# dasongli1/Shift-Net

Hardware: AMD Instinct MI355X
Metric: restored frames/sec at 1280x720 T=16 bf16 (higher is better)
Workload: dtype bf16; 1 GPU; Shift-Net-s (gshift_deblur2), 1280x720, one_len=16 (T_in=20), one window per GPU, synthetic checkpoint; parallelism=clip-parallel x1, gsts_schedule=unit-major, one stream

## Files before the change

include/shiftnet_hip.h:

```cpp
#ifndef SHIFTNET_HIP_H
#define SHIFTNET_HIP_H
#include <stdint.h>

#ifdef __cplusplus
extern "C" {
#endif

#define SN_ABI_VERSION 20

#define SN_F32 0
#define SN_F16 1
#define SN_BF16 2

int sn_abi_version(void);

int sn_selftest_mfma(const float* a, const float* b, float* d, void* stream);

int sn_ingest(const void* src, int src_dtype, const void* noise, void* dst, int T, int C, int H, int W, void* stream);

typedef struct sn_conv_desc {
    const void* in[3];
    int n_in;
    int cs_in;
    int T, h_in, w_in;
    int in_mode;
    int k, stride, pad;
    int h_out, w_out;
    const void* wfrag;
    int mt, ks;
    const float* bias;
    int act;
    float prelu;
    const void* res;
    void* out;
    int cs_out;
    int out_mode;
    int c_out;
    int nchw_dtype;
    const void* sc;
    int sc_dtype;
    float* pool;
    const float* oscale;
    int oscale_stride;
    const void* res2;
    int flags;
    int clip_n, clip_T, clip_lo;
} sn_conv_desc;
#define SN_CONV_TILE_KERNEL 1
int sn_conv2d(const sn_conv_desc* d, void* stream);
int sn_conv_pool_blocks(const sn_conv_desc* d);
#define SN_CONV_K_GENERIC 1
#define SN_CONV_K_FAST    2
#define SN_CONV_K_STATS   3
#define SN_CONV_K_STREAM  4
#define SN_CONV_ROUTE(kernel, mt, a, d, mode, rl) (((kernel) << 24) | ((mt) << 20) | ((a) << 12) | ((d) << 8) | ((mode) << 4) | (rl))
int sn_conv2d_route(const sn_conv_desc* d, int lines_len, int ncu, int* plan);

int sn_upsample2_add(const void* lo, const void* res, void* out, int T, int hs, int ws, int cs, void* stream);

int sn_ca_mlp(const float* partial, int nblk, int cpad, int c, int cr, float inv_hw,
              const float* wa, const float* wb, float* ca, int T, unsigned* bad, void* stream);

int sn_cab_ca_scratch_floats(int T);
int sn_cab_ca(const float* partial, int nblk, int cpad, const void* mid, int cs, int c, int cr, int h, int w,
              const float* w2, const float* wa, const float* wb, float* scratch, float* ca, int T, void* stream);
int sn_cab_fused_supported(const sn_conv_desc* conv1, const sn_conv_desc* conv2);
int sn_cab_stats(const sn_conv_desc* conv1, int lines_len, void* stream);
int sn_cab_ca_lines(const float* partial, int nblk, int cpad, const void* lines, int lines_len, int cs, int c, int cr, int h, int w,
                    const float* w2, const float* wa, const float* wb, float* scratch, float* ca, int T, void* stream);
int sn_cab_fused(const sn_conv_desc* conv1, const sn_conv_desc* conv2, int tile_rows, void* stream);

int sn32_cab_ca(const float* partial, int nblk, int cpad, const float* mid, int c, int cr, int h, int w,
                const float* w2, const float* wa, const float* wb, float* scratch, float* ca, int T, void* stream);

typedef struct sn_unit_src {
    const void* x;
    int T, h, w, C;
    int mode;
    int wrap;
    const void* halo;
    int t0, nt;
    int clip;
} sn_unit_src;

int sn_gsts_gather(const sn_unit_src* s, const int8_t* offs, void* u, void* stream);

int sn_temporal_roll(const sn_unit_src* s, void* y, void* stream);

int sn_gsts_shiftconv(const sn_unit_src* s, const int8_t* offs, const uint32_t* w1, void* hw, void* stream);
int sn_gsts_shiftconv_mfma(const sn_unit_src* s, const int8_t* offs, const uint32_t* w1, void* hw, void* stream);
#define SN_K0_TILE 1
#define SN_K0_WALK 2
#define SN_K0_PLAN_LEN 10
typedef struct sn_k0_opts {
    int form;
    int seg;
    int wgs;
} sn_k0_opts;
int sn_gsts_shiftconv_mfma_plan(const sn_unit_src* s, int ncu, int* plan);
int sn_gsts_shiftconv_mfma_plan_opt(const sn_unit_src* s, int ncu, const sn_k0_opts* opt, int* plan);
int sn_gsts_shiftconv_mfma_opt(const sn_unit_src* s, const int8_t* offs, const uint32_t* w1, void* hw, const sn_k0_opts* opt, void* stream);

int sn_ln_gemm_gate(const sn_unit_src* s, const void* hw, const void* wfrag, const float* bias, const uint32_t* wdw,
                    void* g1, float* pool, int g1_blocked, void* stream);
int sn_lngate_blocks(int h, int w);

int sn_grp5_gemm_gate(const void* g1, const float* ca_in, const void* wgrp, const void* wfrag, void* g2, float* pool,
                      int T, int h, int w, int C, void* stream);
int sn_grp5_blocks(int h, int w);

int sn_planar_pitch(int w);
int sn_nhwc_to_planar(const void* x, void* xp, int T, int h, int w, int C, void* stream);

int sn_dw5m_blocks(int h, int w);
int sn_dw5m_gemm_gate(const void* g1p, const float* ca_in, const void* ttab, const void* wfrag, void* g2, float* pool,
                      int T, int h, int w, int C, void* stream);

typedef struct sn_phase1_weights {
    const void* wfrag1;
    const uint32_t* w3;
    const void* wgrp;
    const void* wfrag2;
} sn_phase1_weights;
typedef struct sn_se_fold {
    const float* wa;
    const float* wb;
    int c, cr;
    unsigned* ticket;
    float* ca;
    unsigned* bad;
} sn_se_fold;
typedef struct sn_phase1_opts {
    const float* g1_scale;
    int g1_sums;
    int team;
    void* g1_store;
} sn_phase1_opts;
int sn_phase1_pool_blocks(int T, int h, int w);
int sn_phase1_g1_store_bytes(int T, int h, int w, int C, long long* bytes);
int sn_gsts_cab2_phase1(const sn_unit_src* s, const void* hw, const sn_phase1_weights* wt, void* g2, float* pool, const sn_se_fold* se,
                        const sn_phase1_opts* opt, void* stream);
int sn_cab1_phase1(const sn_unit_src* s, const sn_phase1_weights* wt, void* g2, float* pool, const sn_se_fold* se, const sn_phase1_opts* opt, void* stream);
int sn_p1r_plan(int nfr, int h, int w, int ncu, int team, int* out7);
int sn_p1r_strip_begin(const int* plan7, int s, int w);

int sn_gsts_cab2_phase2(const sn_unit_src* s, const void* g2, const float* ca, const void* wfrag, const float* bias, void* y, void* stream);
int sn_cab1_phase2(const sn_unit_src* s, const void* g2, const float* ca, const void* wfrag, const float* bias, void* y, void* stream);

int sn_cab2_phase2_cab1_phase1_supported(const sn_unit_src* s);
int sn_cab2_phase2_cab1_phase1(const sn_unit_src* s, const void* g2_in, const float* ca, const void* wfrag, const float* bias, void* y,
                               const sn_phase1_weights* wt, void* g2, float* pool, const sn_se_fold* se, const sn_phase1_opts* opt, void* stream);


typedef struct sn32_conv_desc {
    const float* in[3];
    int c_in[3];
    int cs_in[3];
    int n_in;
    int T, h_in, w_in;
    int in_mode;
    int k, stride, pad, groups;
    int h_out, w_out, c_out;
    const float* w;
    const float* bias;
    int act; float prelu;
    const float* oscale; int oscale_stride;
    const float* res; int cs_res;
    void* out; int cs_out;
    int out_mode;
    int nchw_dtype; const void* sc;
    const void* wsplit;
    const float* iscale; int iscale_stride;
    const float* rscale; int rscale_stride;
    const float* ln_w; const float* ln_b;
    float* csum; int csum_cpad;
    int clip_n, clip_T, clip_lo;
} sn32_conv_desc;
int sn32_conv_csum_tiles(int h_out, int w_out);
int sn32_conv2d(const sn32_conv_desc* d, void* stream);
#define SN32_K_1X1      1
#define SN32_K_SPLIT    2
#define SN32_K_SPLIT_G8 3
#define SN32_K_EXACT    4
#define SN32_K_DW       5
#define SN32_K_DIRECT   6
#define SN32_ROUTE(kernel, a, b) (((kernel) << 16) | ((a) << 8) | (b))
int sn32_conv2d_route(const sn32_conv_desc* d);
int sn32_gsts_gather(const sn_unit_src* s, const int8_t* offs, float* u, float* u2, void* stream);
int sn32_gsts_shiftconv(const sn_unit_src* s, const int8_t* offs, const float* w, float* vin, float* u, void* stream);
int sn32_layernorm(const float* x, int cs_x, int K, const float* w, const float* b, float* out, int cs_out, long long npix, void* stream);
int sn32_gate(const float* a, int C, int mode, float* out, long long npix, void* stream);
int sn32_gate_sum(const float* a, int C, int cpad, int mode, float* out, int T, int hw, int nblk, float* partial, void* stream);
int sn32_conv1x1_gate2(const float* x, int cs_x, int cin, const void* wsplit, int C, int cpad, float* out, int T, int hw, float* partial, void* stream);
int sn32_dw_gate(const float* a, int cs_a, const float* w, int C, int cpad, float* out, int T, int h, int wd, int nblk, float* partial, void* stream);
int sn32_chan_sum(const float* x, int cs, int C, int cpad, int T, int hw, int nblk, float* partial, void* stream);
int sn32_scale_residual(const float* r, const float* x, const float* ca, int ca_stride, float* out, int T, int hw, int C, void* stream);
int sn32_ingest(const void* src, int src_dtype, const void* noise, float* dst, int T, int C, int H, int W, void* stream);


int sn_ingest_u8(const uint8_t* src, void* dst, int dst_dtype, int T, int H, int W, void* stream);
int sn_egress_blocks(void);
int sn_egress_u8(const void* out, int out_dtype, const uint8_t* gt, uint8_t* img, float* sse, int T, int H, int W, void* stream);
int sn_ssim_blocks(void);
int sn_ssim_u8(const void* out, int out_dtype, const uint8_t* gt, float* scratch, float* partial, int T, int H, int W, void* stream);

#define SN_YUV_444 0
#define SN_YUV_420_CENTER 1
#define SN_YUV_420_LEFT 2
#define SN_YUV_BT601 0
#define SN_YUV_BT709 1
#define SN_YUV_LIMITED 0
#define SN_YUV_FULL 1
typedef struct sn_yuv_fmt {
    int bits;
    int chroma;
    int matrix;
    int range;
} sn_yuv_fmt;
int sn_ingest_yuv(const uint8_t* src, const sn_yuv_fmt* fmt, void* dst, int dst_dtype, int T, int H, int W, int Hp, int Wp, void* stream);
int sn_egress_yuv(const void* out, int out_dtype, const sn_yuv_fmt* fmt, uint8_t* dst, int T, int H, int W, int Hp, int Wp, void* stream);

int sn_yuv_thumb(const uint8_t* src, const sn_yuv_fmt* fmt, uint16_t* dst, int T, int H, int W, void* stream);

// ... 100 lines not shown
```

shift-net_amd/csrc/sn_cabf.hip:

```cpp
#include "sn_common.h"
#include "../../include/shiftnet_hip.h"

int sn_cabp_launch(const sn_conv_desc* a, const sn_conv_desc* b, void* stream);

namespace {

struct CabK {
    const bf16_t* x; int h, w;
    const uint4* w1; const float* b1; float prelu; int act;
    const uint4* w2; const float* b2;
    const float* oscale; int oscale_stride;
    const bf16_t* res2; bf16_t* out;
    XcdTiles xg;
};

constexpr __host__ __device__ int cabf_lds_slots(int npb) {
    const int k = npb <= 2 ? 2 : 4 * ((npb - 2 + 3) / 4) + 2;
    return k <= npb + 1 ? k : ((npb & 1) ? npb : npb + 1);
}
constexpr int cabf_waves(int mt, int th) {
    return mt == 1 ? (th == 8 ? 6 : 3) : mt == 2 ? 4 : mt == 3 ? 2 : 2;
}

template <int MT, int CS, int TH, int NC1, int NC2>
__global__ __launch_bounds__(256, cabf_waves(MT, TH)) void cab_fused_kernel(const CabK P) {
    extern __shared__ __attribute__((aligned(16))) char smem[];
    constexpr int TW = 32, RH = TH + 4, RW = TW + 4, MH = TH + 2, MW = TW + 2, NPB = CS / 8;
    constexpr int PS = 16 * cabf_lds_slots(NPB);
    constexpr int KTOT = 9 * CS, KS = (KTOT + 31) / 32;
    constexpr int ROWP = RW * NPB, NITEM = RH * ROWP, NIT = (NITEM + 255) / 256;
    constexpr int X_BYTES = RH * RW * PS;
    constexpr int NM = MH * MW, NT1 = (NM + 15) / 16, PER1 = (NT1 + 3) / 4;
    constexpr int NT2 = (TH * TW) / 64, XB = TW / 16;
    char* const xs = smem;
    char* const ms = smem + X_BYTES;
    const int tid = threadIdx.x & 255, lane = tid & 63, wv = wave_id();
    const int g = lane >> 4, p = lane & 15;
    int t, tyi, txi;
    if (!sn_xcd_tile(P.xg, t, tyi, txi)) return;
    const int oy0 = tyi * TH, ox0 = txi * TW;

    {
        const int iy0 = oy0 - 2, ix0 = ox0 - 2;
        const bf16_t* inb = P.x + (size_t)t * P.h * P.w * CS;
        const bool interior = iy0 >= 0 && iy0 + RH <= P.h && ix0 >= 0 && ix0 + RW <= P.w;
        uint4 v[NIT];
        if (interior) {
#pragma unroll
            for (int k = 0; k < NIT; ++k) {
                const int idx = tid + k * 256, idc = idx < NITEM ? idx : NITEM - 1;
                const int r = idc / ROWP, i = idc - r * ROWP;
                v[k] = *(const uint4*)(inb + ((size_t)iy0 * P.w + ix0) * CS + (size_t)r * P.w * CS + i * 8);
            }
#pragma unroll
            for (int k = 0; k < NIT; ++k) {
                const int idx = tid + k * 256;
                const int r = idx / ROWP, i = idx - r * ROWP, px = i / NPB, blk = i - px * NPB;
                if (idx < NITEM) *(uint4*)(xs + (r * RW + px) * PS + blk * 16) = v[k];
            }
        } else {
            bool in[NIT];
#pragma unroll
            for (int k = 0; k < NIT; ++k) {
                const int idx = tid + k * 256, idc = idx < NITEM ? idx : NITEM - 1;
                const int r = idc / ROWP, i = idc - r * ROWP, px = i / NPB, blk = i - px * NPB;
                const int gy = iy0 + r, gx = ix0 + px;
                in[k] = gy >= 0 && gy < P.h && gx >= 0 && gx < P.w;
                v[k] = *(const uint4*)(inb + (in[k] ? ((size_t)gy * P.w + gx) * CS + blk * 8 : 0));
            }
#pragma unroll
            for (int k = 0; k < NIT; ++k) {
                const int idx = tid + k * 256;
                const int r = idx / ROWP, i = idx - r * ROWP, px = i / NPB, blk = i - px * NPB;
                if (idx < NITEM) *(uint4*)(xs + (r * RW + px) * PS + blk * 16) = in[k] ? v[k] : make_uint4(0, 0, 0, 0);
            }
        }
    }
    const int c0 = g * 4 * MT;
    const float slope = P.prelu;
    const int act = P.act != 1 ? 0 : ((slope >= 0.f && slope <= 1.f) ? 1 : 2);
    __syncthreads();

#pragma unroll
    for (int ch = 0; ch < (PER1 + NC1 - 1) / NC1; ++ch) {
        int pixbase[NC1], moff[NC1];
        bool live[NC1], inimg[NC1];
#pragma unroll
        for (int n = 0; n < NC1; ++n) {
            const int j = wv + 4 * (ch * NC1 + n);
            const int q = j * 16 + p, qc = q < NM ? q : NM - 1;
            const int my = qc / MW, mx = qc - my * MW;
            pixbase[n] = (my * RW + mx) * PS;
            moff[n] = qc * PS;
            live[n] = (ch * NC1 + n < PER1) && q < NM;
            const int gy = oy0 - 1 + my, gx = ox0 - 1 + mx;
            inimg[n] = gy >= 0 && gy < P.h && gx >= 0 && gx < P.w;
        }
        f32x4_t acc[MT][NC1];
#pragma unroll
        for (int m = 0; m < MT; ++m) {
            const float4 b4 = P.b1 ? *(const float4*)(P.b1 + c0 + m * 4) : make_float4(0.f, 0.f, 0.f, 0.f);
#pragma unroll
            for (int n = 0; n < NC1; ++n) acc[m][n] = (f32x4_t){b4.x, b4.y, b4.z, b4.w};
        }
#pragma unroll
        for (int s = 0; s < KS; ++s) {
            int toff = 0;
#pragma unroll
            for (int gg = 0; gg < 4; ++gg) {
                const int kk0 = (s * 4 + gg) * 8;
                const int tap = kk0 / CS, cc0 = kk0 - tap * CS, dy = tap / 3, dx = tap - dy * 3;
                const int o = kk0 < KTOT ? (dy * RW + dx) * PS + cc0 * 2 : 0;
                toff = g == gg ? o : toff;
            }
            bf16x8_t a[MT];
#pragma unroll
            for (int m = 0; m < MT; ++m) a[m] = as_frag(P.w1[(m * KS + s) * 64 + lane]);
            bf16x8_t b[NC1];
#pragma unroll
            for (int n = 0; n < NC1; ++n) b[n] = as_frag(*(const uint4*)(xs + pixbase[n] + toff));
#pragma unroll
            for (int m = 0; m < MT; ++m)
#pragma unroll
                for (int n = 0; n < NC1; ++n) acc[m][n] = mfma16(a[m], b[n], acc[m][n]);
        }
#pragma unroll
        for (int n = 0; n < NC1; ++n) {
            if (ch * NC1 + n >= PER1) continue;
            uint32_t wd[MT][2];
#pragma unroll
            for (int m = 0; m < MT; ++m) {
                float v[4] = {acc[m][n][0], acc[m][n][1], acc[m][n][2], acc[m][n][3]};
                if (act == 1) {
#pragma unroll
                    for (int r = 0; r < 4; ++r) v[r] = fmaxf(v[r], slope * v[r]);
                } else if (act == 2) {
#pragma unroll
                    for (int r = 0; r < 4; ++r) v[r] = fmaf(slope, fminf(v[r], 0.f), fmaxf(v[r], 0.f));
                }
                wd[m][0] = inimg[n] ? pack_bf2(v[0], v[1]) : 0u;
                wd[m][1] = inimg[n] ? pack_bf2(v[2], v[3]) : 0u;
            }
            if (live[n]) {
                char* dst = ms + moff[n] + c0 * 2;
                if constexpr (MT == 2 || MT == 4) {
#pragma unroll
                    for (int m = 0; m < MT; m += 2)
                        if (c0 + m * 4 < CS) *(uint4*)(dst + m * 8) = make_uint4(wd[m][0], wd[m][1], wd[m + 1][0], wd[m + 1][1]);
                } else {
#pragma unroll
                    for (int m = 0; m < MT; ++m)
                        if (c0 + m * 4 < CS) *(uint2*)(dst + m * 8) = make_uint2(wd[m][0], wd[m][1]);
                }
            }
        }
    }
// ... 1 lines not shown

    const bool full = (oy0 + TH <= P.h) && (ox0 + TW <= P.w);
    const size_t tbase = (((size_t)t * P.h + oy0) * P.w + ox0) * CS;
    bf16_t* const outb = P.out + tbase;
    const bf16_t* const res2b = P.res2 ? P.res2 + tbase : nullptr;
    float4 osc[MT];
    const bool has_osc = P.oscale != nullptr;
#pragma unroll
    for (int m = 0; m < MT; ++m)
        osc[m] = has_osc ? *(const float4*)(P.oscale + (size_t)t * P.oscale_stride + c0 + m * 4) : make_float4(1.f, 1.f, 1.f, 1.f);
#pragma unroll
    for (int ch = 0; ch < (NT2 + NC2 - 1) / NC2; ++ch) {
        int pixbase[NC2], loff[NC2], xoff[NC2];
        bool valid[NC2];
#pragma unroll
        for (int n = 0; n < NC2; ++n) {
            const int nl = ch * NC2 + n < NT2 ? ch * NC2 + n : NT2 - 1;
            const int nn = wv * NT2 + nl, row = nn / XB, xb = nn - row * XB;
            pixbase[n] = (row * MW + xb * 16 + p) * PS;
            xoff[n] = ((row + 2) * RW + xb * 16 + p + 2) * PS + c0 * 2;
            loff[n] = (row * P.w + xb * 16 + p) * CS + c0;
            valid[n] = full || ((oy0 + row < P.h) && (ox0 + xb * 16 + p < P.w));
        }
        f32x4_t acc[MT][NC2];
#pragma unroll
        for (int m = 0; m < MT; ++m) {
            const float4 b4 = P.b2 ? *(const float4*)(P.b2 + c0 + m * 4) : make_float4(0.f, 0.f, 0.f, 0.f);
#pragma unroll
            for (int n = 0; n < NC2; ++n) acc[m][n] = (f32x4_t){b4.x, b4.y, b4.z, b4.w};
        }
#pragma unroll
        for (int s = 0; s < KS; ++s) {
            int toff = 0;
#pragma unroll
            for (int gg = 0; gg < 4; ++gg) {
                const int kk0 = (s * 4 + gg) * 8;
                const int tap = kk0 / CS, cc0 = kk0 - tap * CS, dy = tap / 3, dx = tap - dy * 3;
                const int o = kk0 < KTOT ? (dy * MW + dx) * PS + cc0 * 2 : 0;
                toff = g == gg ? o : toff;
            }
            bf16x8_t a[MT];
#pragma unroll
            for (int m = 0; m < MT; ++m) a[m] = as_frag(P.w2[(m * KS + s) * 64 + lane]);
            bf16x8_t b[NC2];
#pragma unroll
            for (int n = 0; n < NC2; ++n) b[n] = as_frag(*(const uint4*)(ms + pixbase[n] + toff));
#pragma unroll
            for (int m = 0; m < MT; ++m)
#pragma unroll
                for (int n = 0; n < NC2; ++n) acc[m][n] = mfma16(a[m], b[n], acc[m][n]);
        }
#pragma unroll
        for (int n = 0; n < NC2; ++n) {
            if (ch * NC2 + n >= NT2) continue;
            float v[MT][4];
#pragma unroll
            for (int m = 0; m < MT; ++m) {
                v[m][0] = acc[m][n][0]; v[m][1] = acc[m][n][1]; v[m][2] = acc[m][n][2]; v[m][3] = acc[m][n][3];
                if (has_osc) { v[m][0] *= osc[m].x; v[m][1] *= osc[m].y; v[m][2] *= osc[m].z; v[m][3] *= osc[m].w; }
            }
            if constexpr (MT == 2 || MT == 4) {
#pragma unroll
                for (int m = 0; m < MT; m += 2)
                    if (c0 + m * 4 < CS) {
                        const uint4 rr = *(const uint4*)(xs + xoff[n] + m * 8);
                        v[m][0] += bf_lo(rr.x); v[m][1] += bf_hi(rr.x); v[m][2] += bf_lo(rr.y); v[m][3] += bf_hi(rr.y);
                        v[m + 1][0] += bf_lo(rr.z); v[m + 1][1] += bf_hi(rr.z); v[m + 1][2] += bf_lo(rr.w); v[m + 1][3] += bf_hi(rr.w);
                    }
            } else {
#pragma unroll
                for (int m = 0; m < MT; ++m)
                    if (c0 + m * 4 < CS) {
                        const uint2 rr = *(const uint2*)(xs + xoff[n] + m * 8);
                        v[m][0] += bf_lo(rr.x); v[m][1] += bf_hi(rr.x); v[m][2] += bf_lo(rr.y); v[m][3] += bf_hi(rr.y);
                    }
            }
            if (!valid[n]) continue;
            if (res2b) {
                const bf16_t* src = res2b + loff[n];
                if constexpr (MT == 2 || MT == 4) {
#pragma unroll
                    for (int m = 0; m < MT; m += 2)
                        if (c0 + m * 4 < CS) {
                            const uint4 rr = *(const uint4*)(src + m * 4);
                            v[m][0] += bf_lo(rr.x); v[m][1] += bf_hi(rr.x); v[m][2] += bf_lo(rr.y); v[m][3] += bf_hi(rr.y);
                            v[m + 1][0] += bf_lo(rr.z); v[m + 1][1] += bf_hi(rr.z); v[m + 1][2] += bf_lo(rr.w); v[m + 1][3] += bf_hi(rr.w);
                        }
                } else {
#pragma unroll
                    for (int m = 0; m < MT; ++m)
                        if (c0 + m * 4 < CS) {
                            const uint2 rr = *(const uint2*)(src + m * 4);
                            v[m][0] += bf_lo(rr.x); v[m][1] += bf_hi(rr.x); v[m][2] += bf_lo(rr.y); v[m][3] += bf_hi(rr.y);
                        }
                }
            }
            bf16_t* dst = outb + loff[n];
            if constexpr (MT == 2 || MT == 4) {
#pragma unroll
                for (int m = 0; m < MT; m += 2)
                    if (c0 + m * 4 < CS)
                        *(uint4*)(dst + m * 4) = make_uint4(pack_bf2(v[m][0], v[m][1]), pack_bf2(v[m][2], v[m][3]),
                                                            pack_bf2(v[m + 1][0], v[m + 1][1]), pack_bf2(v[m + 1][2], v[m + 1][3]));
            } else {
#pragma unroll
                for (int m = 0; m < MT; ++m)
                    if (c0 + m * 4 < CS) {
                        uint2 o; o.x = pack_bf2(v[m][0], v[m][1]); o.y = pack_bf2(v[m][2], v[m][3]);
                        *(uint2*)(dst + m * 4) = o;
                    }
            }
        }
    }
}

template <int MT, int CS, int TH, int NC1, int NC2>
int launch_cab_fused(const CabK& K, int T, hipStream_t st) {
    constexpr int TW = 32, PS = 16 * cabf_lds_slots(CS / 8);
    CabK P = K; P.xg = sn_xcd_tiles((K.w + TW - 1) / TW, (K.h + TH - 1) / TH, T);
    const dim3 grid = sn_xcd_grid(P.xg);
    const size_t lds = (size_t)((TH + 4) * (TW + 4) + (TH + 2) * (TW + 2)) * PS;
    if (lds > 64 * 1024) {
        if (hipFuncSetAttribute((const void*)cab_fused_kernel<MT, CS, TH, NC1, NC2>, hipFuncAttributeMaxDynamicSharedMemorySize, (int)lds) != hipSuccess)
            return SN_ELAUNCH;
    }
    hipLaunchKernelGGL((cab_fused_kernel<MT, CS, TH, NC1, NC2>), grid, dim3(256), lds, st, P);
    return sn_check_launch();
}

int cabf_key(const sn_conv_desc* a, const sn_conv_desc* b) {
    if (!a || !b) return 0;
    const sn_conv_desc* ds[2] = {a, b};
    for (const sn_conv_desc* d : ds)
        if (!(d->k == 3 && d->stride == 1 && d->pad == 1 && d->in_mode == 0 && d->out_mode == 0 && d->n_in == 1 && d->cs_in == d->cs_out &&
              d->ks == (9 * d->cs_in + 31) / 32 && d->h_in == d->h_out && d->w_in == d->w_out && d->wfrag &&
              !sn_remap_set(d->clip_n, d->clip_T, d->clip_lo))) return 0;
    if (a->mt != b->mt || a->cs_in != b->cs_in || a->T != b->T || a->h_in != b->h_in || a->w_in != b->w_in) return 0;
    const int key = a->mt * 1000 + a->cs_in;
    return (key == 1016 || key == 2024) ? key : 0;
}

}

extern "C" {

int sn_cab_fused_supported(const sn_conv_desc* conv1, const sn_conv_desc* conv2) { return cabf_key(conv1, conv2) != 0 ? 1 : 0; }

int sn_cab_fused(const sn_conv_desc* a, const sn_conv_desc* b, int tile_rows, void* stream) {
    sn_clear_error();
    const int key = cabf_key(a, b);
    if (!key) return SN_EINVAL;
    if (tile_rows == 0) {
        if (!a->in[0] || a->res || a->res2 || a->oscale || b->pool || b->act != 0 || !b->out || b->res != a->in[0] || a->h_in < 2 || a->w_in < 2) return SN_EINVAL;
        return sn_cabp_launch(a, b, stream);
    }
    if (!a->in[0] || a->res || a->res2 || a->oscale || b->pool || b->act != 0 || !b->out || b->res != a->in[0]) return SN_EINVAL;
    if (b->oscale && b->oscale_stride < 16 * b->mt) return SN_EINVAL;
    if (a->h_in < 2 || a->w_in < 2) return SN_EINVAL;
    CabK K;
    K.x = (const bf16_t*)a->in[0]; K.h = a->h_in; K.w = a->w_in;
    K.w1 = (const uint4*)a->wfrag; K.b1 = a->bias; K.prelu = a->prelu; K.act = a->act;
    K.w2 = (const uint4*)b->wfrag; K.b2 = b->bias; K.oscale = b->oscale; K.oscale_stride = b->oscale_stride;
    K.res2 = (const bf16_t*)b->res2; K.out = (bf16_t*)b->out;
    hipStream_t st = (hipStream_t)stream;
    const bool tall = tile_rows == 16;
    switch (key) {
        case 1016: return tall ? launch_cab_fused<1, 16, 16, 5, 4>(K, a->T, st) : launch_cab_fused<1, 16, 8, 6, 4>(K, a->T, st);
        case 2024: return tall ? launch_cab_fused<2, 24, 16, 5, 4>(K, a->T, st) : launch_cab_fused<2, 24, 8, 3, 4>(K, a->T, st);
        default: return SN_EINVAL;
    }
}

}
```

shift-net_amd/csrc/sn_conv.hip:

```cpp
#include "sn_common.h"
#include "../../include/shiftnet_hip.h"

int sn_conv3p_key(const sn_conv_desc* d, bool want_pool);
int sn_conv3p_pool_rows(const sn_conv_desc* d);
int sn_conv3p_route(const sn_conv_desc* d, int lines_len, int ncu, int* plan8);
int sn_conv3p_launch(const sn_conv_desc* d, int lines_len, int route, const int* plan8, void* stream);

namespace {

struct ConvK {
    const bf16_t* in0; const bf16_t* in1; const bf16_t* in2;
    int n_in, cs, cv;
    int hin, win, in_mode, k, stride, pad, hout, wout;
    const uint4* wfrag; int ks;
    const float* bias; int act; float prelu;
    const bf16_t* res; bf16_t* out; int cs_out, out_mode, c_out, nchw_dtype, sc_dtype;
    const void* sc; float* pool; const float* oscale; int oscale_stride; const bf16_t* res2;
    int rh, rw, ps;
    int clip_n, clip_T, clip_lo;
    int lines_len;
    XcdTiles xg;
    unsigned m_nblk8, m_rw, m_csb, m_cv, m_k;
};

constexpr __host__ __device__ int sn_lds_slots(int npb) {
    const int k = npb <= 2 ? 2 : 4 * ((npb - 2 + 3) / 4) + 2;
    return k <= npb + 1 ? k : ((npb & 1) ? npb : npb + 1);
}

__device__ __forceinline__ int fdiv(int x, unsigned magic) { return (int)(((unsigned)x * (unsigned long long)magic) >> 24); }

__device__ __forceinline__ uint4 ld_bilinear(const bf16_t* src, int t, int hs, int ws, int cs, int cb, int gy, int gx) {
    float sy = gy * 0.5f - 0.25f; if (sy < 0.f) sy = 0.f;
    float sx = gx * 0.5f - 0.25f; if (sx < 0.f) sx = 0.f;
    int y0 = (int)sy, x0 = (int)sx;
    int y1 = min(y0 + 1, hs - 1), x1 = min(x0 + 1, ws - 1);
    float ly = sy - y0, lx = sx - x0, hy = 1.f - ly, hx = 1.f - lx;
    const bf16_t* b = src + (size_t)t * hs * ws * cs + cb * 8;
    float v00[8], v01[8], v10[8], v11[8], o[8];
    unpack8(*(const uint4*)(b + ((size_t)y0 * ws + x0) * cs), v00);
    unpack8(*(const uint4*)(b + ((size_t)y0 * ws + x1) * cs), v01);
    unpack8(*(const uint4*)(b + ((size_t)y1 * ws + x0) * cs), v10);
    unpack8(*(const uint4*)(b + ((size_t)y1 * ws + x1) * cs), v11);
#pragma unroll
    for (int j = 0; j < 8; ++j) o[j] = hy * (hx * v00[j] + lx * v01[j]) + ly * (hx * v10[j] + lx * v11[j]);
    return pack8(o);
}

constexpr int sn_conv_waves(int mt) {
    return mt == 1 ? 6 : mt == 2 ? 5 : mt == 3 ? 4 : mt == 4 ? 3 : 2;
}
constexpr int sn_conv3_waves(int mt, int cs) {
    return mt == 1 ? 7 : mt == 2 ? 6 : mt == 3 ? (cs == 48 ? 3 : 4) : mt == 4 ? 3 : 2;
}

template <int MT, int TH, int TW>
__global__ __launch_bounds__(256, sn_conv_waves(MT)) void conv_mfma_kernel(const ConvK P) {
    extern __shared__ __attribute__((aligned(16))) char smem[];
    constexpr int NTW = (TH * TW) / 64;
    constexpr int XB = TW / 16;
    const int tid = threadIdx.x, lane = tid & 63, wv = wave_id();
    const int g = lane >> 4, p = lane & 15;
    int t, tyi, txi;
    if (!sn_xcd_tile(P.xg, t, tyi, txi)) return;
    const int ti = sn_remap_frame(t, P.clip_n, P.clip_T, P.clip_lo);
    const int oy0 = tyi * TH, ox0 = txi * TW;
    const int tile_bytes = P.rh * P.rw * P.ps;
    int* tapoff = (int*)(smem + tile_bytes);
    float* red = (float*)(smem + tile_bytes + ((P.ks * 4 * 4 + 15) & ~15));

    for (int e = tid; e < P.ks * 4; e += 256) {
        const int kk0 = e * 8, K = P.k * P.k * P.cv;
        int off = 0;
        if (kk0 < K) {
            const int tap = fdiv(kk0, P.m_cv), cc0 = kk0 - tap * P.cv;
            const int dy = fdiv(tap, P.m_k), dx = tap - dy * P.k;
            off = (dy * P.rw + dx) * P.ps + cc0 * 2;
        }
        tapoff[e] = off;
    }
    {
        const int nblk8 = P.cv >> 3, csb = P.cs >> 3, total = P.rh * P.rw * nblk8;
        const int iy0 = oy0 * P.stride - P.pad, ix0 = ox0 * P.stride - P.pad;
        for (int idx0 = tid; idx0 < total; idx0 += 4 * 256) {
            uint4 v[4];
            int dst[4];
#pragma unroll
            for (int u = 0; u < 4; ++u) {
                const int idx = idx0 + u * 256;
                const int idc = idx < total ? idx : tid;
                const int pix = fdiv(idc, P.m_nblk8), blk = idc - pix * nblk8;
                const int ry = fdiv(pix, P.m_rw), rx = pix - ry * P.rw;
                const int ii = fdiv(blk, P.m_csb), cb = blk - ii * csb;
                const bf16_t* src = ii == 0 ? P.in0 : (ii == 1 ? P.in1 : P.in2);
                const int gy = iy0 + ry, gx = ix0 + rx;
                const bool in = gy >= 0 && gy < P.hin && gx >= 0 && gx < P.win;
                dst[u] = idx < total ? (in ? pix * P.ps + blk * 16 : -(pix * P.ps + blk * 16) - 1) : 0x7fffffff;
                if (P.in_mode == 0) v[u] = *(const uint4*)(src + (in ? (((size_t)ti * P.hin + gy) * P.win + gx) * P.cs + cb * 8 : 0));
                else v[u] = in ? ld_bilinear(src, ti, P.hin >> 1, P.win >> 1, P.cs, cb, gy, gx) : make_uint4(0, 0, 0, 0);
            }
#pragma unroll
            for (int u = 0; u < 4; ++u) {
                if (dst[u] == 0x7fffffff) continue;
                const bool in = dst[u] >= 0;
                *(uint4*)(smem + (in ? dst[u] : -(dst[u] + 1))) = in ? v[u] : make_uint4(0, 0, 0, 0);
            }
        }
    }
    bf16x8_t a_cur[MT];
#pragma unroll
    for (int m = 0; m < MT; ++m) a_cur[m] = as_frag(P.wfrag[(m * P.ks) * 64 + lane]);
    __syncthreads();

    f32x4_t acc[MT][NTW];
#pragma unroll
    for (int m = 0; m < MT; ++m)
#pragma unroll
        for (int n = 0; n < NTW; ++n) acc[m][n] = (f32x4_t){0.f, 0.f, 0.f, 0.f};
    int pixbase[NTW];
#pragma unroll
    for (int n = 0; n < NTW; ++n) {
        const int nn = wv * NTW + n, row = nn / XB, xb = nn - row * XB;
        pixbase[n] = ((row * P.stride) * P.rw + (xb * 16 + p) * P.stride) * P.ps;
    }
    constexpr bool PRE_RES = MT == 1;
    uint2 rres[PRE_RES ? MT : 1][PRE_RES ? NTW : 1];
    if constexpr (PRE_RES) {
        const bf16_t* rb = P.res ? P.res : (const bf16_t*)P.wfrag;
#pragma unroll
        for (int n = 0; n < NTW; ++n) {
            const int nn = wv * NTW + n, row = nn / XB, xb = nn - row * XB;
            const int oy = oy0 + row, ox = ox0 + xb * 16 + p;
            const bool valid = P.res && (oy < P.hout) && (ox < P.wout);
            const size_t opix = ((size_t)t * P.hout + oy) * P.wout + ox;
#pragma unroll
            for (int m = 0; m < MT; ++m) {
                const int co0 = g * 4 * MT + m * 4;
                rres[m][n] = *(const uint2*)(rb + ((valid && co0 < P.cs_out) ? opix * P.cs_out + co0 : 0));
            }
        }
    }
    for (int s = 0; s < P.ks; ++s) {
        const int toff = tapoff[s * 4 + g];
        const int sn = s + 1 < P.ks ? s + 1 : s;
        bf16x8_t a_nxt[MT];
#pragma unroll
        for (int m = 0; m < MT; ++m) a_nxt[m] = as_frag(P.wfrag[(m * P.ks + sn) * 64 + lane]);
        bf16x8_t b[NTW];
#pragma unroll
        for (int n = 0; n < NTW; ++n) b[n] = as_frag(*(const uint4*)(smem + pixbase[n] + toff));
#pragma unroll
        for (int m = 0; m < MT; ++m)
#pragma unroll
// ... 406 lines not shown
    }
    __syncthreads();
    if (tid < cr) {
        float h = 0.f;
        for (int j = 0; j < c; ++j) h += wa[tid * c + j] * mean[j];
        hid[tid] = h > 0.f ? h : 0.f;
    }
    __syncthreads();
    if (tid < cpad) {
        float o = 0.f;
        if (tid < c) {
            for (int j = 0; j < cr; ++j) o += wb[tid * cr + j] * hid[j];
            o = sigmoidf_(o);
        }
        ca[(size_t)t * cpad + tid] = o;
    }
}

#define SN_CABCA_NS 16
__device__ __forceinline__ float cab_ldf(const bf16_t* p) { return bf_to_f(*p); }
__device__ __forceinline__ float cab_ldf(const float* p) { return *p; }
template <typename E>
__device__ __forceinline__ const E* cab_px(const E* mt, int L, int w, int cs, int line, int y, int x) {
    return L > 0 ? mt + ((size_t)line * L + (line < 2 ? x : y)) * cs : mt + ((size_t)y * w + x) * cs;
}
template <typename E>
__global__ __launch_bounds__(256) void cab_ca_part_kernel(const float* partial, int nblk, int cpad, const E* mid, int cs,
                                                        int h, int w, float* scratch, int L) {
    __shared__ float acc[256];
    const int t = blockIdx.y, sidx = blockIdx.x, tid = threadIdx.x;
    const E* mt = mid + (L > 0 ? (size_t)t * 4 * L * cs : (size_t)t * h * w * cs);
    float* out = scratch + ((size_t)t * SN_CABCA_NS + sidx) * 5 * 128;
    {
        const int nsplit = 256 / cpad, ch = tid % cpad, part = tid / cpad;
        float sm = 0.f;
        if (part < nsplit) {
            const float* pp = partial + (size_t)t * nblk * cpad + ch;
            for (int bb = sidx * nsplit + part; bb < nblk; bb += SN_CABCA_NS * nsplit) sm += pp[(size_t)bb * cpad];
        }
        acc[tid] = sm;
        __syncthreads();
        if (tid < cpad) {
            float m = 0.f;
            for (int q = 0; q < nsplit; ++q) m += acc[q * cpad + tid];
            if (tid < 128) out[tid] = m;
        }
        __syncthreads();
    }
    for (int line = 0; line < 4; ++line) {
        const int len = line < 2 ? w : h;
        const int nseg = 256 / cs, ch = tid % cs, seg = tid / cs;
        float sm = 0.f;
        if (seg < nseg)
            for (int i = sidx * nseg + seg; i < len; i += SN_CABCA_NS * nseg) {
                const int y = line == 0 ? 0 : (line == 1 ? h - 1 : i), x = line == 2 ? 0 : (line == 3 ? w - 1 : i);
                sm += cab_ldf(cab_px(mt, L, w, cs, line, y, x) + ch);
            }
        acc[tid] = sm;
        __syncthreads();
        if (tid < cs) {
            float m = 0.f;
            for (int q = 0; q < nseg; ++q) m += acc[q * cs + tid];
            out[(1 + line) * 128 + tid] = m;
        }
        __syncthreads();
    }
}

template <typename E>
__global__ __launch_bounds__(1024) void cab_ca_kernel(const float* scratch, int cpad, const E* mid, int cs, int c, int cr,
                                                     int h, int w, const float* w2, const float* wa, const float* wb, float* ca, int L) {
    __shared__ float acc[1024];
    __shared__ float S[9][128];
    __shared__ float mean[128];
    __shared__ float hid[128];
    const int t = blockIdx.x, tid = threadIdx.x;
    const E* mt = mid + (L > 0 ? (size_t)t * 4 * L * cs : (size_t)t * h * w * cs);
    if (tid < 5 * 128) {
        const int k = tid >> 7, ch = tid & 127;
        float m = 0.f;
        if (ch < (k == 0 ? cpad : cs)) {
            const float* sp = scratch + (size_t)t * SN_CABCA_NS * 5 * 128 + tid;
            for (int q = 0; q < SN_CABCA_NS; ++q) m += sp[q * 5 * 128];
        }
        S[k][ch] = m;
    }
    if (tid < cs) {
        S[5][tid] = cab_ldf(cab_px(mt, L, w, cs, 0, 0, 0) + tid);
        S[6][tid] = cab_ldf(cab_px(mt, L, w, cs, 0, 0, w - 1) + tid);
        S[7][tid] = cab_ldf(cab_px(mt, L, w, cs, 1, h - 1, 0) + tid);
        S[8][tid] = cab_ldf(cab_px(mt, L, w, cs, 1, h - 1, w - 1) + tid);
    }
    __syncthreads();
    {
        const int nsplit = 1024 / cpad, co = tid % cpad, part = tid / cpad;
        float r = 0.f;
        if (part < nsplit)
            for (int cin = part; cin < c; cin += nsplit) {
                const float tot = S[0][cin], r0 = S[1][cin], r1 = S[2][cin], c0 = S[3][cin], c1 = S[4][cin];
                const float k00 = S[5][cin], k01 = S[6][cin], k10 = S[7][cin], k11 = S[8][cin];
                const float* wk = w2 + (size_t)cin * 9 * cpad + co;
                const float rowex[3] = {r1, 0.f, r0}, colex[3] = {c1, 0.f, c0};
                const float cor[3][3] = {{k11, 0.f, k10}, {0.f, 0.f, 0.f}, {k01, 0.f, k00}};
#pragma unroll
                for (int ky = 0; ky < 3; ++ky)
#pragma unroll
                    for (int kx = 0; kx < 3; ++kx) r += wk[(ky * 3 + kx) * cpad] * (tot - rowex[ky] - colex[kx] + cor[ky][kx]);
            }
        acc[tid] = r;
        __syncthreads();
        if (tid < cpad) {
            float m = 0.f;
            for (int q = 0; q < nsplit; ++q) m += acc[q * cpad + tid];
            if (tid < 128) mean[tid] = m / ((float)h * (float)w);
        }
    }
    __syncthreads();
    if (tid < cr) {
        float hh = 0.f;
        for (int j = 0; j < c; ++j) hh += wa[tid * c + j] * mean[j];
        hid[tid] = hh > 0.f ? hh : 0.f;
    }
    __syncthreads();
    if (tid < cpad) {
        float o = 0.f;
        if (tid < c) {
            for (int j = 0; j < cr; ++j) o += wb[tid * cr + j] * hid[j];
            o = sigmoidf_(o);
        }
        ca[(size_t)t * cpad + tid] = o;
    }
}

__global__ void selftest_mfma_kernel(const float* a, const float* b, float* d) {
    const int lane = threadIdx.x, g = lane >> 4, m = lane & 15;
    float av[8], bv[8];
#pragma unroll
    for (int j = 0; j < 8; ++j) {
        av[j] = a[m * 32 + g * 8 + j];
        bv[j] = b[(g * 8 + j) * 16 + m];
    }
    f32x4_t acc = {0.f, 0.f, 0.f, 0.f};
    acc = mfma16(as_frag(pack8(av)), as_frag(pack8(bv)), acc);
#pragma unroll
    for (int r = 0; r < 4; ++r) d[(g * 4 + r) * 16 + m] = acc[r];
}

__global__ __launch_bounds__(256) void upsample2_add_kernel(const bf16_t* __restrict__ lo, const bf16_t* __restrict__ res, bf16_t* __restrict__ out,
                                                            int hs, int ws, int npb) {
    const int w2 = 2 * ws, cs = npb * 8, i = (int)blockIdx.y, t = (int)blockIdx.z;
    const int e = (int)blockIdx.x * 256 + (int)threadIdx.x;
    if (e >= w2 * npb) return;
    const int x = e / npb, piece = e - x * npb;
    float sx = x * 0.5f - 0.25f; if (sx < 0.f) sx = 0.f;
    const int x0 = (int)sx, x1 = min(x0 + 1, ws - 1);
    const float lx = sx - x0, hx = 1.f - lx;
    const int ra = max(i - 1, 0), rc = min(i + 1, hs - 1);
    const bf16_t* b = lo + (size_t)t * hs * ws * cs + piece * 8;
    const uint4 qa0 = *(const uint4*)(b + ((size_t)ra * ws + x0) * cs), qa1 = *(const uint4*)(b + ((size_t)ra * ws + x1) * cs);
    const uint4 qb0 = *(const uint4*)(b + ((size_t)i * ws + x0) * cs), qb1 = *(const uint4*)(b + ((size_t)i * ws + x1) * cs);
    const uint4 qc0 = *(const uint4*)(b + ((size_t)rc * ws + x0) * cs), qc1 = *(const uint4*)(b + ((size_t)rc * ws + x1) * cs);
    const size_t o0 = (((size_t)t * 2 * hs + 2 * i) * w2 + x) * cs + piece * 8, o1 = o0 + (size_t)w2 * cs;
    const uint4 r0 = *(const uint4*)(res + o0), r1 = *(const uint4*)(res + o1);
    float a0[8], a1[8], b0[8], b1[8], c0[8], c1[8], f0[8], f1[8], u0[8], u1[8];
    unpack8(qa0, a0); unpack8(qa1, a1); unpack8(qb0, b0); unpack8(qb1, b1); unpack8(qc0, c0); unpack8(qc1, c1); unpack8(r0, f0); unpack8(r1, f1);
    const float ly0 = i > 0 ? 0.75f : 0.f, hy0 = 1.f - ly0;
#pragma unroll
    for (int j = 0; j < 8; ++j) {
        const float va = hx * a0[j] + lx * a1[j], vb = hx * b0[j] + lx * b1[j], vc = hx * c0[j] + lx * c1[j];
        u0[j] = (hy0 * va + ly0 * vb) + f0[j];
        u1[j] = (0.75f * vb + 0.25f * vc) + f1[j];
    }
    *(uint4*)(out + o0) = pack8(u0);
    *(uint4*)(out + o1) = pack8(u1);
}

}

extern "C" {

int sn_abi_version(void) { return SN_ABI_VERSION; }

int sn_selftest_mfma(const float* a, const float* b, float* d, void* stream) {
    sn_clear_error();
    hipLaunchKernelGGL(selftest_mfma_kernel, dim3(1), dim3(64), 0, (hipStream_t)stream, a, b, d);
    return sn_check_launch();
}

int sn_ingest(const void* src, int dt, const void* noise, void* dst, int T, int C, int H, int W, void* stream) {
    sn_clear_error();
    if (!src || !dst || C < 1 || C + (noise ? 1 : 0) > 8 || dt < 0 || dt > 2) return SN_EINVAL;
    const int hw = H * W;
    hipLaunchKernelGGL(ingest_kernel, dim3((hw + 255) / 256, T), dim3(256), 0, (hipStream_t)stream, src, dt, noise, (uint4*)dst, C, hw);
    return sn_check_launch();
}

static int conv3_key(const sn_conv_desc* d) {
    if (!(d->k == 3 && d->stride == 1 && d->pad == 1 && d->in_mode == 0 && d->out_mode == 0 && d->n_in == 1 && d->ks == (9 * d->cs_in + 31) / 32)) return 0;
    const int key = d->mt * 1000 + d->cs_in;
    return (key == 1016 || key == 2024 || key == 4064 || key == 3040 || key == 3048 || key == 5080) ? key : 0;
}
static void conv_tile(const sn_conv_desc* d, int* th, int* tw) {
    if (d->stride == 1) { *tw = 32; *th = 8; }
    else if (d->n_in * d->cs_in <= 24 && !(d->flags & (1 << 15))) { *th = 8; *tw = 32; }
    else { *th = 4; *tw = 16; }
}

int sn_conv_pool_blocks(const sn_conv_desc* d) {
    if (!d) return SN_EINVAL;
    if (!(d->flags & SN_CONV_TILE_KERNEL)) {
        const int rows = sn_conv3p_pool_rows(d);
        if (rows > 0) return rows;
    }
    int th, tw; conv_tile(d, &th, &tw);
    return ((d->h_out + th - 1) / th) * ((d->w_out + tw - 1) / tw);
}

static int conv_ps(const sn_conv_desc* d) {
    const int blocks = d->n_in * d->cs_in >> 3;
    return d->stride == 1 ? 16 * sn_lds_slots(blocks) : ((blocks & 1) ? blocks * 16 : blocks * 16 + 16);
}

static int conv_route(const sn_conv_desc* d, int lines_len, int ncu, int* plan8) {
    if (!d) return SN_EINVAL;
    const bool stream_ok = !(d->flags & SN_CONV_TILE_KERNEL);
    if (lines_len > 0) {
        if (!d->out || !d->pool || !d->wfrag || !d->in[0] || d->res || d->res2 || d->oscale || d->cs_in != d->cs_out ||
            sn_remap_set(d->clip_n, d->clip_T, d->clip_lo)) return SN_EINVAL;
        if (lines_len < (d->h_out > d->w_out ? d->h_out : d->w_out) || d->h_out < 2 || d->w_out < 2) return SN_EINVAL;
        if (stream_ok) {
            const int r = sn_conv3p_route(d, lines_len, ncu, plan8);
            if (r >= 0) return r;
        }
        const int key = conv3_key(d);
        if (key != 1016 && key != 2024) return SN_EINVAL;
        return SN_CONV_ROUTE(SN_CONV_K_STATS, key / 1000, key % 1000, 0, 0, 0);
    }
    if (d->n_in < 1 || d->n_in > 3 || (d->cs_in & 7) || (d->cs_out & 7) || !d->wfrag) return SN_EINVAL;
    if (!d->out) return SN_EINVAL;
    if (d->k < 1 || d->k > 5 || (d->stride != 1 && d->stride != 2) || d->mt < 1 || d->mt > 6 || d->ks < 1) return SN_EINVAL;
    if (d->in_mode == 1 && ((d->h_in | d->w_in) & 1)) return SN_EINVAL;
    if (d->out_mode == 2 && (!d->sc || d->c_out > 4 * d->mt || d->nchw_dtype < 0 || d->nchw_dtype > 2 || d->sc_dtype < 0 || d->sc_dtype > 2)) return SN_EINVAL;
    if (d->ks * 32 < d->k * d->k * d->n_in * d->cs_in) return SN_EINVAL;
    if (d->oscale && d->oscale_stride < 16 * d->mt) return SN_EINVAL;
    if ((d->res || d->res2) && d->out_mode != 0) return SN_EINVAL;
    if (d->out_mode == 1 && d->cs_out != 4 * d->mt) return SN_EINVAL;
    const bool remap = sn_remap_set(d->clip_n, d->clip_T, d->clip_lo);
    if (!sn_remap_ok(d->T, d->clip_n, d->clip_T, d->clip_lo) || (remap && (conv3_key(d) || (stream_ok && sn_conv3p_key(d, false)))))
        return SN_EINVAL;
    if (stream_ok && sn_conv3p_key(d, false)) {
        const int r = sn_conv3p_route(d, 0, ncu, plan8);
        if (r >= 0) return r;
    }
    const int key = conv3_key(d);
    if (key) return SN_CONV_ROUTE(SN_CONV_K_FAST, key / 1000, key % 1000, 0, 0, 0);
    int th, tw; conv_tile(d, &th, &tw);
    if (conv_generic_lds(th, tw, d->stride, d->k, conv_ps(d), d->ks, d->mt) > 160 * 1024) return SN_EINVAL;
    return SN_CONV_ROUTE(SN_CONV_K_GENERIC, d->mt, th, 0, 0, 0);
}

int sn_conv2d_route(const sn_conv_desc* d, int lines_len, int ncu, int* plan) {
    sn_clear_error();
    return conv_route(d, lines_len, ncu, plan);
}

int sn_conv2d(const sn_conv_desc* d, void* stream) {
    sn_clear_error();
    int plan8[8];
    const int route = conv_route(d, 0, 0, plan8);
    if (route < 0) return route;
    ConvK K;
    K.in0 = (const bf16_t*)d->in[0]; K.in1 = (const bf16_t*)d->in[1]; K.in2 = (const bf16_t*)d->in[2];
    K.n_in = d->n_in; K.cs = d->cs_in; K.cv = d->n_in * d->cs_in;
    K.hin = d->h_in; K.win = d->w_in; K.in_mode = d->in_mode; K.k = d->k; K.stride = d->stride; K.pad = d->pad;
    K.hout = d->h_out; K.wout = d->w_out;
    K.wfrag = (const uint4*)d->wfrag; K.ks = d->ks; K.bias = d->bias; K.act = d->act; K.prelu = d->prelu;
    K.res = (const bf16_t*)d->res; K.out = (bf16_t*)d->out; K.cs_out = d->cs_out; K.out_mode = d->out_mode;
    K.c_out = d->c_out; K.nchw_dtype = d->nchw_dtype; K.sc_dtype = d->sc_dtype; K.sc = d->sc; K.pool = d->pool; K.oscale = d->oscale; K.oscale_stride = d->oscale_stride; K.res2 = (const bf16_t*)d->res2;
    K.ps = conv_ps(d);
    K.rh = K.rw = 0; K.lines_len = 0;
    K.clip_n = d->clip_n; K.clip_T = d->clip_T; K.clip_lo = d->clip_lo;
    hipStream_t st = (hipStream_t)stream;
    const int mt = (route >> 20) & 15, a = (route >> 12) & 255;
    switch (route >> 24) {
        case SN_CONV_K_STREAM: return sn_conv3p_launch(d, 0, route, plan8, stream);
        case SN_CONV_K_FAST:
            switch (mt * 1000 + a) {
                case 1016: return launch_conv3_fast<1, 16>(K, d->T, st);
                case 2024: return launch_conv3_fast<2, 24>(K, d->T, st);
                case 4064: return launch_conv3_fast<4, 64>(K, d->T, st);
                case 3040: return launch_conv3_fast<3, 40>(K, d->T, st);
                case 3048: return launch_conv3_fast<3, 48>(K, d->T, st);
                case 5080: return launch_conv3_fast<5, 80>(K, d->T, st);
                default: return SN_EINVAL;
            }
        case SN_CONV_K_GENERIC: return a == 8 ? launch_conv<8, 32>(K, mt, d->T, st) : launch_conv<4, 16>(K, mt, d->T, st);
        default: return SN_EINVAL;
    }
}


int sn_ca_mlp(const float* partial, int nblk, int cpad, int c, int cr, float inv_hw,
              const float* wa, const float* wb, float* ca, int T, unsigned* bad, void* stream) {
    sn_clear_error();
    if (!partial || !wa || !wb || !ca || cpad < 16 || cpad > 128 || c > cpad || cr > 128 || cr < 1 || nblk < 1) return SN_EINVAL;
    hipLaunchKernelGGL(ca_mlp_kernel, dim3(T), dim3(1024), 0, (hipStream_t)stream, partial, nblk, cpad, c, cr, inv_hw, wa, wb, ca, bad);
    return sn_check_launch();
}

int sn_cab_ca_scratch_floats(int T) { return T * SN_CABCA_NS * 5 * 128; }

static int cab_ca_launch(const float* partial, int nblk, int cpad, const void* mid, int lines_len, int cs, int c, int cr, int h, int w,
                         const float* w2, const float* wa, const float* wb, float* scratch, float* ca, int T, void* stream) {
    sn_clear_error();
    if (!partial || !mid || !w2 || !wa || !wb || !ca || !scratch || cpad < 16 || cpad > 128 || cs > 128 || (cs & 7) || c > cs ||
        c > cpad || cr < 1 || cr > 128 || nblk < 1 || h < 2 || w < 2 || (lines_len != 0 && lines_len < (h > w ? h : w))) return SN_EINVAL;
    hipLaunchKernelGGL(cab_ca_part_kernel<bf16_t>, dim3(SN_CABCA_NS, T), dim3(256), 0, (hipStream_t)stream, partial, nblk, cpad,
                       (const bf16_t*)mid, cs, h, w, scratch, lines_len);
    hipLaunchKernelGGL(cab_ca_kernel<bf16_t>, dim3(T), dim3(1024), 0, (hipStream_t)stream, (const float*)scratch, cpad, (const bf16_t*)mid, cs,
                       c, cr, h, w, w2, wa, wb, ca, lines_len);
    return sn_check_launch();
}

int sn_cab_ca(const float* partial, int nblk, int cpad, const void* mid, int cs, int c, int cr, int h, int w,
// ... 51 lines not shown
```

shift-net_amd/csrc/sn_conv3p.hip:

```cpp
#include "sn_common.h"
#include "../../include/shiftnet_hip.h"

namespace {

typedef __attribute__((address_space(3))) void lds_void_t;

struct C3P {
    const bf16_t* in; const bf16_t* res; bf16_t* out;
    const uint4* wfrag; const float* bias; const float* oscale; int oscale_stride;
    const uint4* w2; const float* b2;
    float* pool; int pool_rows;
    int act; float prelu;
    int T, h, w, ntx, nty;
    int dbg;
    int lines_len;
    int S, nseg, nsg, qs;
};

__device__ __forceinline__ float max_bare(float a, float b) {
    float r;
    asm("v_max_f32 %0, %1, %2" : "=v"(r) : "v"(a), "v"(b));
    return r;
}

__device__ __forceinline__ float mul_then_add(float a, float b, float c) {
    float r;
    asm("v_mul_f32 %0, %1, %2\n\tv_add_f32 %0, %0, %3" : "=&v"(r) : "v"(a), "v"(b), "v"(c));
    return r;
}

__device__ __forceinline__ void dma16(const __amdgpu_buffer_rsrc_t rs, char* dst, int voffset) {
    __builtin_amdgcn_raw_ptr_buffer_load_lds(rs, (lds_void_t*)dst, 16, voffset, 0, 0, 0);
}

template <typename V> __device__ __forceinline__ void pin(V& x) { asm volatile("" : "+v"(x)); }

template <int N> __device__ __forceinline__ void wait_vmcnt() { asm volatile("s_waitcnt vmcnt(%0)" ::"n"(N) : "memory"); }

__device__ __forceinline__ __amdgpu_buffer_rsrc_t frame_rsrc(const bf16_t* base, int frame_bytes) {
    return __builtin_amdgcn_make_buffer_rsrc((void*)base, 0, frame_bytes, 0x00020000);
}

constexpr int c3p_waves(int mt) { return mt == 1 ? 4 : mt == 2 ? 3 : 2; }

template <int MT, int CS, int TH, int D, int MODE, bool RL = false>
__global__ __launch_bounds__(320, c3p_waves(MT)) void conv3p_kernel(const C3P P) {
    extern __shared__ __attribute__((aligned(16))) char smem[];
    constexpr int TW = 32, RH = TH + 2, RW = TW + 2, NPB = CS / 8, PSB = CS * 2;
    constexpr int KTOT = 9 * CS, KS = (KTOT + 31) / 32;
    constexpr int ROWP = RW * NPB, NITEM = RH * ROWP, NDMA = (NITEM + 63) / 64, XBUF = NDMA * 1024;
    static_assert(!RL || MODE == 2, "residual staging belongs to MODE 2");
    constexpr int RDMA = RL ? (TH * TW * NPB) / 64 : 0;
    constexpr int NBUF = D + 1, BUFSZ = XBUF + RDMA * 1024, NL = NDMA + RDMA;
    constexpr bool WLDS = MT * KS > 16;
    constexpr int WBYTES = WLDS ? MT * KS * 1024 : 0;
    constexpr int RPW = TH / 4, NTW = RPW * 2;
    constexpr int NH = MT == 1 ? (NTW < 4 ? NTW : 4) : 2;
    static_assert(NTW % NH == 0 && NTW <= 4 * NH, "passes");
    static_assert(TH % 4 == 0 && NL * (D - 1) <= 63 && D >= 1, "tile / prefetch shape");
    const int lane = threadIdx.x & 63, wv = wave_id();
    const int G = (int)gridDim.x, c = ((int)blockIdx.x & 7) * (G >> 3) + ((int)blockIdx.x >> 3);
    const int fseg = c * P.qs, nsegs = min(P.qs, P.nsg - fseg);
    if (nsegs <= 0) return;
    int t = fseg / (P.ntx * P.nseg), tx, ty, n = 0;
    {
        const int rem = fseg - t * (P.ntx * P.nseg);
        tx = rem / P.nseg;
        const int sg = rem - tx * P.nseg;
        ty = sg * P.S;
        const int tail = P.nty - (P.nseg - 1) * P.S;
        for (int k = 0, g2 = sg; k < nsegs; ++k) { n += g2 == P.nseg - 1 ? tail : P.S; if (++g2 == P.nseg) g2 = 0; }
    }
    n = __builtin_amdgcn_readfirstlane(n);
    t = __builtin_amdgcn_readfirstlane(t); tx = __builtin_amdgcn_readfirstlane(tx); ty = __builtin_amdgcn_readfirstlane(ty);
    const int rowpitch = P.w * PSB, frame_bytes = P.h * rowpitch;
    const size_t frame_elems = (size_t)P.h * P.w * CS;
    char* const xbufs = smem + WBYTES;
    if constexpr (WLDS) {
        for (int i = (int)threadIdx.x; i < MT * KS * 64; i += 320) *(uint4*)(smem + i * 16) = P.wfrag[i];
        __syncthreads();
    }

    if (wv == 4) {
        int voff[NDMA], pxk[NDMA];
#pragma unroll
        for (int k = 0; k < NDMA; ++k) {
            const int i = k * 64 + lane, ic = i < NITEM ? i : NITEM - 1;
            const int r = ic / ROWP, j = ic - r * ROWP;
            voff[k] = r * rowpitch + j * 16;
            pxk[k] = j / NPB;
        }
        int rvoff[RL ? RDMA : 1];
        if constexpr (RL) {
#pragma unroll
            for (int k = 0; k < RDMA; ++k) {
                const int i = k * 64 + lane, row = i / (TW * NPB), rem = i - row * (TW * NPB);
                rvoff[k] = row * rowpitch + rem * 16;
            }
        }
        int ft = t, ftx = tx, fty = ty;
        for (int i = -D; i < n; ++i) {
            if (i >= 0) {
                if (n - 1 - i >= D - 1) wait_vmcnt<NL * (D - 1)>(); else wait_vmcnt<0>();
                __builtin_amdgcn_s_barrier();
            }
            const int j = i + D;
            if (j < n && !(P.dbg & 1)) {
                const __amdgpu_buffer_rsrc_t rs = frame_rsrc(P.in + (size_t)ft * frame_elems, frame_bytes);
                const int ix0 = ftx * TW - 1;
                const int o = ((fty * TH - 1) * P.w + ix0) * PSB;
                const bool edge = ftx == 0 || ix0 + RW > P.w;
                char* const dst = xbufs + (j % NBUF) * BUFSZ;
#pragma unroll
                for (int k = 0; k < NDMA; ++k) {
                    int vo = voff[k] + o;
                    if (edge) { const int gx = ix0 + pxk[k]; vo = (gx < 0 || gx >= P.w) ? (int)0x80000000 : vo; }
                    dma16(rs, dst + k * 1024, vo);
                }
                if constexpr (RL) {
                    const __amdgpu_buffer_rsrc_t rr = frame_rsrc(P.res + (size_t)ft * frame_elems, frame_bytes);
                    const int o2 = ((fty * TH) * P.w + ftx * TW) * PSB;
#pragma unroll
                    for (int k = 0; k < RDMA; ++k)
                        dma16(rr, dst + XBUF + k * 1024, rvoff[k] + o2);
                }
                if (++fty == P.nty) { fty = 0; if (++ftx == P.ntx) { ftx = 0; ++ft; } }
            }
        }
        return;
    }

    const int g = lane >> 4, p = lane & 15;
    const int c0 = g * 4 * MT;
    int addr_s[KS];
    const int lane_base = ((wv * RPW) * RW + p) * PSB;
#pragma unroll
    for (int s = 0; s < KS; ++s) {
        int toff = 0;
#pragma unroll
        for (int gg = 0; gg < 4; ++gg) {
            const int kk0 = (s * 4 + gg) * 8;
            const int tap = kk0 / CS, cc0 = kk0 - tap * CS, dy = tap / 3, dx = tap - dy * 3;
            const int o = kk0 < KTOT ? (dy * RW + dx) * PSB + cc0 * 2 : 0;
            toff = g == gg ? o : toff;
        }
        addr_s[s] = lane_base + toff;
    }
    bf16x8_t A[WLDS ? 1 : MT][WLDS ? 1 : KS];
    if constexpr (!WLDS) {
#pragma unroll
        for (int m = 0; m < MT; ++m)
#pragma unroll
            for (int s = 0; s < KS; ++s) A[m][s] = as_frag(P.wfrag[(m * KS + s) * 64 + lane]);
    }
    const char* const wl = smem + lane * 16;
    f32x4_t biasv[MT];
#pragma unroll
    for (int m = 0; m < MT; ++m) {
        const float4 b4 = P.bias ? *(const float4*)(P.bias + c0 + m * 4) : make_float4(0.f, 0.f, 0.f, 0.f);
        biasv[m] = (f32x4_t){b4.x, b4.y, b4.z, b4.w};
    }
    const float slope = P.prelu;
    float4 osc[MT];
    auto load_osc = [&](int ft) {
        if constexpr (MODE == 2) {
#pragma unroll
            for (int m = 0; m < MT; ++m) osc[m] = *(const float4*)(P.oscale + (size_t)ft * P.oscale_stride + c0 + m * 4);
        }
    };
    load_osc(t);
    auto pin_loaded = [&]() __attribute__((always_inline)) {
        if constexpr (!WLDS) {
#pragma unroll
            for (int m = 0; m < MT; ++m)
#pragma unroll
                for (int s = 0; s < KS; ++s) pin(A[m][s]);
        }
#pragma unroll
        for (int m = 0; m < MT; ++m) {
            pin(biasv[m]);
            if constexpr (MODE == 2) { pin(osc[m].x); pin(osc[m].y); pin(osc[m].z); pin(osc[m].w); }
        }
    };
    pin_loaded();
    constexpr int OOR = (int)0x80000000;
    constexpr int PIECE = (MT == 2 || MT == 4) ? 16 : 8;
    constexpr int NP = (MT * 8) / PIECE;
    typedef unsigned rword_t __attribute__((ext_vector_type(PIECE / 4)));
    int ooff[RPW][NP];
#pragma unroll
    for (int rr = 0; rr < RPW; ++rr)
#pragma unroll
        for (int q = 0; q < NP; ++q)
            ooff[rr][q] = (c0 + q * (PIECE / 2) < CS) ? ((wv * RPW + rr) * P.w + p) * PSB + c0 * 2 + q * PIECE : OOR;
    typedef rword_t rset_t[(MODE == 2 && !RL) ? NTW : 1][(MODE == 2 && !RL) ? NP : 1];
    rset_t rA, rB;
    auto load_res = [&](rset_t& rnxt, int ft, int ftx, int fty) __attribute__((always_inline)) {
        if constexpr (MODE == 2 && !RL) {
            const __amdgpu_buffer_rsrc_t rr = frame_rsrc(P.res + (size_t)ft * frame_elems, frame_bytes);
            const int o2 = ((fty * TH) * P.w + ftx * TW) * PSB;
#pragma unroll
            for (int nn = 0; nn < NTW; ++nn)
#pragma unroll
                for (int q = 0; q < NP; ++q) {
                    const int vo = o2 + ooff[nn >> 1][q] + (nn & 1) * 16 * PSB;
                    if constexpr (PIECE == 16) rnxt[nn][q] = __builtin_amdgcn_raw_buffer_load_b128(rr, vo, 0, 0);
                    else rnxt[nn][q] = __builtin_amdgcn_raw_buffer_load_b64(rr, vo, 0, 0);
                }
        }
    };
    load_res(rA, t, tx, ty);
    float psum[MT][4];
#pragma unroll
    for (int m = 0; m < MT; ++m)
#pragma unroll
        for (int r = 0; r < 4; ++r) psum[m][r] = 0.f;
    auto flush_pool = [&](int ft, int ftx, int fsg) {
        if constexpr (MODE == 1 || MODE == 3) {
            const int row = (ftx * P.nseg + fsg) * 4 + wv;
            float* dst = P.pool + ((size_t)ft * P.pool_rows + row) * (16 * MT);
#pragma unroll
            for (int m = 0; m < MT; ++m)
#pragma unroll
                for (int r = 0; r < 4; ++r) {
                    const float sm = row_sum16(psum[m][r]);
                    if (p == 0) dst[c0 + m * 4 + r] = sm;
                    psum[m][r] = 0.f;
                }
        }
    };

    const int raddr = XBUF + ((wv * RPW) * TW + p) * PSB + c0 * 2;
    auto finish = [&](const f32x4_t (&acc)[MT][NH], const rset_t& rres, const char* xs, const int N0, const __amdgpu_buffer_rsrc_t ro, int o2, const bool MASKED,
                      int ylim, int xlim) __attribute__((always_inline)) {
#pragma unroll
        for (int nh = 0; nh < NH; ++nh) {
            const int nn = N0 + nh, rr = nn >> 1, xb = nn & 1;
            float v[MT][4];
#pragma unroll
            for (int m = 0; m < MT; ++m) {
                v[m][0] = acc[m][nh][0]; v[m][1] = acc[m][nh][1]; v[m][2] = acc[m][nh][2]; v[m][3] = acc[m][nh][3];
                if constexpr (MODE == 1 || MODE == 3) {
#pragma unroll
                    for (int r = 0; r < 4; ++r) {
                        v[m][r] = max_bare(v[m][r], slope * v[m][r]);
                    }
                }
            }
            if constexpr (MODE == 2) {
#pragma unroll
                for (int m = 0; m < MT; ++m) {
                    rword_t qv;
                    if constexpr (RL) qv = *(const rword_t*)(xs + raddr + (rr * TW + xb * 16) * PSB + ((m * 8) / PIECE) * PIECE);
                    else qv = rres[nn][(m * 8) / PIECE];
                    const unsigned lo = qv[((m * 8) % PIECE) / 4], hi = qv[((m * 8) % PIECE) / 4 + 1];
                    v[m][0] = mul_then_add(v[m][0], osc[m].x, bf_lo(lo)); v[m][1] = mul_then_add(v[m][1], osc[m].y, bf_hi(lo));
                    v[m][2] = mul_then_add(v[m][2], osc[m].z, bf_lo(hi)); v[m][3] = mul_then_add(v[m][3], osc[m].w, bf_hi(hi));
                }
            }
            bool ok = true;
            if (MASKED) ok = (rr < ylim) && (xb * 16 < xlim);
            if constexpr (MODE == 1 || MODE == 3) {
#pragma unroll
                for (int m = 0; m < MT; ++m)
#pragma unroll
                    for (int r = 0; r < 4; ++r) psum[m][r] += (MASKED && !ok) ? 0.f : v[m][r];
            }
            if constexpr (MODE == 3) {
                if (MASKED && ok && c0 < CS) {
                    const int oy = ty * TH + wv * RPW + rr, ox = tx * TW + xb * 16 + p;
                    bf16_t* const lb = P.out + (size_t)t * 4 * P.lines_len * CS + c0;
                    bf16_t* tgt[4] = {oy == 0 ? lb + (size_t)ox * CS : nullptr, oy == P.h - 1 ? lb + ((size_t)P.lines_len + ox) * CS : nullptr,
                                      ox == 0 ? lb + ((size_t)2 * P.lines_len + oy) * CS : nullptr, ox == P.w - 1 ? lb + ((size_t)3 * P.lines_len + oy) * CS : nullptr};
#pragma unroll
                    for (int e = 0; e < 4; ++e) {
                        if (!tgt[e]) continue;
#pragma unroll
                        for (int m = 0; m < MT; ++m)
                            if (c0 + m * 4 < CS) *(uint2*)(tgt[e] + m * 4) = make_uint2(pack_bf2(v[m][0], v[m][1]), pack_bf2(v[m][2], v[m][3]));
                    }
                }
                continue;
            }
#pragma unroll
            for (int q = 0; q < NP; ++q) {
                int vo = o2 + ooff[rr][q] + xb * 16 * PSB;
                if (MASKED) vo = ok ? vo : OOR;
                if (P.dbg & 4) vo = OOR;
                if constexpr (PIECE == 16) {
                    const int m = q * 2;
                    const rword_t d = {pack_bf2(v[m][0], v[m][1]), pack_bf2(v[m][2], v[m][3]), pack_bf2(v[m + 1][0], v[m + 1][1]), pack_bf2(v[m + 1][2], v[m + 1][3])};
                    __builtin_amdgcn_raw_buffer_store_b128(d, ro, vo, 0, 0);
                } else {
                    const rword_t d = {pack_bf2(v[q][0], v[q][1]), pack_bf2(v[q][2], v[q][3])};
                    __builtin_amdgcn_raw_buffer_store_b64(d, ro, vo, 0, 0);
                }
            }
        }
    };

    int sgi = ty / P.S, sleft = min(P.S, P.nty - ty);
    int t2 = t, tx2 = tx, ty2 = ty;
    auto advance2 = [&]() { if (++ty2 == P.nty) { ty2 = 0; if (++tx2 == P.ntx) { tx2 = 0; ++t2; } } };
    advance2();
    auto tile = [&](const int i, const rset_t& rres, rset_t& rnxt) __attribute__((always_inline)) {
        __builtin_amdgcn_s_barrier();
        const char* const xs = xbufs + (i % NBUF) * BUFSZ;
        if (i + 1 < n) load_res(rnxt, t2, tx2, ty2);
        const int oy0 = ty * TH, ox0 = tx * TW;
        const __amdgpu_buffer_rsrc_t ro = frame_rsrc(P.out + (size_t)t * frame_elems, frame_bytes);
        const int o2 = (oy0 * P.w + ox0) * PSB;
        const bool full = (oy0 + TH <= P.h) && (ox0 + TW <= P.w);
#pragma unroll
        for (int ps = 0; ps < NTW / NH; ++ps) {
            const int N0 = ps * NH;
            f32x4_t acc[MT][NH];
            bf16x8_t bq[2][NH], aq[2][WLDS ? MT : 1];
#pragma unroll
            for (int m = 0; m < MT; ++m)
#pragma unroll
                for (int nh = 0; nh < NH; ++nh) acc[m][nh] = biasv[m];
            if (!(P.dbg & 2)) {
#pragma unroll
            for (int nh = 0; nh < NH; ++nh)
                bq[0][nh] = as_frag(*(const uint4*)(xs + addr_s[0] + (((N0 + nh) >> 1) * RW + ((N0 + nh) & 1) * 16) * PSB));
            if constexpr (WLDS) {
#pragma unroll
                for (int m = 0; m < MT; ++m) aq[0][m] = as_frag(*(const uint4*)(wl + (m * KS) * 1024));
            }
#pragma unroll
            for (int s = 0; s < KS; ++s) {
                if (s + 1 < KS) {
#pragma unroll
                    for (int nh = 0; nh < NH; ++nh)
                        bq[(s + 1) & 1][nh] = as_frag(*(const uint4*)(xs + addr_s[s + 1] + (((N0 + nh) >> 1) * RW + ((N0 + nh) & 1) * 16) * PSB));
                    if constexpr (WLDS) {
#pragma unroll
                        for (int m = 0; m < MT; ++m) aq[(s + 1) & 1][m] = as_frag(*(const uint4*)(wl + (m * KS + s + 1) * 1024));
                    }
                }
                __builtin_amdgcn_sched_barrier(0);
#pragma unroll
                for (int m = 0; m < MT; ++m)
#pragma unroll
                    for (int nh = 0; nh < NH; ++nh)
                        acc[m][nh] = mfma16(WLDS ? aq[s & 1][m] : A[WLDS ? 0 : m][WLDS ? 0 : s], bq[s & 1][nh], s == 0 ? biasv[m] : acc[m][nh]);
                __builtin_amdgcn_sched_barrier(0);
            }
            }
            const bool plain = full && !(MODE == 3 && (ty == 0 || ty == P.nty - 1 || tx == 0 || tx == P.ntx - 1));
            if (plain) finish(acc, rres, xs, N0, ro, o2, false, 0, 0);
            else finish(acc, rres, xs, N0, ro, o2, true, P.h - oy0 - wv * RPW, P.w - ox0 - p);
        }
        if (--sleft == 0) {
            flush_pool(t, tx, sgi);
            ++sgi;
            sleft = min(P.S, P.nty - ty - 1);
        }
        if (++ty == P.nty) {
            ty = 0; sgi = 0; sleft = min(P.S, P.nty);
            if (++tx == P.ntx) {
                tx = 0;
                ++t;
                if (i + 1 < n) {
                    load_osc(t);
                    if constexpr (MODE == 2) {
#pragma unroll
                        for (int m = 0; m < MT; ++m) { pin(osc[m].x); pin(osc[m].y); pin(osc[m].z); pin(osc[m].w); }
                    }
                }
            }
        }
        advance2();
    };
    for (int i = 0; i < n; i += 2) {
        tile(i, rA, rB);
        if (i + 1 < n) tile(i + 1, rB, rA);
    }
}

template <int MT, int CS, int TH, int D, int WR>
__global__ __launch_bounds__(320, c3p_waves(MT)) void cabp_kernel(const C3P P) {
    extern __shared__ __attribute__((aligned(16))) char smem[];
    constexpr int TW = 32, RH = TH + 4, RW = TW + 4, MH = TH + 2, MW = TW + 2, NPB = CS / 8, PSB = CS * 2;
    constexpr int KTOT = 9 * CS, KS = (KTOT + 31) / 32;
    constexpr int ROWP = RW * NPB, NITEM = RH * ROWP, NDMA = (NITEM + 63) / 64, XBUF = NDMA * 1024;
    constexpr int NBUF = D + 1, NL = NDMA;
    constexpr bool W1L = !(WR & 1), W2L = !(WR & 2);
    constexpr int WSET = MT * KS * 1024, W2OFF = W1L ? WSET : 0, WBYTES = W2OFF + (W2L ? WSET : 0);
    constexpr int NM = MH * MW, NT1 = (NM + 15) / 16, PER1 = (NT1 + 3) / 4;
    constexpr int NH1 = MT == 1 ? 3 : 2;
    constexpr int RPW = TH / 4, NTW = RPW * 2, NH = MT == 1 ? (NTW < 4 ? NTW : 4) : 2;
    constexpr int MIDB = (NM * PSB + 15) / 16 * 16;
    static_assert(TH % 4 == 0 && NL * (D - 1) <= 63 && D >= 1 && PER1 % NH1 == 0 && NTW % NH == 0, "tile / prefetch shape");
    const int lane = threadIdx.x & 63, wv = wave_id();
    const int G = (int)gridDim.x, c = ((int)blockIdx.x & 7) * (G >> 3) + ((int)blockIdx.x >> 3);
    const int fseg = c * P.qs, nsegs = min(P.qs, P.nsg - fseg);
    if (nsegs <= 0) return;
    int t = fseg / (P.ntx * P.nseg), tx, ty, n = 0;
    {
        const int rem = fseg - t * (P.ntx * P.nseg);
        tx = rem / P.nseg;
        const int sg = rem - tx * P.nseg;
        ty = sg * P.S;
        const int tail = P.nty - (P.nseg - 1) * P.S;
        for (int k = 0, g2 = sg; k < nsegs; ++k) { n += g2 == P.nseg - 1 ? tail : P.S; if (++g2 == P.nseg) g2 = 0; }
    }
    n = __builtin_amdgcn_readfirstlane(n);
    t = __builtin_amdgcn_readfirstlane(t); tx = __builtin_amdgcn_readfirstlane(tx); ty = __builtin_amdgcn_readfirstlane(ty);
    const int rowpitch = P.w * PSB, frame_bytes = P.h * rowpitch;
    const size_t frame_elems = (size_t)P.h * P.w * CS;
    char* const mids = smem + WBYTES;
    char* const xbufs = mids + MIDB;
    if constexpr (W1L || W2L) {
        for (int i = (int)threadIdx.x; i < MT * KS * 64; i += 320) {
            if constexpr (W1L) *(uint4*)(smem + i * 16) = P.wfrag[i];
            if constexpr (W2L) *(uint4*)(smem + W2OFF + i * 16) = P.w2[i];
        }
        __syncthreads();
    }

    if (wv == 4) {
        int voff[NDMA], pxk[NDMA];
#pragma unroll
        for (int k = 0; k < NDMA; ++k) {
            const int i = k * 64 + lane, ic = i < NITEM ? i : NITEM - 1;
            const int r = ic / ROWP, j = ic - r * ROWP;
            voff[k] = r * rowpitch + j * 16;
            pxk[k] = j / NPB;
        }
        int ft = t, ftx = tx, fty = ty;
        for (int i = -D; i < n; ++i) {
            if (i >= 0) {
                if (n - 1 - i >= D - 1) wait_vmcnt<NL * (D - 1)>(); else wait_vmcnt<0>();
                __builtin_amdgcn_s_barrier();
            }
            const int j = i + D;
            if (j < n) {
                const __amdgpu_buffer_rsrc_t rs = frame_rsrc(P.in + (size_t)ft * frame_elems, frame_bytes);
                const int ix0 = ftx * TW - 2;
                const int o = ((fty * TH - 2) * P.w + ix0) * PSB;
                const bool edge = ftx == 0 || ix0 + RW > P.w;
                char* const dst = xbufs + (j % NBUF) * XBUF;
#pragma unroll
                for (int k = 0; k < NDMA; ++k) {
                    int vo = voff[k] + o;
                    if (edge) { const int gx = ix0 + pxk[k]; vo = (gx < 0 || gx >= P.w) ? (int)0x80000000 : vo; }
                    dma16(rs, dst + k * 1024, vo);
                }
                if (++fty == P.nty) { fty = 0; if (++ftx == P.ntx) { ftx = 0; ++ft; } }
            }
            if (i >= 0) __builtin_amdgcn_s_barrier();
        }
        return;
    }

    const int g = lane >> 4, p = lane & 15;
    const int c0 = g * 4 * MT;
    int toff1[KS], addr2[KS];
    const int lane_base2 = ((wv * RPW) * MW + p) * PSB;
#pragma unroll
    for (int s = 0; s < KS; ++s) {
        int o1 = 0, o2 = 0;
#pragma unroll
        for (int gg = 0; gg < 4; ++gg) {
            const int kk0 = (s * 4 + gg) * 8;
            const int tap = kk0 / CS, cc0 = kk0 - tap * CS, dy = tap / 3, dx = tap - dy * 3;
            const int a = kk0 < KTOT ? (dy * RW + dx) * PSB + cc0 * 2 : 0, b = kk0 < KTOT ? (dy * MW + dx) * PSB + cc0 * 2 : 0;
            o1 = g == gg ? a : o1; o2 = g == gg ? b : o2;
        }
        toff1[s] = o1;
        addr2[s] = lane_base2 + o2;
    }
    int pix1[PER1], mwr[PER1];
#pragma unroll
    for (int i = 0; i < PER1; ++i) {
        const int q = (wv + 4 * i) * 16 + p, qc = q < NM ? q : NM - 1;
        const int my = qc / MW, mx = qc - my * MW;
        pix1[i] = (my * RW + mx) * PSB;
        mwr[i] = (q < NM && c0 < CS) ? qc * PSB + c0 * 2 : -1;
    }
    bf16x8_t A1[W1L ? 1 : MT][W1L ? 1 : KS], A2[W2L ? 1 : MT][W2L ? 1 : KS];
    if constexpr (!W1L) {
#pragma unroll
        for (int m = 0; m < MT; ++m)
#pragma unroll
            for (int s = 0; s < KS; ++s) A1[m][s] = as_frag(P.wfrag[(m * KS + s) * 64 + lane]);
    }
    if constexpr (!W2L) {
#pragma unroll
        for (int m = 0; m < MT; ++m)
#pragma unroll
            for (int s = 0; s < KS; ++s) A2[m][s] = as_frag(P.w2[(m * KS + s) * 64 + lane]);
    }
    const char* const wl = smem + lane * 16;
    f32x4_t bias1[MT], bias2[MT];
#pragma unroll
    for (int m = 0; m < MT; ++m) {
        const float4 a4 = P.bias ? *(const float4*)(P.bias + c0 + m * 4) : make_float4(0.f, 0.f, 0.f, 0.f);
        const float4 b4 = P.b2 ? *(const float4*)(P.b2 + c0 + m * 4) : make_float4(0.f, 0.f, 0.f, 0.f);
        bias1[m] = (f32x4_t){a4.x, a4.y, a4.z, a4.w};
        bias2[m] = (f32x4_t){b4.x, b4.y, b4.z, b4.w};
    }
    const float slope = P.prelu;
    float4 osc[MT];
    auto load_osc = [&](int ft) {
#pragma unroll
        for (int m = 0; m < MT; ++m) osc[m] = *(const float4*)(P.oscale + (size_t)ft * P.oscale_stride + c0 + m * 4);
    };
    load_osc(t);
    auto pin_osc = [&]() __attribute__((always_inline)) {
#pragma unroll
        for (int m = 0; m < MT; ++m) { pin(osc[m].x); pin(osc[m].y); pin(osc[m].z); pin(osc[m].w); }
    };
#pragma unroll
    for (int m = 0; m < MT; ++m) {
        pin(bias1[m]); pin(bias2[m]);
        if constexpr (!W1L) {
#pragma unroll
            for (int s = 0; s < KS; ++s) pin(A1[m][s]);
        }
        if constexpr (!W2L) {
#pragma unroll
            for (int s = 0; s < KS; ++s) pin(A2[m][s]);
        }
    }
    pin_osc();
    constexpr int OOR = (int)0x80000000;
    constexpr int PIECE = (MT == 2 || MT == 4) ? 16 : 8, NP = (MT * 8) / PIECE;
    typedef unsigned rword_t __attribute__((ext_vector_type(PIECE / 4)));
    int ooff[RPW][NP];
#pragma unroll
    for (int rr = 0; rr < RPW; ++rr)
#pragma unroll
        for (int q = 0; q < NP; ++q)
            ooff[rr][q] = (c0 + q * (PIECE / 2) < CS) ? ((wv * RPW + rr) * P.w + p) * PSB + c0 * 2 + q * PIECE : OOR;
    const int raddr = ((wv * RPW + 2) * RW + p + 2) * PSB + c0 * 2;

    for (int i = 0; i < n; ++i) {
        __builtin_amdgcn_s_barrier();
        const char* const xs = xbufs + (i % NBUF) * XBUF;
        const int oy0 = ty * TH, ox0 = tx * TW;
        const bool inner = oy0 >= 1 && oy0 + TH + 1 <= P.h && ox0 >= 1 && ox0 + TW + 1 <= P.w;
#pragma unroll
        for (int ps = 0; ps < PER1 / NH1; ++ps) {
            f32x4_t acc[MT][NH1];
            bf16x8_t bq[2][NH1], aq[2][W1L ? MT : 1];
#pragma unroll
            for (int nh = 0; nh < NH1; ++nh) bq[0][nh] = as_frag(*(const uint4*)(xs + pix1[ps * NH1 + nh] + toff1[0]));
            if constexpr (W1L) {
#pragma unroll
                for (int m = 0; m < MT; ++m) aq[0][m] = as_frag(*(const uint4*)(wl + (m * KS) * 1024));
            }
#pragma unroll
            for (int s = 0; s < KS; ++s) {
                if (s + 1 < KS) {
#pragma unroll
                    for (int nh = 0; nh < NH1; ++nh) bq[(s + 1) & 1][nh] = as_frag(*(const uint4*)(xs + pix1[ps * NH1 + nh] + toff1[s + 1]));
                    if constexpr (W1L) {
#pragma unroll
                        for (int m = 0; m < MT; ++m) aq[(s + 1) & 1][m] = as_frag(*(const uint4*)(wl + (m * KS + s + 1) * 1024));
                    }
                }
                __builtin_amdgcn_sched_barrier(0);
#pragma unroll
                for (int m = 0; m < MT; ++m)
#pragma unroll
                    for (int nh = 0; nh < NH1; ++nh)
                        acc[m][nh] = mfma16(W1L ? aq[s & 1][m] : A1[W1L ? 0 : m][W1L ? 0 : s], bq[s & 1][nh], s == 0 ? bias1[m] : acc[m][nh]);
                __builtin_amdgcn_sched_barrier(0);
            }
#pragma unroll
            for (int nh = 0; nh < NH1; ++nh) {
                const int i1 = ps * NH1 + nh;
                bool in = true;
                if (!inner) {
                    const int pq = pix1[i1] / PSB, my = pq / RW, mx = pq - my * RW;
                    const int gy = oy0 - 1 + my, gx = ox0 - 1 + mx;
                    in = gy >= 0 && gy < P.h && gx >= 0 && gx < P.w;
                }
                unsigned wd[MT][2];
#pragma unroll
                for (int m = 0; m < MT; ++m) {
                    float v[4] = {acc[m][nh][0], acc[m][nh][1], acc[m][nh][2], acc[m][nh][3]};
#pragma unroll
                    for (int r = 0; r < 4; ++r) v[r] = max_bare(v[r], slope * v[r]);
                    wd[m][0] = in ? pack_bf2(v[0], v[1]) : 0u;
                    wd[m][1] = in ? pack_bf2(v[2], v[3]) : 0u;
                }
                if (mwr[i1] >= 0) {
                    char* dst = mids + mwr[i1];
                    if constexpr (MT == 2 || MT == 4) {
#pragma unroll
                        for (int m = 0; m < MT; m += 2)
                            if (c0 + m * 4 < CS) *(uint4*)(dst + m * 8) = make_uint4(wd[m][0], wd[m][1], wd[m + 1][0], wd[m + 1][1]);
                    } else {
#pragma unroll
                        for (int m = 0; m < MT; ++m)
                            if (c0 + m * 4 < CS) *(uint2*)(dst + m * 8) = make_uint2(wd[m][0], wd[m][1]);
                    }
                }
            }
        }
        __builtin_amdgcn_s_barrier();
        const __amdgpu_buffer_rsrc_t ro = frame_rsrc(P.out + (size_t)t * frame_elems, frame_bytes);
        const int o2 = (oy0 * P.w + ox0) * PSB;
        const bool full = (oy0 + TH <= P.h) && (ox0 + TW <= P.w);
        const int ylim = P.h - oy0 - wv * RPW, xlim = P.w - ox0 - p;
#pragma unroll
        for (int ps = 0; ps < NTW / NH; ++ps) {
            const int N0 = ps * NH;
            f32x4_t acc[MT][NH];
            bf16x8_t bq[2][NH], aq[2][W2L ? MT : 1];
#pragma unroll
            for (int nh = 0; nh < NH; ++nh)
                bq[0][nh] = as_frag(*(const uint4*)(mids + addr2[0] + (((N0 + nh) >> 1) * MW + ((N0 + nh) & 1) * 16) * PSB));
            if constexpr (W2L) {
#pragma unroll
                for (int m = 0; m < MT; ++m) aq[0][m] = as_frag(*(const uint4*)(wl + W2OFF + (m * KS) * 1024));
            }
#pragma unroll
            for (int s = 0; s < KS; ++s) {
                if (s + 1 < KS) {
#pragma unroll
                    for (int nh = 0; nh < NH; ++nh)
                        bq[(s + 1) & 1][nh] = as_frag(*(const uint4*)(mids + addr2[s + 1] + (((N0 + nh) >> 1) * MW + ((N0 + nh) & 1) * 16) * PSB));
                    if constexpr (W2L) {
#pragma unroll
                        for (int m = 0; m < MT; ++m) aq[(s + 1) & 1][m] = as_frag(*(const uint4*)(wl + W2OFF + (m * KS + s + 1) * 1024));
                    }
                }
                __builtin_amdgcn_sched_barrier(0);
#pragma unroll
                for (int m = 0; m < MT; ++m)
#pragma unroll
                    for (int nh = 0; nh < NH; ++nh)
                        acc[m][nh] = mfma16(W2L ? aq[s & 1][m] : A2[W2L ? 0 : m][W2L ? 0 : s], bq[s & 1][nh], s == 0 ? bias2[m] : acc[m][nh]);
                __builtin_amdgcn_sched_barrier(0);
            }
#pragma unroll
            for (int nh = 0; nh < NH; ++nh) {
                const int nn = N0 + nh, rr = nn >> 1, xb = nn & 1;
                float v[MT][4];
#pragma unroll
                for (int m = 0; m < MT; ++m) {
                    const rword_t qv = *(const rword_t*)(xs + raddr + (rr * RW + xb * 16) * PSB + ((m * 8) / PIECE) * PIECE);
                    const unsigned lo = qv[((m * 8) % PIECE) / 4], hi = qv[((m * 8) % PIECE) / 4 + 1];
                    v[m][0] = mul_then_add(acc[m][nh][0], osc[m].x, bf_lo(lo)); v[m][1] = mul_then_add(acc[m][nh][1], osc[m].y, bf_hi(lo));
                    v[m][2] = mul_then_add(acc[m][nh][2], osc[m].z, bf_lo(hi)); v[m][3] = mul_then_add(acc[m][nh][3], osc[m].w, bf_hi(hi));
                }
                const bool ok = full || ((rr < ylim) && (xb * 16 < xlim));
#pragma unroll
                for (int q = 0; q < NP; ++q) {
                    int vo = o2 + ooff[rr][q] + xb * 16 * PSB;
                    vo = ok ? vo : OOR;
                    if constexpr (PIECE == 16) {
                        const int m = q * 2;
                        const rword_t d = {pack_bf2(v[m][0], v[m][1]), pack_bf2(v[m][2], v[m][3]), pack_bf2(v[m + 1][0], v[m + 1][1]), pack_bf2(v[m + 1][2], v[m + 1][3])};
                        __builtin_amdgcn_raw_buffer_store_b128(d, ro, vo, 0, 0);
                    } else {
                        const rword_t d = {pack_bf2(v[q][0], v[q][1]), pack_bf2(v[q][2], v[q][3])};
                        __builtin_amdgcn_raw_buffer_store_b64(d, ro, vo, 0, 0);
                    }
                }
            }
        }
        if (++ty == P.nty) {
            ty = 0;
            if (++tx == P.ntx) { tx = 0; ++t; if (i + 1 < n) { load_osc(t); pin_osc(); } }
        }
    }
}

int c3p_segment(int h, int w, int th, int wgs_model) {
    const int ntx = (w + 31) / 32, nty = (h + th - 1) / th;
    const int cand[6] = {8, 6, 4, 3, 2, 1}, Ts[5] = {12, 16, 20, 36, 52};
    double best = 1e30;
    int bestS = 1;
    for (int k = 0; k < 6; ++k) {
        const int S = cand[k] < nty ? cand[k] : nty;
        const int nseg = (nty + S - 1) / S;
        double cost = 0.0;
        for (int j = 0; j < 5; ++j) {
            const long ntiles = (long)ntx * nty * Ts[j];
            long g = 256L * wgs_model;
            if (g > (ntiles + 7) / 8) g = (ntiles + 7) / 8;
            if (g < 1) g = 1;
            const long nsg = (long)nseg * ntx * Ts[j], qs = (nsg + g - 1) / g;
            cost += (1.0 + 0.25 / S) * (double)(qs * S) * (double)g / (double)ntiles;
        }
        if (cost < best - 1e-9) { best = cost; bestS = S; }
    }
    return bestS;
}

struct C3PPlan { int ntx, nty, S, nseg, nsg, qs, grid, pool_rows; };

C3PPlan c3p_plan(int T, int h, int w, int th, int ncu, int wgs, int S) {
    C3PPlan p;
    p.ntx = (w + 31) / 32; p.nty = (h + th - 1) / th;
    const long ntiles = (long)p.ntx * p.nty * T;
    long g = (long)ncu * wgs;
    if (g > (ntiles + 7) / 8) g = (ntiles + 7) / 8;
    if (g < 1) g = 1;
    p.S = S < p.nty ? S : p.nty;
    p.nseg = (p.nty + p.S - 1) / p.S;
    const long nsg = (long)p.nseg * p.ntx * T;
    p.nsg = (int)nsg;
    p.qs = (int)((nsg + g - 1) / g);
    const int chunks = (p.nsg + p.qs - 1) / p.qs;
    p.grid = (chunks + 7) / 8 * 8;
    p.pool_rows = 4 * p.ntx * p.nseg;
    return p;
}

template <int MT, int CS, int TH, int D, int MODE, bool RL>
int launch_conv3p_mode(const C3P& K, const C3PPlan& pl, hipStream_t st) {
    constexpr int NPB = CS / 8, NDMA = ((TH + 2) * 34 * NPB + 63) / 64, KS = (9 * CS + 31) / 32, RDMA = RL ? (TH * 32 * NPB) / 64 : 0;
    C3P P = K;
    P.ntx = pl.ntx; P.nty = pl.nty; P.S = pl.S; P.nseg = pl.nseg; P.nsg = pl.nsg; P.qs = pl.qs; P.pool_rows = pl.pool_rows;
    const size_t lds = (size_t)(D + 1) * (NDMA + RDMA) * 1024 + (MT * KS > 16 ? MT * KS * 1024 : 0);
    if (lds > 160 * 1024) return SN_EINVAL;
    if (lds > 64 * 1024 && hipFuncSetAttribute((const void*)conv3p_kernel<MT, CS, TH, D, MODE, RL>, hipFuncAttributeMaxDynamicSharedMemorySize, (int)lds) != hipSuccess)
        return SN_ELAUNCH;
    hipLaunchKernelGGL((conv3p_kernel<MT, CS, TH, D, MODE, RL>), dim3(pl.grid), dim3(320), lds, st, P);
    return sn_check_launch();
}

template <int MT, int CS, int TH, int D, int D2, bool RL2>
int launch_conv3p(const C3P& K, const C3PPlan& pl, int mode, hipStream_t st) {
    switch (mode) {
        case 0: return launch_conv3p_mode<MT, CS, TH, D, 0, false>(K, pl, st);
        case 1: return launch_conv3p_mode<MT, CS, TH, D, 1, false>(K, pl, st);
        case 2: return launch_conv3p_mode<MT, CS, TH, D2, 2, RL2>(K, pl, st);
        case 3: return launch_conv3p_mode<MT, CS, TH, D, 3, false>(K, pl, st);
        default: return SN_EINVAL;
    }
}

template <int MT, int CS, int TH, int D, int WR = 0>
int launch_cabp(const C3P& K, const C3PPlan& pl, hipStream_t st) {
    constexpr int NPB = CS / 8, NDMA = ((TH + 4) * 36 * NPB + 63) / 64, KS = (9 * CS + 31) / 32;
    C3P P = K;
    P.ntx = pl.ntx; P.nty = pl.nty; P.S = pl.S; P.nseg = pl.nseg; P.nsg = pl.nsg; P.qs = pl.qs; P.pool_rows = 0;
    const size_t lds = (size_t)(D + 1) * NDMA * 1024 + ((TH + 2) * 34 * CS * 2 + 15) / 16 * 16 + ((WR & 1) ? 0 : MT * KS * 1024) + ((WR & 2) ? 0 : MT * KS * 1024);
    if (lds > 160 * 1024) return SN_EINVAL;
    if (lds > 64 * 1024 && hipFuncSetAttribute((const void*)cabp_kernel<MT, CS, TH, D, WR>, hipFuncAttributeMaxDynamicSharedMemorySize, (int)lds) != hipSuccess)
        return SN_ELAUNCH;
    hipLaunchKernelGGL((cabp_kernel<MT, CS, TH, D, WR>), dim3(pl.grid), dim3(320), lds, st, P);
    return sn_check_launch();
}

int c3p_mode(const sn_conv_desc* d, bool want_pool = false) {
    if (d->res2) return -1;
    const bool pool = d->pool != nullptr || want_pool;
    if (d->act == 0 && !pool && !d->oscale && !d->res) return 0;
    if (d->act == 1 && d->prelu >= 0.f && d->prelu <= 1.f && pool && !d->oscale && !d->res) return 1;
    if (d->act == 0 && !pool && d->oscale && d->res) return 2;
    return -1;
}

}

int sn_conv3p_key(const sn_conv_desc* d, bool want_pool) {
    if (!(d->k == 3 && d->stride == 1 && d->pad == 1 && d->in_mode == 0 && d->out_mode == 0 && d->n_in == 1 && d->cs_in == d->cs_out &&
          d->ks == (9 * d->cs_in + 31) / 32 && d->h_in == d->h_out && d->w_in == d->w_out) || c3p_mode(d, want_pool) < 0) return 0;
    if ((size_t)d->h_out * d->w_out * d->cs_out * 2 >= 0x7fffffffull) return 0;
    const int key = d->mt * 1000 + d->cs_in;
    if (key == 1016 && c3p_mode(d, want_pool) == 2 && !(d->flags & 256)) return 0;
    return (key == 1016 || key == 2024 || key == 3040 || key == 3048 || key == 4064) ? key : 0;
}

static int c3p_ncu() {
    int dev = 0, ncu = 0;
    if (hipGetDevice(&dev) != hipSuccess || hipDeviceGetAttribute(&ncu, hipDeviceAttributeMultiprocessorCount, dev) != hipSuccess || ncu < 1) {
        (void)hipGetLastError();
        return 0;
    }
    return ncu;
}
static bool c3p_rl(const sn_conv_desc* d, int key, int mode) { return mode == 2 && (key == 1016 || key == 2024) && !(d->flags & 512); }
static int c3p_wgs_default(int key) { return key == 1016 ? 3 : key == 2024 ? 2 : 1; }
static int c3p_wgs(const sn_conv_desc* d, int key, int mode) {
    const int o = (d->flags >> 4) & 15;
    if (o) return o;
    if (key == 1016) return c3p_rl(d, key, mode) ? 2 : 3;
    return key == 2024 ? 2 : 1;
}

int sn_conv3p_pool_rows(const sn_conv_desc* d) {
    const int key = sn_conv3p_key(d, true), ncu = key ? c3p_ncu() : 0;
    if (!key || !ncu) return 0;
    return c3p_plan(d->T, d->h_out, d->w_out, 8, ncu, c3p_wgs(d, key, 1), c3p_segment(d->h_out, d->w_out, 8, c3p_wgs_default(key))).pool_rows;
}

int sn_conv3p_route(const sn_conv_desc* d, int lines_len, int ncu, int* plan8) {
    const int key = sn_conv3p_key(d, false);
    if (!key) return SN_EINVAL;
    if (ncu == 0) ncu = c3p_ncu();
    if (ncu < 1) return SN_EINVAL;
    const int mode = lines_len > 0 ? 3 : c3p_mode(d);
    if (mode < 0 || (lines_len > 0 && c3p_mode(d) != 1)) return SN_EINVAL;
    const int mt = key / 1000, cs = key % 1000, depth = (d->flags >> 10) & 3;
    bool rl = c3p_rl(d, key, mode);
    int D = 2;
    if (key == 1016 && (depth == 1 || depth == 2)) { D = depth + 2; rl = false; }
    else if (key == 2024 && rl) D = 1;
    else if (key == 4064) D = 1;
    const int npb = cs / 8, ndma = (10 * 34 * npb + 63) / 64, ks = (9 * cs + 31) / 32, rdma = rl ? (8 * 32 * npb) / 64 : 0;
    const size_t lds = (size_t)(D + 1) * (ndma + rdma) * 1024 + (mt * ks > 16 ? mt * ks * 1024 : 0);
    if (lds > 160 * 1024) return SN_EINVAL;
    if (plan8) {
        const C3PPlan pl = c3p_plan(d->T, d->h_out, d->w_out, 8, ncu, c3p_wgs(d, key, mode), c3p_segment(d->h_out, d->w_out, 8, c3p_wgs_default(key)));
        const int v[8] = {pl.ntx, pl.nty, pl.S, pl.nseg, pl.nsg, pl.qs, pl.grid, pl.pool_rows};
        for (int i = 0; i < 8; ++i) plan8[i] = v[i];
    }
    return SN_CONV_ROUTE(SN_CONV_K_STREAM, mt, cs, D, mode, rl ? 1 : 0);
}

template <int MT, int CS, int D>
int launch_conv3p_rf(const C3P& K, const C3PPlan& pl, int mode, hipStream_t st) {
    return launch_conv3p<MT, CS, 8, D, D, false>(K, pl, mode, st);
}

int sn_conv3p_launch(const sn_conv_desc* d, int lines_len, int route, const int* plan8, void* stream) {
    if ((route >> 24) != SN_CONV_K_STREAM || !plan8) return SN_EINVAL;
    C3P K;
    K.in = (const bf16_t*)d->in[0]; K.res = (const bf16_t*)d->res; K.out = (bf16_t*)d->out;
    K.wfrag = (const uint4*)d->wfrag; K.bias = d->bias; K.oscale = d->oscale; K.oscale_stride = d->oscale_stride;
    K.pool = d->pool; K.pool_rows = 0; K.act = d->act; K.prelu = d->prelu;
    K.T = d->T; K.h = d->h_out; K.w = d->w_out; K.lines_len = lines_len; K.dbg = (d->flags >> 12) & 7;
    const C3PPlan pl = {plan8[0], plan8[1], plan8[2], plan8[3], plan8[4], plan8[5], plan8[6], plan8[7]};
    hipStream_t st = (hipStream_t)stream;
    const int mt = (route >> 20) & 15, cs = (route >> 12) & 255, D = (route >> 8) & 15, mode = (route >> 4) & 15;
    const bool rl = route & 1;
    switch (mt * 1000 + cs) {
        case 1016:
            if (rl) return launch_conv3p_mode<1, 16, 8, 2, 2, true>(K, pl, st);
            return D == 3 ? launch_conv3p_rf<1, 16, 3>(K, pl, mode, st) : (D == 4 ? launch_conv3p_rf<1, 16, 4>(K, pl, mode, st)
                                                                                  : launch_conv3p_rf<1, 16, 2>(K, pl, mode, st));
        case 2024: return rl ? launch_conv3p_mode<2, 24, 8, 1, 2, true>(K, pl, st) : launch_conv3p_rf<2, 24, 2>(K, pl, mode, st);
        case 3040: return launch_conv3p_rf<3, 40, 2>(K, pl, mode, st);
        case 3048: return launch_conv3p_rf<3, 48, 2>(K, pl, mode, st);
        case 4064: return launch_conv3p_rf<4, 64, 1>(K, pl, mode, st);
        default: return SN_EINVAL;
    }
}

int sn_cabp_launch(const sn_conv_desc* a, const sn_conv_desc* b, void* stream) {
    const int key = a->mt * 1000 + a->cs_in, ncu = c3p_ncu();
    if (!ncu || !(key == 1016 || key == 2024) || a->act != 1 || !(a->prelu >= 0.f && a->prelu <= 1.f) || !b->oscale || b->res2) return SN_EINVAL;
    if ((size_t)a->h_out * a->w_out * a->cs_out * 2 >= 0x7fffffffull) return SN_EINVAL;
    C3P K;
    K.in = (const bf16_t*)a->in[0]; K.res = nullptr; K.out = (bf16_t*)b->out;
    K.wfrag = (const uint4*)a->wfrag; K.bias = a->bias; K.w2 = (const uint4*)b->wfrag; K.b2 = b->bias;
    K.oscale = b->oscale; K.oscale_stride = b->oscale_stride; K.pool = nullptr; K.pool_rows = 0; K.act = 1; K.prelu = a->prelu;
    K.T = a->T; K.h = a->h_out; K.w = a->w_out; K.lines_len = 0; K.dbg = 0;
    const int o = (a->flags >> 4) & 15;
    const bool shallow = ((a->flags >> 10) & 3) == 3;
    const C3PPlan pl = c3p_plan(a->T, a->h_out, a->w_out, 8, ncu, o ? o : (key == 1016 ? (shallow ? 3 : 2) : 1), c3p_segment(a->h_out, a->w_out, 8, c3p_wgs_default(key)));
    hipStream_t st = (hipStream_t)stream;
    if (shallow) return key == 1016 ? launch_cabp<1, 16, 8, 1>(K, pl, st) : launch_cabp<2, 24, 8, 1>(K, pl, st);
    if (key == 1016 && !((b->flags >> 12) & 1)) return launch_cabp<1, 16, 8, 2, 2>(K, pl, st);
    return key == 1016 ? launch_cabp<1, 16, 8, 2>(K, pl, st) : launch_cabp<2, 24, 8, 2>(K, pl, st);
}
```

shift-net_amd/shiftnet_amd/engine.py:

```python
from __future__ import annotations

import contextlib
import ctypes as C
import os
from typing import Dict, List, NamedTuple, Optional, Sequence, Tuple

import torch

from . import lib as L
from . import prep
from .network import Act, Network, _dtype_code
from .plan import Plan, host_f32_copy
from .schedule import stream_plan, wavefront_order
from .spec import UNIT_NAMES, Variant


class Route(NamedTuple):
    fused: bool
    fold: bool
    k4: bool
    mstencil: bool
    g1_store: bool


class Engine(Network):

    def __init__(self, plan: Plan, dtype: torch.dtype = torch.bfloat16) -> None:
        super().__init__(plan, dtype, graph_auto=True)
        self._tickets = None
        self._old_tickets: List[torch.Tensor] = []
        self._bad = None
        self.fallbacks = 0
        if self.phase1 not in ("auto", "r", "0"):
            raise ValueError(f"SN_PHASE1={self.phase1!r}: expected auto, r (fused kernel) or 0 (two-kernel bf16 chain)")
        if self.k4_fuse not in ("0", "1"):
            raise ValueError(f"SN_K4_FUSE={self.k4_fuse!r}: expected 1 (CAB2's phase 2 inside CAB1's phase 1, four launches per unit) or 0 (five launches)")
        if self.cab_fused not in ("0", "p", "p16", "8", "16", "s8", "s16"):
            raise ValueError(f"SN_CAB_FUSED={self.cab_fused!r}: expected 0 (two launches), p / p16 (streaming form) or 8 / 16 / s8 / s16 (tile form)")
        bad = getattr(plan, "p1r_not_finite", None)
        if bad is not None and self.phase1 != "0":
            msg = (f"shiftnet_amd: {bad}: an fp16 operand of the fused phase-1 kernel is not finite for this checkpoint (body.0 rows small against the "
                   "second 1x1, which the kernel takes times 16 in fp16)")
            if self.phase1 == "r":
                raise ValueError(msg + ".  SN_PHASE1=r was asked for explicitly; SN_PHASE1=auto starts the module on the two-kernel chain, float32 has no fp16 operands.")
            import warnings
            warnings.warn(msg + ": this module runs phase 1 as the two-kernel chain (SN_PHASE1=0), whose second 1x1 is bf16.")
            self.phase1 = "0"

    act_dtype = torch.bfloat16

    conv_tiles = os.environ.get("SN_CONV_TILES", "0") == "1"
    conv_stream_all = os.environ.get("SN_CONV_STREAM_ALL", "0") == "1"
    conv_res_regs = os.environ.get("SN_CONV_RES_REGS", "0") == "1"
    conv_dbg = int(os.environ.get("SN_CONV_DBG", "0"))
    conv_depth = int(os.environ.get("SN_CONV_DEPTH", "0"))
    conv_wgs = int(os.environ.get("SN_CONV_WGS", "0"))
    conv_s2_small = os.environ.get("SN_CONV_S2_SMALL", "0") == "1"

    def conv(self, name: str, ins: Sequence[Act], *, stride: int = 1, pad: Optional[int] = None, prelu: Optional[float] = None,
             res: Optional[Act] = None, out_mode: int = 0, pool: bool = False, in_mode: int = 0, oscale: Optional[torch.Tensor] = None,
             nchw_out: Optional[torch.Tensor] = None, nchw_sc: Optional[torch.Tensor] = None, res2: Optional[Act] = None,
             remap: Optional[Tuple[int, int, int]] = None):
        p = self.P.convs[name]
        k, cout = int(p["k"]), int(p["cout"])
        T, hs, ws, cs_in = ins[0].dims
        if remap is not None:
            T = T // remap[1] * remap[0]
        assert cs_in == p["cs_in"] and len(ins) == p["n_in"], (name, cs_in, p["cs_in"])
        h_in, w_in = (2 * hs, 2 * ws) if in_mode == 1 else (hs, ws)
        if pad is None:
            pad = k // 2
        h_out = (h_in + 2 * pad - k) // stride + 1
        w_out = (w_in + 2 * pad - k) // stride + 1
        d = L.ConvDesc()
        for i in range(3):
            d.inp[i] = ins[i].t.data_ptr() if i < len(ins) else None
        d.n_in, d.cs_in, d.T, d.h_in, d.w_in, d.in_mode = len(ins), cs_in, T, h_in, w_in, in_mode
        d.k, d.stride, d.pad, d.h_out, d.w_out = k, stride, pad, h_out, w_out
        d.wfrag, d.mt, d.ks = p["wfrag"].data_ptr(), int(p["mt"]), int(p["ks"])
        d.bias = p["bias"].data_ptr() if p["bias"] is not None else None
        d.act, d.prelu = (1, prelu) if prelu is not None else (0, 0.0)
        pool_buf = None
        out_act: Optional[Act] = None
        if out_mode == 2:
            assert nchw_out is not None and nchw_sc is not None
            d.out, d.sc, d.cs_out = nchw_out.data_ptr(), nchw_sc.data_ptr(), 8
            d.c_out, d.nchw_dtype, d.sc_dtype = cout, _dtype_code(nchw_out.dtype), _dtype_code(nchw_sc.dtype)
        else:
            c_log = cout // 4 if out_mode == 1 else cout
            cs_out = prep.ceil8(c_log)
            o = self._new(T, 2 * h_out, 2 * w_out, cs_out) if out_mode == 1 else self._new(T, h_out, w_out, cs_out)
            out_act = Act(o, c_log)
            d.out, d.cs_out, d.c_out = o.data_ptr(), cs_out, cout
        d.out_mode = out_mode
        d.flags = (L.SN_CONV_TILE_KERNEL | L.conv_flags(s2_small=self.conv_s2_small) if self.conv_tiles else
                   L.conv_flags(self.conv_wgs, self.conv_stream_all, self.conv_res_regs, self.conv_depth, self.conv_dbg, self.conv_s2_small))
        if res is not None:
            assert out_mode == 0 and res.dims == out_act.dims
            d.res = res.t.data_ptr()
        if res2 is not None:
            assert out_mode == 0 and res2.dims == out_act.dims
            d.res2 = res2.t.data_ptr()
        if oscale is not None:
            d.oscale, d.oscale_stride = oscale.data_ptr(), oscale.shape[1]
        if remap is not None:
            d.clip_n, d.clip_T, d.clip_lo = remap
        if pool:
            nblk = self.lib.sn_conv_pool_blocks(C.byref(d))
            pool_buf = torch.empty((T, nblk, 16 * d.mt), dtype=torch.float32, device=self.dev)
            d.pool = pool_buf.data_ptr()
        self._meta = ("conv", T, h_out, w_out, len(ins) * cs_in, int(d.cs_out), k, stride, in_mode, out_mode)
        self._call("sn_conv2d", f"sn_conv2d[{name}]", C.byref(d), self._stream())
        if pool:
            return out_act, pool_buf, h_out * w_out
        return out_act

    k0_mfma = os.environ.get("SN_K0_MFMA", "1") != "0"
    g1_store = os.environ.get("SN_G1_STORE", "1") != "0"
    fold_se = True
    phase1 = os.environ.get("SN_PHASE1", "auto")
    k4_fuse = os.environ.get("SN_K4_FUSE", "1")
    range_guard = os.environ.get("SN_RANGE_GUARD", "1") != "0"
    range_guard_async = os.environ.get("SN_RANGE_GUARD", "1") == "async"

    def cab(self, pre: str, x: Act, extra: Optional[Act] = None) -> Act:
        p = self.P.cas[pre + "CA"]
        T, h, w, cs = x.dims
        slope = self.P.scalar(pre + "body.1.weight")
        if self.cab_fused in ("8", "16", "s8", "s16") or (self.cab_fused[0] == "p" and extra is None and not self.conv_tiles and
                                                          (self.cab_fused == "p" or (cs == 16 and T * h * w >= self.CAB_FUSED_MIN_PX))):
            out = self._cab_fused(pre, x, extra, slope)
            if out is not None:
                return out
        scratch = torch.empty((self.lib.sn_cab_ca_scratch_floats(T),), dtype=torch.float32, device=self.dev)
        mid, pool, _ = self.conv(pre + "body.0", [x], prelu=slope, pool=True)
        _, nblk, cpad = pool.shape
        ca = torch.empty((T, cpad), dtype=torch.float32, device=self.dev)
        self._call("sn_cab_ca", f"sn_cab_ca[{pre}]", pool.data_ptr(), nblk, cpad, mid.t.data_ptr(), cs, p["c"], p["cr"], h, w,
                   p["w2"].data_ptr(), p["wa"].data_ptr(), p["wb"].data_ptr(), scratch.data_ptr(), ca.data_ptr(), T, self._stream())
        return self.conv(pre + "body.2", [mid], res=x, oscale=ca, res2=extra)

    cab_fused = os.environ.get("SN_CAB_FUSED", "p16")
    CAB_FUSED_MIN_PX = 4 << 20

    def _conv_desc(self, name: str, x: Act, *, prelu: Optional[float] = None) -> L.ConvDesc:
        p = self.P.convs[name]
        T, h, w, cs = x.dims
        assert cs == p["cs_in"] and p["n_in"] == 1 and int(p["k"]) == 3
        d = L.ConvDesc()
        d.inp[0] = x.t.data_ptr()
        d.n_in, d.cs_in, d.T, d.h_in, d.w_in, d.in_mode = 1, cs, T, h, w, 0
        d.k, d.stride, d.pad, d.h_out, d.w_out = 3, 1, 1, h, w
        d.wfrag, d.mt, d.ks = p["wfrag"].data_ptr(), int(p["mt"]), int(p["ks"])
        d.bias = p["bias"].data_ptr() if p["bias"] is not None else None
        d.act, d.prelu = (1, prelu) if prelu is not None else (0, 0.0)
        d.cs_out, d.c_out, d.out_mode = prep.ceil8(int(p["cout"])), int(p["cout"]), 0
        d.flags = L.SN_CONV_TILE_KERNEL
        return d

    def _cab_fused(self, pre: str, x: Act, extra: Optional[Act], slope: float) -> Optional[Act]:
        lib = self.lib
        T, h, w, cs = x.dims
        if h < 2 or w < 2:
            return None
        if self.cab_fused[0] == "p" and not 0.0 <= slope <= 1.0:
            return None
        d1 = self._conv_desc(pre + "body.0", x, prelu=slope)
        d2 = self._conv_desc(pre + "body.2", x)
        if self.cab_fused[0] in "sp" and not self.conv_tiles:
            d1.flags = L.conv_flags(wgs=self.conv_wgs, depth=self.conv_depth, dbg=0 if self.cab_fused[0] == "p" else self.conv_dbg)
            if self.cab_fused[0] == "p":
                d2.flags = L.conv_flags(dbg=self.conv_dbg & 1)
        if d1.cs_out != cs or d2.cs_out != cs or not lib.sn_cab_fused_supported(C.byref(d1), C.byref(d2)):
            return None
        p = self.P.cas[pre + "CA"]
        ll = max(h, w)
        lines = torch.empty((T, 4, ll, cs), dtype=self.act_dtype, device=self.dev)
        nblk = lib.sn_conv_pool_blocks(C.byref(d1))
        pool = torch.empty((T, nblk, 16 * d1.mt), dtype=torch.float32, device=self.dev)
        scratch = torch.empty((lib.sn_cab_ca_scratch_floats(T),), dtype=torch.float32, device=self.dev)
        ca = torch.empty((T, 16 * d1.mt), dtype=torch.float32, device=self.dev)
        out = self._new(T, h, w, cs)
        d1.out, d1.pool = lines.data_ptr(), pool.data_ptr()
        d2.out, d2.res, d2.oscale, d2.oscale_stride = out.data_ptr(), x.t.data_ptr(), ca.data_ptr(), ca.shape[1]
        if extra is not None:
            assert extra.dims == x.dims
            d2.res2 = extra.t.data_ptr()
        rows = 0 if self.cab_fused[0] == "p" else 16 if self.cab_fused.endswith("16") else 8
        st = self._stream()
        self._meta = ("cabf", T, h, w, cs, 1)
        self._call("sn_cab_stats", f"sn_cab_stats[{pre}]", C.byref(d1), ll, st)
        self._meta = ()
        self._call("sn_cab_ca_lines", f"sn_cab_ca[{pre}]", pool.data_ptr(), nblk, 16 * d1.mt, lines.data_ptr(), ll, cs, p["c"], p["cr"], h, w,
                   p["w2"].data_ptr(), p["wa"].data_ptr(), p["wb"].data_ptr(), scratch.data_ptr(), ca.data_ptr(), T, st)
        self._meta = ("cabf", T, h, w, cs, 3 if extra is not None else 2)
        self._call("sn_cab_fused", f"sn_cab_fused[{pre}]", C.byref(d1), C.byref(d2), rows, st)
        return Act(out, x.c)

    def temporal_roll(self, x: Act, reverse: bool) -> Act:
        T, h, w, cs = x.dims
        assert cs == x.c, "Shift_CAB widths (24, 80) are stored unpadded"
        y = self._new(T, h, w, cs)
        mode = 2 if reverse else 1
        self._meta = ("roll", T, h, w, cs)
        for wrap, halo, t0, nt in self._split_pieces(x, mode, False):
            s = self._unit_src(x, mode, wrap=wrap, halo=halo, t0=t0, nt=nt)
            self._call("sn_temporal_roll", "sn_temporal_roll", C.byref(s), y.data_ptr(), self._stream())
        return Act(y, x.c)

    def _guard_ptr(self) -> Optional[int]:
        if not self.range_guard:
            return None
        if self._bad is None:
            self._bad = torch.zeros((1,), dtype=torch.int32, device=self.dev)
        return self._bad.data_ptr()

    def _fold_ok(self, T: int) -> bool:
        return self.fold_se and (self._clip or T) <= self.MAX_TICKETS

    def _ticket_ptr(self, T: int) -> int:
        if self._tickets is None or self._tickets.numel() < T:
            if self._tickets is not None:
                self._old_tickets.append(self._tickets)
            self._tickets = torch.zeros((max(self.MAX_TICKETS, T),), dtype=torch.int32, device=self.dev)
        return self._tickets.data_ptr()

    def _fused_phase1(self, T: int) -> bool:
        if self.phase1 == "0":
            return False
        return not (self.V.denoise and not self._fold_ok(T))

    def k4_fused(self, T: int, c: int) -> bool:
        return (self.k4_fuse == "1" and self._fused_phase1(T) and self._fold_ok(T) and c == 64 and not self.V.denoise and self.split is None
                and not self._clip and self.schedule == "unit")

    def route(self, T: int, c: int) -> Route:
        fused = self._fused_phase1(T)
        return Route(fused, fused and self._fold_ok(T), self.k4_fused(T, c), not self.V.grouped_rep, fused and self.V.denoise and self.g1_store)

    def _k0(self, pre: str, src: L.UnitSrc, B: Dict[str, torch.Tensor], st: int) -> None:
        fn = "sn_gsts_shiftconv_mfma" if self.k0_mfma and self.P.k0_mfma_ok else "sn_gsts_shiftconv"
        self._call(fn, "sn_gsts_shiftconv", C.byref(src), self.P.offs.data_ptr(), self.P.units[pre]["w1"].data_ptr(), B["hwb"].data_ptr(), st)

    def _se_fold(self, name: str, T: int, ca: torch.Tensor):
        q = self.P.cas[name]
        return C.byref(L.SeFold(q["wa"].data_ptr(), q["wb"].data_ptr(), q["c"], q["cr"], self._ticket_ptr(T), ca.data_ptr(), self._guard_ptr()))

    def _phase1(self, pre: str, r: Route, src: L.UnitSrc, f0: int, n: int, B: Dict[str, torch.Tensor], st: int) -> bool:
        V, u = self.V, self.P.units[pre]
        if r.fused:
            fn = "sn_gsts_cab2_phase1" if src.mode else "sn_cab1_phase1"
            def args(g2_ptr, se, opt):
                return (C.byref(src),) + ((B["hwb"].data_ptr(),) if src.mode else ()) + (C.byref(u["p1r"]["desc"]), g2_ptr, B["pool2"].data_ptr(), se, opt, st)
            opt = None
            if V.denoise:
                g1s = B["g1s"].data_ptr() if r.g1_store else None
                self._call(fn, fn + "[g1 sums]", *args(None, self._se_fold(pre + "ca1", src.T, B["ca1"]), C.byref(L.Phase1Opts(None, 1, 0, g1s))))
                opt = C.byref(L.Phase1Opts(B["ca1"].data_ptr(), 0, 0, g1s))
            self._call(fn, fn, *args(B["g2"].data_ptr(), self._se_fold(pre + "ca2", src.T, B["ca2"]) if r.fold else None, opt))
            return r.fold
        g1, g2, pool1, pool2, h, w, c, es = B["g1"], B["g2"], B.get("pool1"), B["pool2"], src.h, src.w, src.C, 2
        self._call("sn_ln_gemm_gate", "sn_ln_gemm_gate", C.byref(src), B["hwb"].data_ptr() if src.mode else None, u["w_ln"].data_ptr(), u["b_ln"].data_ptr(),
                   u["w_dw3_h2"].data_ptr(), g1.data_ptr(), pool1.data_ptr() if pool1 is not None else None, 2 if r.mstencil else 0, st)
        ca1_ptr = self.ca_mlp(pre + "ca1", pool1, h * w, out=B["ca1"], frames=(f0, n), guard=self._guard_ptr()).data_ptr() + f0 * c * 4 if V.denoise else None
        k3 = "sn_dw5m_gemm_gate" if r.mstencil else "sn_grp5_gemm_gate"
        self._call(k3, k3, g1.data_ptr() + g1.stride(0) * es * f0, ca1_ptr, u["w_toep5" if r.mstencil else "w_grp"].data_ptr(), u["w_gate"].data_ptr(),
                   g2.data_ptr() + g2.stride(0) * es * f0, pool2.data_ptr() + f0 * pool2.stride(0) * 4, n, h, w, c, st)
        return False

    def _phase2_args(self, pre: str, src: L.UnitSrc, B: Dict[str, torch.Tensor]) -> Tuple:
        u = self.P.units[pre]
        return C.byref(src), B["g2"].data_ptr(), B["ca2"].data_ptr(), u["w_out"].data_ptr(), u["b_out"].data_ptr() if u["b_out"] is not None else None, B["y"].data_ptr()

    def _phase2(self, pre: str, src: L.UnitSrc, B: Dict[str, torch.Tensor], st: int) -> None:
        fn = "sn_gsts_cab2_phase2" if src.mode else "sn_cab1_phase2"
        self._call(fn, fn, *self._phase2_args(pre, src, B), st)

    def _cab2_phase2_cab1_phase1(self, pre2: str, src2: L.UnitSrc, B2: Dict[str, torch.Tensor], meta2: Tuple, pre1: str, B1: Dict[str, torch.Tensor], st: int) -> None:
        fn = "sn_cab2_phase2_cab1_phase1"
        self._call(fn, fn, *self._phase2_args(pre2, src2, B2), C.byref(self.P.units[pre1]["p1r"]["desc"]), B1["g2"].data_ptr(), B1["pool2"].data_ptr(),
                   self._se_fold(pre1 + "ca2", src2.T, B1["ca2"]), None, st)
        if self.prof is not None:
            _, label, meta, e0, e1 = self.prof.pop()
            self.prof += [("sn_gsts_cab2_phase2", "sn_gsts_cab2_phase2 [in sn_cab1_phase1]", meta2, e0, e0), ("sn_cab1_phase1", label, meta, e0, e1)]

    def naf(self, pre: str, x: Act, mode: int, *, frames: Optional[Tuple[int, int]] = None, bufs: Optional[Dict[str, torch.Tensor]] = None) -> Act:
        T, h, w, c = x.dims
        r = self.route(T, c)
        self._meta = ("naf", frames[1] if frames is not None else T, h, w, c, mode, T)
        B = bufs if bufs is not None else self.naf_buffers(T, h, w, c, mode)
        assert frames is None or self.split is None
        pieces = ([(self._wrap_flag(mode, self.V.wrap) if mode else 0, None, frames[0], frames[1])] if frames is not None
                  else self._split_pieces(x, mode, self.V.wrap) if mode else [(0, None, 0, 0)])
        for wrap, halo, t0, nt in pieces:
            st = self._stream()
            src = self._unit_src(x, mode, wrap=wrap, halo=halo, t0=t0, nt=nt)
            f0, n = (t0, nt) if nt else (0, T)
            if mode:
                self._k0(pre, src, B, st)
            if not self._phase1(pre, r, src, f0, n, B, st):
                self.ca_mlp(pre + "ca2", B["pool2"], h * w, out=B["ca2"], frames=(f0, n), guard=self._guard_ptr())
            self._phase2(pre, src, B, st)
        return Act(B["y"], c)

    def naf_buffers(self, T: int, h: int, w: int, c: int, mode: int) -> Dict[str, torch.Tensor]:
        lib, V, r = self.lib, self.V, self.route(T, c)
        B: Dict[str, torch.Tensor] = {}
        if mode:
            B["hwb"] = self._new(T, h, w, c // 2)
        B["g2"] = self._new(T, h, w, c)
        B["y"] = self._new(T, h, w, c)
        if r.fused:
            nb2 = lib.sn_phase1_pool_blocks(T, h, w)
            if nb2 < 1:
                raise L.ShiftNetLibError(f"sn_phase1_pool_blocks failed with code {nb2}")
            if r.g1_store:
                nbytes = C.c_longlong(0)
                L.check(lib.sn_phase1_g1_store_bytes(T, h, w, c, C.byref(nbytes)), "sn_phase1_g1_store_bytes")
                B["g1s"] = torch.empty((nbytes.value,), dtype=torch.uint8, device=self.dev)
        else:
            B["g1"] = (torch.empty((T, h, c, lib.sn_planar_pitch(w)), dtype=torch.bfloat16, device=self.dev) if r.mstencil else self._new(T, h, w, c))
            nb2 = lib.sn_dw5m_blocks(h, w) if r.mstencil else lib.sn_grp5_blocks(h, w)
            if V.denoise:
                B["pool1"] = torch.empty((T, lib.sn_lngate_blocks(h, w), c), dtype=torch.float32, device=self.dev)
        if V.denoise:
            B["ca1"] = torch.empty((T, c), dtype=torch.float32, device=self.dev)
        B["pool2"] = torch.empty((T, nb2, c), dtype=torch.float32, device=self.dev)
        B["ca2"] = torch.empty((T, c), dtype=torch.float32, device=self.dev)
        return B

    def gsts_unit(self, pre: str, x: Act, reverse: bool) -> Act:
        mode, (T, h, w, c) = 2 if reverse else 1, x.dims
        r = self.route(T, c)
        if not r.k4:
            return super().gsts_unit(pre, x, reverse)
        B2, B1 = self.naf_buffers(T, h, w, c, mode), self.naf_buffers(T, h, w, c, 0)
        src2, src1, st = self._unit_src(x, mode), self._unit_src(Act(B2["y"], c), 0, wrap=0), self._stream()
        self._meta = meta2 = ("naf", T, h, w, c, mode, T)
        self._k0(pre + "0.", src2, B2, st)
        self._phase1(pre + "0.", r, src2, 0, T, B2, st)
        self._meta = ("naf", T, h, w, c, 0, T)
        self._cab2_phase2_cab1_phase1(pre + "0.", src2, B2, meta2, pre + "1.", B1, st)
        self._phase2(pre + "1.", src1, B1, st)
        return Act(B1["y"], c)

    schedule = os.environ.get("SN_SCHEDULE", "unit")
    frame_group = int(os.environ.get("SN_FRAME_GROUP", "4"))
    stream_groups = int(os.environ.get("SN_STREAM_GROUPS", "2"))
    STREAMS_MIN_PXF = 400_000

    def _shift_chain(self, pres: Sequence[str], x: Act) -> Act:
        T = x.dims[0]
        if self.schedule not in ("unit", "frame", "streams") or self.frame_group < 1 or self.stream_groups < 1:
            raise ValueError(f"SN_SCHEDULE={self.schedule!r} / SN_FRAME_GROUP={self.frame_group} / SN_STREAM_GROUPS={self.stream_groups}: "
                             "expected unit, frame or streams, and groups of >= 1 frames")
        if self.schedule == "streams" and self.split is None and not self._clip and not torch.cuda.is_current_stream_capturing():
            ng = min(self.stream_groups, T // 2)
            if ng >= 2 and (T // ng) * x.dims[1] * x.dims[2] >= self.STREAMS_MIN_PXF:
                return self._shift_chain_streams(pres, x, ng)
        if self.schedule != "frame" or self.split is not None or self._clip or T <= self.frame_group:
            return super()._shift_chain(pres, x)
        _, h, w, c = x.dims
        units = [(f"{pre}{UNIT_NAMES[i]}.", i % 2 == 1) for pre in pres for i in range(self.V.units)]
        G = self.frame_group
        groups = [(t0, min(G, T - t0)) for t0 in range(0, T, G)]
        bufs = [(self.naf_buffers(T, h, w, c, 2 if rev else 1), self.naf_buffers(T, h, w, c, 0)) for _, rev in units]
        ins = [x] + [Act(b1["y"], c) for _, b1 in bufs]
        for u, j in wavefront_order([rev for _, rev in units], T, G, self.V.wrap):
            pre, rev = units[u]
            y2 = self.naf(pre + "0.", ins[u], 2 if rev else 1, frames=groups[j], bufs=bufs[u][0])
            self.naf(pre + "1.", y2, 0, frames=groups[j], bufs=bufs[u][1])
        return ins[-1]

    STREAM_RING = 3

    def _shift_chain_streams(self, pres: Sequence[str], x: Act, ng: int) -> Act:
        T, h, w, c = x.dims
        units = [(f"{pre}{UNIT_NAMES[i]}.", i % 2 == 1) for pre in pres for i in range(self.V.units)]
        R = min(self.STREAM_RING, max(len(units), 2))
        groups, plan = stream_plan([rev for _, rev in units], T, ng, self.V.wrap, R)
        if getattr(self, "_gstreams", None) is None or len(self._gstreams) < ng:
            self._gstreams = [torch.cuda.Stream(self.dev) for _ in range(ng)]
        streams = self._gstreams[:ng]
        main = torch.cuda.current_stream(self.dev)
        sets = [(self.naf_buffers(T, h, w, c, 1), self.naf_buffers(T, h, w, c, 0)) for _ in range(R)]
        if self.route(T, c).fold:
            self._ticket_ptr(T)
        self._guard_ptr()
        ready = main.record_event()
        done: List[List[Optional[torch.cuda.Event]]] = [[None] * ng for _ in units]
        cab2: List[List[Optional[torch.cuda.Event]]] = [[None] * ng for _ in units]
        cur = x
        for u, (pre, rev) in enumerate(units):
            b2, b1 = sets[u % R]
            for g, fr in enumerate(groups):
                raw, war = plan[u][g]
                with torch.cuda.stream(streams[g]):
                    s = streams[g]
                    if u == 0:
                        s.wait_event(ready)
                    for uu, gg in raw:
                        s.wait_event(done[uu][gg])
                    for uu, gg in war:
                        s.wait_event(cab2[uu][gg])
                    y2 = self.naf(pre + "0.", cur, 2 if rev else 1, frames=fr, bufs=b2)
                    cab2[u][g] = s.record_event()
                    self.naf(pre + "1.", y2, 0, frames=fr, bufs=b1)
                    done[u][g] = s.record_event()
            cur = Act(b1["y"], c)
        for g in range(ng):
            main.wait_event(done[-1][g])
        return cur

    skip_up_lowres = os.environ.get("SN_SKIPUP_LOWRES", "1") != "0"

    def skip_up(self, name: str, x: Act, y: Act) -> Act:
        if not self.skip_up_lowres:
            return super().skip_up(name, x, y)
        lo = self.conv(name, [x])
        T, hs, ws, cs = lo.dims
        assert y.dims == (T, 2 * hs, 2 * ws, cs), (y.dims, lo.dims)
        out = self._new(T, 2 * hs, 2 * ws, cs)
        self._meta = ("up2add", T, hs, ws, cs)
        self._call("sn_upsample2_add", f"sn_upsample2_add[{name}]", lo.t.data_ptr(), y.t.data_ptr(), out.data_ptr(), T, hs, ws, cs, self._stream())
        return Act(out, lo.c)

    def _ingest(self, x: torch.Tensor, noise_map: Optional[torch.Tensor]) -> Act:
        T, cin, H, W = x.shape
        nm_ptr = None
        if self.V.denoise:
            noise_map = noise_map.to(x.dtype).expand(T, 1, H, W).contiguous()
            nm_ptr = noise_map.data_ptr()
        x8 = self._new(T, H, W, 8)
        self._call("sn_ingest", "sn_ingest", x.data_ptr(), _dtype_code(x.dtype), nm_ptr, x8.data_ptr(), T, cin, H, W, self._stream())
        return Act(x8, self.V.in_ch)

    def _checked(self, first, rerun, frames: int) -> torch.Tensor:
        if self.range_guard_async:
            self.check_range_guard()
        out = first()
        if self._scope is not None:
            self._scope.frames = max(self._scope.frames, frames)
        elif self.range_guard_async:
            self._post_guard_copy()
        elif self._guard_tripped():
            out = self._recover(rerun, out, frames)
        return out

    _scope = None

    @contextlib.contextmanager
    def guard_scope(self):
        sc = Engine.GuardScope()
        outer, self._scope = self._scope, sc
        try:
            yield sc
        finally:
            self._scope = outer
            if outer is None and not self.range_guard_async:
                sc.tripped = self._guard_tripped()
                if sc.tripped:
                    self._recover(None, None, sc.frames)
            elif outer is not None:
                outer.frames = max(outer.frames, sc.frames)
            else:
                self._post_guard_copy()

    def _post_guard_copy(self) -> None:
        if self._bad is None or torch.cuda.is_current_stream_capturing():
            return
        if getattr(self, "_bad_host", None) is None:
            self._bad_host = torch.zeros((1,), dtype=torch.int32).pin_memory()
            self._bad_event = torch.cuda.Event()
        self._bad_host.copy_(self._bad, non_blocking=True)
        self._bad.zero_()
        self._bad_event.record()
        self._bad_pending = True

    def check_range_guard(self) -> bool:
        if not getattr(self, "_bad_pending", False):
            return False
        self._bad_event.synchronize()
        self._bad_pending = False
        v = int(self._bad_host.item())
        if self.split is not None:
            v = self.split.any_rank(v)
        if v:
            self._recover(None, None, 1)
        return bool(v)

    def _guard_tripped(self) -> bool:
        if self._bad is None or torch.cuda.is_current_stream_capturing():
            return False
        v = int(self._bad.item())
        if self.split is not None:
            v = self.split.any_rank(v)
        if v:
            self._bad.zero_()
        return bool(v)

    def _recover(self, rerun, out, T: int = 1):
        import warnings
        if self._fused_phase1(T) and self.phase1 == "r":
            warnings.warn(f"shiftnet_amd: {self.V.name}: a channel sum of the GSTS path is not finite -- an activation left the fp16 range of the fused "
                          "phase-1 kernel (`a`, g1, r).  SN_PHASE1=r was asked for explicitly, so the module stays on it: the result of this window is "
                          "not reliable (SN_PHASE1=auto would have moved to the two-kernel chain).")
            return out
        if self._fused_phase1(T) and self.phase1 != "0":
            warnings.warn(f"shiftnet_amd: {self.V.name}: a channel sum of the GSTS path is not finite -- an activation left the fp16 range of the fused "
                          "phase-1 kernel (`a`, g1, r).  This module now runs phase 1 as the two-kernel chain with g1 in bf16 (SN_PHASE1=0)"
                          + (" and the window is recomputed." if rerun is not None else "; the results since the previous check (a guard_scope, or the "
                             "window already handed out under SN_RANGE_GUARD=async) are NOT reliable: run them again."))
            self.phase1 = "0"
            self.fallbacks += 1
            for v in self._graphs.values():
                if isinstance(v, tuple):
                    v[0].reset()
            self._graphs.clear()
            if rerun is None:
                return out
            out = rerun()
            if not self._guard_tripped():
                return out
        warnings.warn(f"shiftnet_amd: {self.V.name}: non-finite channel sums on the bf16 chain as well (its `a` is fp16): the result of this window is "
                      "not reliable -- run the module in float32 (net.float(): the fp32 engine has no half-precision intermediates).")
        return out

    MAX_TICKETS = 4096


def make_engine(V: Variant, sd: Dict[str, torch.Tensor], device: torch.device, dtype: torch.dtype):
    if dtype == torch.float32:
        from .engine32 import Engine32, Plan32
        return Engine32(Plan32(V, sd, device))
    return Engine(Plan(V, sd, device), dtype)
```

shift-net_amd/shiftnet_amd/lib.py:

```python
from __future__ import annotations

import ctypes as C
import os
from typing import Optional

_HERE = os.path.dirname(os.path.abspath(__file__))
LIB_PATH = os.path.join(os.path.dirname(_HERE), "lib", "libshiftnet_hip.so")

SN_F32, SN_F16, SN_BF16 = 0, 1, 2

ABI_VERSION = 20

SYMBOLS = [
    "sn_abi_version", "sn_selftest_mfma", "sn_ingest", "sn_conv2d", "sn_conv_pool_blocks", "sn_conv2d_route","sn_upsample2_add", "sn_ca_mlp",
    "sn_cab_ca", "sn_cab_ca_scratch_floats", "sn_cab_fused_supported", "sn_cab_stats", "sn_cab_ca_lines", "sn_cab_fused", "sn_planar_pitch", "sn_nhwc_to_planar", "sn_dw5m_blocks",
    "sn_dw5m_gemm_gate", "sn_gsts_gather", "sn_temporal_roll", "sn_gsts_shiftconv", "sn_gsts_shiftconv_mfma", "sn_gsts_shiftconv_mfma_plan", "sn_gsts_shiftconv_mfma_plan_opt", "sn_gsts_shiftconv_mfma_opt", "sn_gsts_cab2_phase2", "sn_cab1_phase2",
    "sn_ingest_u8", "sn_egress_blocks", "sn_egress_u8", "sn_ssim_blocks", "sn_ssim_u8",
    "sn_ingest_yuv", "sn_egress_yuv", "sn_yuv_thumb", "sn_yuv_noise_hist",
    "sn_ingest_yuv_rect", "sn_egress_yuv_rect", "sn_yuv_noise_hist_rect", "sn_yuv_rowcol_sums", "sn_egress_yuv_dither",
    "sn_yuv_noise_hist_bands", "sn_noise_map_level", "sn_egress_yuv_mix", "sn_yuv_noise_hist_pairs", "sn_yuv_noise_hist_pairs_bands",
    "sn_yuv_diff_stats", "sn_yuv_diff_stats_mv", "sn_yuv_block_motion", "sn_yuv_noise_hist_pairs_mv", "sn_yuv_noise_hist_pairs_bands_mv",
    "sn_tile_accumulate", "sn_geo_transform", "sn_geo_accumulate", "sn_time_crossfade", "sn_yuv_niqe_sums", "sn_yuv_ssim_sums", "sn_yuv_degrade", "sn_yuv_blur", "sn_yuv_grain",
    "sn_yuv_code_hist", "sn_yuv_apply_lut",
    "sn32_conv2d", "sn32_conv2d_route", "sn32_gsts_gather", "sn32_layernorm", "sn32_gate", "sn32_gate_sum", "sn32_chan_sum", "sn32_scale_residual", "sn32_ingest", "sn32_cab_ca", "sn32_dw_gate", "sn32_conv1x1_gate2", "sn32_gsts_shiftconv", "sn32_conv_csum_tiles",
    "sn_ln_gemm_gate", "sn_lngate_blocks", "sn_grp5_gemm_gate", "sn_grp5_blocks", "sn_gsts_cab2_phase1", "sn_cab1_phase1", "sn_phase1_pool_blocks", "sn_phase1_g1_store_bytes", "sn_p1r_plan", "sn_p1r_strip_begin",
    "sn_cab2_phase2_cab1_phase1", "sn_cab2_phase2_cab1_phase1_supported",
]


class Phase1Weights(C.Structure):
    _fields_ = [("wfrag1", C.c_void_p), ("w3", C.c_void_p), ("wgrp", C.c_void_p), ("wfrag2", C.c_void_p)]


class SeFold(C.Structure):
    _fields_ = [("wa", C.c_void_p), ("wb", C.c_void_p), ("c", C.c_int), ("cr", C.c_int), ("ticket", C.c_void_p), ("ca", C.c_void_p), ("bad", C.c_void_p)]


class Phase1Opts(C.Structure):
    _fields_ = [("g1_scale", C.c_void_p), ("g1_sums", C.c_int), ("team", C.c_int), ("g1_store", C.c_void_p)]


def cab_phase1(lib, src: "UnitSrc", hw_ptr, wt: "Phase1Weights", g2_ptr, pool_ptr, stream, se: "SeFold" = None, opt: "Phase1Opts" = None) -> int:
    sep = C.byref(se) if se is not None else None
    op = C.byref(opt) if opt is not None else None
    if src.mode:
        return lib.sn_gsts_cab2_phase1(C.byref(src), hw_ptr, C.byref(wt), g2_ptr, pool_ptr, sep, op, stream)
    return lib.sn_cab1_phase1(C.byref(src), C.byref(wt), g2_ptr, pool_ptr, sep, op, stream)


class ConvDesc(C.Structure):
    _fields_ = [
        ("inp", C.c_void_p * 3), ("n_in", C.c_int), ("cs_in", C.c_int),
        ("T", C.c_int), ("h_in", C.c_int), ("w_in", C.c_int), ("in_mode", C.c_int),
        ("k", C.c_int), ("stride", C.c_int), ("pad", C.c_int), ("h_out", C.c_int), ("w_out", C.c_int),
        ("wfrag", C.c_void_p), ("mt", C.c_int), ("ks", C.c_int), ("bias", C.c_void_p),
        ("act", C.c_int), ("prelu", C.c_float), ("res", C.c_void_p), ("out", C.c_void_p),
        ("cs_out", C.c_int), ("out_mode", C.c_int), ("c_out", C.c_int), ("nchw_dtype", C.c_int),
        ("sc", C.c_void_p), ("sc_dtype", C.c_int), ("pool", C.c_void_p), ("oscale", C.c_void_p), ("oscale_stride", C.c_int), ("res2", C.c_void_p),
        ("flags", C.c_int), ("clip_n", C.c_int), ("clip_T", C.c_int), ("clip_lo", C.c_int),
    ]


SN_CONV_TILE_KERNEL = 1


def conv_flags(wgs: int = 0, stream_all: bool = False, res_regs: bool = False, depth: int = 0, dbg: int = 0, s2_small: bool = False) -> int:
    if not (0 <= wgs < 16 and 0 <= depth < 4 and 0 <= dbg < 8):
        raise ValueError(f"sn_conv_desc.flags: wgs={wgs} (0..15), depth={depth} (0..3) or dbg={dbg} (0..7) does not fit its field")
    return (wgs << 4) | (bool(stream_all) << 8) | (bool(res_regs) << 9) | (depth << 10) | (dbg << 12) | (bool(s2_small) << 15)


SN_CONV_K_GENERIC, SN_CONV_K_FAST, SN_CONV_K_STATS, SN_CONV_K_STREAM = 1, 2, 3, 4
CONV_KERNEL_NAMES = {SN_CONV_K_GENERIC: "conv_mfma", SN_CONV_K_FAST: "conv3_fast", SN_CONV_K_STATS: "conv3_fast_stats", SN_CONV_K_STREAM: "conv3p"}
CONV_PLAN_FIELDS = ("ntx", "nty", "S", "nseg", "nsg", "qs", "grid", "pool_rows")


def conv_route(kernel: int, mt: int, a: int, d: int = 0, mode: int = 0, rl: int = 0) -> int:
    return (kernel << 24) | (mt << 20) | (a << 12) | (d << 8) | (mode << 4) | rl


def conv_route_name(r: int) -> str:
    if r < 0:
        return f"EINVAL({r})"
    k, mt, a, d, mode, rl = r >> 24, (r >> 20) & 15, (r >> 12) & 255, (r >> 8) & 15, (r >> 4) & 15, r & 15
    name = CONV_KERNEL_NAMES.get(k, str(k))
    if k == SN_CONV_K_GENERIC:
        return f"{name}<{mt},{a},{4 * a}>"
    if k == SN_CONV_K_STREAM:
        return f"{name}<{mt},{a},D{d},MODE{mode},RL{rl}>"
    return f"{name}<{mt},{a}>"


class Conv32Desc(C.Structure):
    _fields_ = [
        ("inp", C.c_void_p * 3), ("c_in", C.c_int * 3), ("cs_in", C.c_int * 3), ("n_in", C.c_int),
        ("T", C.c_int), ("h_in", C.c_int), ("w_in", C.c_int), ("in_mode", C.c_int),
        ("k", C.c_int), ("stride", C.c_int), ("pad", C.c_int), ("groups", C.c_int),
        ("h_out", C.c_int), ("w_out", C.c_int), ("c_out", C.c_int),
        ("w", C.c_void_p), ("bias", C.c_void_p), ("act", C.c_int), ("prelu", C.c_float),
        ("oscale", C.c_void_p), ("oscale_stride", C.c_int), ("res", C.c_void_p), ("cs_res", C.c_int),
        ("out", C.c_void_p), ("cs_out", C.c_int), ("out_mode", C.c_int), ("nchw_dtype", C.c_int), ("sc", C.c_void_p),
        ("wsplit", C.c_void_p), ("iscale", C.c_void_p), ("iscale_stride", C.c_int), ("rscale", C.c_void_p), ("rscale_stride", C.c_int),
        ("ln_w", C.c_void_p), ("ln_b", C.c_void_p), ("csum", C.c_void_p), ("csum_cpad", C.c_int),
        ("clip_n", C.c_int), ("clip_T", C.c_int), ("clip_lo", C.c_int),
    ]


class UnitSrc(C.Structure):
    _fields_ = [("x", C.c_void_p), ("T", C.c_int), ("h", C.c_int), ("w", C.c_int), ("C", C.c_int),
                ("mode", C.c_int), ("wrap", C.c_int), ("halo", C.c_void_p), ("t0", C.c_int), ("nt", C.c_int),
                ("clip", C.c_int)]


SN_K0_TILE, SN_K0_WALK = 1, 2
K0_PLAN_FIELDS = ("form", "S", "nseg", "wgs", "per_x", "per_tile", "ntx", "nty", "nt", "grid")


class K0Opts(C.Structure):
    _fields_ = [("form", C.c_int), ("seg", C.c_int), ("wgs", C.c_int)]


def k0_plan(lib, src: "UnitSrc", ncu: int, opt: "K0Opts" = None) -> dict:
    plan = (C.c_int * len(K0_PLAN_FIELDS))()
    if opt is None:
        check(lib.sn_gsts_shiftconv_mfma_plan(C.byref(src), ncu, plan), "sn_gsts_shiftconv_mfma_plan")
    else:
        check(lib.sn_gsts_shiftconv_mfma_plan_opt(C.byref(src), ncu, C.byref(opt), plan), "sn_gsts_shiftconv_mfma_plan_opt")
    return dict(zip(K0_PLAN_FIELDS, plan))


SN_YUV_444, SN_YUV_420_CENTER, SN_YUV_420_LEFT = 0, 1, 2
SN_YUV_BT601, SN_YUV_BT709 = 0, 1
SN_YUV_LIMITED, SN_YUV_FULL = 0, 1


class YuvFmt(C.Structure):
    _fields_ = [("bits", C.c_int), ("chroma", C.c_int), ("matrix", C.c_int), ("range", C.c_int)]

    def frame_bytes(self, H: int, W: int) -> int:
        c = H * W if self.chroma == SN_YUV_444 else ((H + 1) // 2) * ((W + 1) // 2)
        return (H * W + 2 * c) * (1 if self.bits == 8 else 2)


class YuvRect(C.Structure):
    _fields_ = [("x0", C.c_int), ("y0", C.c_int), ("w", C.c_int), ("h", C.c_int)]


SN_DITHER_NONE, SN_DITHER_TPDF = 0, 1
SN_BLUR_MAX_TAPS = 15
SN_NLF_BANDS = 16
SN_DIFF_STATS = 16
SN_DIFF_STATS_MV = 8
SN_NIQE_BLOCK, SN_NIQE_MAPS, SN_NIQE_SUMS = 96, 5, 5
SN_SSIM_TILE = 32


class YuvDither(C.Structure):
    _fields_ = [("mode", C.c_int), ("seed", C.c_uint32), ("t0", C.c_int)]


SN_MIX_AMOUNT, SN_MIX_REMOVED = 0, 1
SN_GEO_FLIP_X, SN_GEO_FLIP_Y, SN_GEO_TRANSPOSE, SN_GEO_REVERSE_T = 1, 2, 4, 8


class YuvMix(C.Structure):
    _fields_ = [("mode", C.c_int), ("ay", C.c_float), ("ac", C.c_float)]


class YuvDegradeNoise(C.Structure):
    _fields_ = [("seed", C.c_uint32), ("t0", C.c_int), ("knots", C.c_float * SN_NLF_BANDS)]


class YuvBlurWindow(C.Structure):
    _fields_ = [("n", C.c_int), ("c0", C.c_int), ("lo", C.c_int), ("hi", C.c_int)]


class YuvGrainNoise(C.Structure):
    _fields_ = [("seed", C.c_uint32), ("t0", C.c_int), ("knots", C.c_float * SN_NLF_BANDS), ("chroma", C.c_float), ("taps", C.c_float * 3)]


class ShiftNetLibError(RuntimeError):
    pass


_lib: Optional[C.CDLL] = None


def load() -> C.CDLL:
    global _lib
    if _lib is not None:
        return _lib
    import torch
    if not os.path.exists(LIB_PATH):
        raise ShiftNetLibError(
            f"{LIB_PATH} not found: build it with `python shift-net_amd/build.py` (hipcc, gfx950). "
            "There is no CPU fallback for the Shift-Net HIP path.")
    lib = C.CDLL(LIB_PATH)
    missing = [s for s in SYMBOLS if not hasattr(lib, s)]
    if missing:
        raise ShiftNetLibError(f"{LIB_PATH} lacks symbols {missing}")
    vp, ci, cf = C.c_void_p, C.c_int, C.c_float
    lib.sn_abi_version.restype = ci
    lib.sn_selftest_mfma.argtypes = [vp, vp, vp, vp]
    lib.sn_ingest.argtypes = [vp, ci, vp, vp, ci, ci, ci, ci, vp]
    lib.sn_conv2d.argtypes = [C.POINTER(ConvDesc), vp]
    lib.sn_conv_pool_blocks.argtypes = [C.POINTER(ConvDesc)]
    lib.sn_conv2d_route.argtypes = [C.POINTER(ConvDesc), ci, ci, C.POINTER(ci * 8)]
    lib.sn_upsample2_add.argtypes = [vp, vp, vp, ci, ci, ci, ci, vp]
    lib.sn_ca_mlp.argtypes = [vp, ci, ci, ci, ci, cf, vp, vp, vp, ci, vp, vp]
    lib.sn_planar_pitch.argtypes = [ci]
    lib.sn_nhwc_to_planar.argtypes = [vp, vp, ci, ci, ci, ci, vp]
    lib.sn_dw5m_blocks.argtypes = [ci, ci]
    lib.sn_dw5m_gemm_gate.argtypes = [vp, vp, vp, vp, vp, vp, ci, ci, ci, ci, vp]
    lib.sn_cab_ca.argtypes = [vp, ci, ci, vp, ci, ci, ci, ci, ci, vp, vp, vp, vp, vp, ci, vp]
    lib.sn_cab_ca_scratch_floats.argtypes = [ci]
    lib.sn_cab_fused_supported.argtypes = [C.POINTER(ConvDesc), C.POINTER(ConvDesc)]
    lib.sn_cab_stats.argtypes = [C.POINTER(ConvDesc), ci, vp]
    lib.sn_cab_ca_lines.argtypes = [vp, ci, ci, vp, ci, ci, ci, ci, ci, ci, vp, vp, vp, vp, vp, ci, vp]
    lib.sn_cab_fused.argtypes = [C.POINTER(ConvDesc), C.POINTER(ConvDesc), ci, vp]
    lib.sn32_cab_ca.argtypes = [vp, ci, ci, vp, ci, ci, ci, ci, vp, vp, vp, vp, vp, ci, vp]
    lib.sn_gsts_gather.argtypes = [C.POINTER(UnitSrc), vp, vp, vp]
    lib.sn_temporal_roll.argtypes = [C.POINTER(UnitSrc), vp, vp]
    lib.sn_gsts_shiftconv.argtypes = [C.POINTER(UnitSrc), vp, vp, vp, vp]
    lib.sn_gsts_shiftconv_mfma.argtypes = [C.POINTER(UnitSrc), vp, vp, vp, vp]
    lib.sn_gsts_shiftconv_mfma_plan.argtypes = [C.POINTER(UnitSrc), ci, C.POINTER(ci * len(K0_PLAN_FIELDS))]
    lib.sn_gsts_shiftconv_mfma_plan_opt.argtypes = [C.POINTER(UnitSrc), ci, C.POINTER(K0Opts), C.POINTER(ci * len(K0_PLAN_FIELDS))]
    lib.sn_gsts_shiftconv_mfma_opt.argtypes = [C.POINTER(UnitSrc), vp, vp, vp, C.POINTER(K0Opts), vp]
    lib.sn_ln_gemm_gate.argtypes = [C.POINTER(UnitSrc), vp, vp, vp, vp, vp, vp, ci, vp]
    lib.sn_lngate_blocks.argtypes = [ci, ci]
    lib.sn_grp5_gemm_gate.argtypes = [vp, vp, vp, vp, vp, vp, ci, ci, ci, ci, vp]
    lib.sn_grp5_blocks.argtypes = [ci, ci]
    lib.sn_phase1_pool_blocks.argtypes = [ci, ci, ci]
    lib.sn_phase1_g1_store_bytes.argtypes = [ci, ci, ci, ci, C.POINTER(C.c_longlong)]
    lib.sn_p1r_plan.argtypes = [ci, ci, ci, ci, ci, C.POINTER(ci * 7)]
    lib.sn_p1r_strip_begin.argtypes = [C.POINTER(ci * 7), ci, ci]
    lib.sn_gsts_cab2_phase1.argtypes = [C.POINTER(UnitSrc), vp, C.POINTER(Phase1Weights), vp, vp, C.POINTER(SeFold), C.POINTER(Phase1Opts), vp]
    lib.sn_cab1_phase1.argtypes = [C.POINTER(UnitSrc), C.POINTER(Phase1Weights), vp, vp, C.POINTER(SeFold), C.POINTER(Phase1Opts), vp]
    lib.sn_gsts_cab2_phase2.argtypes = [C.POINTER(UnitSrc), vp, vp, vp, vp, vp, vp]
    lib.sn_cab1_phase2.argtypes = [C.POINTER(UnitSrc), vp, vp, vp, vp, vp, vp]
    lib.sn_cab2_phase2_cab1_phase1_supported.argtypes = [C.POINTER(UnitSrc)]
    lib.sn_cab2_phase2_cab1_phase1.argtypes = [C.POINTER(UnitSrc), vp, vp, vp, vp, vp, C.POINTER(Phase1Weights), vp, vp, C.POINTER(SeFold), C.POINTER(Phase1Opts), vp]
    lib.sn_ingest_u8.argtypes = [vp, vp, ci, ci, ci, ci, vp]
    lib.sn_egress_blocks.argtypes = []
    lib.sn_egress_u8.argtypes = [vp, ci, vp, vp, vp, ci, ci, ci, vp]
    lib.sn_ssim_blocks.argtypes = []
    lib.sn_ssim_u8.argtypes = [vp, ci, vp, vp, vp, ci, ci, ci, vp]
    lib.sn_ingest_yuv.argtypes = [vp, C.POINTER(YuvFmt), vp, ci, ci, ci, ci, ci, ci, vp]
    lib.sn_egress_yuv.argtypes = [vp, ci, C.POINTER(YuvFmt), vp, ci, ci, ci, ci, ci, vp]
    lib.sn_yuv_thumb.argtypes = [vp, C.POINTER(YuvFmt), vp, ci, ci, ci, vp]
    lib.sn_yuv_noise_hist.argtypes = [vp, C.POINTER(YuvFmt), vp, ci, ci, ci, ci, ci, vp]
    lib.sn_ingest_yuv_rect.argtypes = [vp, C.POINTER(YuvFmt), C.POINTER(YuvRect), vp, ci, ci, ci, ci, ci, ci, vp]
    lib.sn_egress_yuv_rect.argtypes = [vp, ci, C.POINTER(YuvFmt), C.POINTER(YuvRect), vp, ci, ci, ci, ci, ci, vp]
    lib.sn_yuv_noise_hist_rect.argtypes = [vp, C.POINTER(YuvFmt), C.POINTER(YuvRect), vp, ci, ci, ci, ci, ci, vp]
    lib.sn_yuv_rowcol_sums.argtypes = [vp, C.POINTER(YuvFmt), vp, vp, ci, ci, ci, vp]
    lib.sn_egress_yuv_dither.argtypes = [vp, ci, C.POINTER(YuvFmt), C.POINTER(YuvRect), C.POINTER(YuvDither), vp, ci, ci, ci, ci, ci, vp]
    lib.sn_egress_yuv_mix.argtypes = [vp, ci, C.POINTER(YuvFmt), C.POINTER(YuvRect), C.POINTER(YuvDither), C.POINTER(YuvMix), vp, vp, ci, ci, ci, ci, ci, vp]
    lib.sn_yuv_noise_hist_bands.argtypes = [vp, C.POINTER(YuvFmt), C.POINTER(YuvRect), vp, ci, ci, ci, ci, ci, vp]
    lib.sn_yuv_noise_hist_pairs.argtypes = [vp, C.POINTER(YuvFmt), C.POINTER(YuvRect), vp, ci, ci, ci, ci, ci, vp]
    lib.sn_yuv_noise_hist_pairs_bands.argtypes = [vp, C.POINTER(YuvFmt), C.POINTER(YuvRect), vp, ci, ci, ci, ci, ci, vp]
    lib.sn_yuv_block_motion.argtypes = [vp, C.POINTER(YuvFmt), C.POINTER(YuvRect), vp, vp, ci, ci, ci, vp]
    lib.sn_yuv_noise_hist_pairs_mv.argtypes = [vp, C.POINTER(YuvFmt), C.POINTER(YuvRect), vp, vp, ci, ci, ci, ci, ci, vp]
    lib.sn_yuv_noise_hist_pairs_bands_mv.argtypes = [vp, C.POINTER(YuvFmt), C.POINTER(YuvRect), vp, vp, ci, ci, ci, ci, ci, vp]
    lib.sn_yuv_diff_stats.argtypes = [vp, vp, C.POINTER(YuvFmt), C.POINTER(YuvRect), ci, vp, ci, ci, ci, vp]
    lib.sn_yuv_diff_stats_mv.argtypes = [vp, vp, C.POINTER(YuvFmt), C.POINTER(YuvRect), vp, vp, ci, ci, ci, vp]
    lib.sn_noise_map_level.argtypes = [vp, C.POINTER(YuvFmt), C.POINTER(YuvRect), C.POINTER(cf * SN_NLF_BANDS), ci, ci, vp, ci, ci, ci, ci, ci, ci, vp]
    lib.sn_tile_accumulate.argtypes = [vp, vp, vp, vp, ci, ci, ci, ci, ci, ci, ci, ci, vp]
    lib.sn_geo_transform.argtypes = [vp, vp, ci, ci, ci, ci, ci, ci, vp]
    lib.sn_geo_accumulate.argtypes = [vp, vp, ci, ci, cf, ci, ci, ci, ci, vp]
    lib.sn_time_crossfade.argtypes = [vp, vp, vp, vp, vp, ci, ci, ci, ci, ci, ci, vp]
    lib.sn_yuv_niqe_sums.argtypes = [vp, C.POINTER(YuvFmt), C.POINTER(YuvRect), vp, vp, ci, ci, ci, vp]
    lib.sn_yuv_ssim_sums.argtypes = [vp, vp, C.POINTER(YuvFmt), C.POINTER(YuvRect), vp, ci, ci, ci, vp]
    lib.sn_yuv_degrade.argtypes = [vp, C.POINTER(YuvFmt), C.POINTER(YuvDegradeNoise), vp, vp, ci, ci, ci, vp]
    lib.sn_yuv_blur.argtypes = [vp, ci, C.POINTER(YuvFmt), C.POINTER(YuvBlurWindow), vp, vp, vp, ci, ci, ci, vp]
    lib.sn_yuv_grain.argtypes = [vp, C.POINTER(YuvFmt), C.POINTER(YuvRect), C.POINTER(YuvGrainNoise), vp, vp, ci, ci, ci, vp]
    lib.sn_yuv_code_hist.argtypes = [vp, C.POINTER(YuvFmt), C.POINTER(YuvRect), vp, ci, ci, ci, vp]
    lib.sn_yuv_apply_lut.argtypes = [vp, C.POINTER(YuvFmt), C.POINTER(YuvRect), vp, vp, ci, ci, ci, vp]
    ll = C.c_longlong
    lib.sn32_conv2d.argtypes = [C.POINTER(Conv32Desc), vp]
    lib.sn32_conv2d_route.argtypes = [C.POINTER(Conv32Desc)]
    lib.sn32_gsts_gather.argtypes = [C.POINTER(UnitSrc), vp, vp, vp, vp]
    lib.sn32_layernorm.argtypes = [vp, ci, ci, vp, vp, vp, ci, ll, vp]
    lib.sn32_gate.argtypes = [vp, ci, ci, vp, ll, vp]
    lib.sn32_gate_sum.argtypes = [vp, ci, ci, ci, vp, ci, ci, ci, vp, vp]
    lib.sn32_dw_gate.argtypes = [vp, ci, vp, ci, ci, vp, ci, ci, ci, ci, vp, vp]
    lib.sn32_conv_csum_tiles.argtypes = [ci, ci]
    lib.sn32_gsts_shiftconv.argtypes = [vp, vp, vp, vp, vp, vp]
    lib.sn32_conv1x1_gate2.argtypes = [vp, ci, ci, vp, ci, ci, vp, ci, ci, vp, vp]
    lib.sn32_chan_sum.argtypes = [vp, ci, ci, ci, ci, ci, ci, vp, vp]
    lib.sn32_scale_residual.argtypes = [vp, vp, vp, ci, vp, ci, ci, ci, vp]
    lib.sn32_ingest.argtypes = [vp, ci, vp, vp, ci, ci, ci, ci, vp]
    for s in SYMBOLS:
        getattr(lib, s).restype = ci
    if lib.sn_abi_version() != ABI_VERSION:
        raise ShiftNetLibError(f"ABI version mismatch: {LIB_PATH} reports {lib.sn_abi_version()}, shiftnet_amd/lib.py expects {ABI_VERSION} "
                               "(stale build: run `python shift-net_amd/build.py`)")
    _lib = lib
    return lib


def check(rc: int, what: str) -> None:
    if rc != 0:
        raise ShiftNetLibError(f"{what} failed with code {rc}")
```

shift-net_amd/shiftnet_amd/network.py:

```python
from __future__ import annotations

import contextlib
import os
from collections import OrderedDict
from dataclasses import dataclass
from typing import Optional, Sequence, Tuple

import torch

from . import lib as L
from .spec import UNIT_NAMES


@dataclass
class Act:
    t: torch.Tensor
    c: int

    @property
    def dims(self) -> Tuple[int, int, int, int]:
        return tuple(self.t.shape)


def _dtype_code(dt: torch.dtype) -> int:
    return {torch.float32: L.SN_F32, torch.float16: L.SN_F16, torch.bfloat16: L.SN_BF16}[dt]


class Network:
    schedule, frame_group, stream_groups = "unit", 4, 2

    def __init__(self, plan, dtype: Optional[torch.dtype] = None, graph_auto: bool = False) -> None:
        self.P = plan
        self.dtype = dtype or self.act_dtype
        self.V = plan.V
        self.lib = L.load()
        self.dev = plan.device
        self.prof: Optional[list] = None
        self._meta: Tuple = ()
        self._unit: Optional[Tuple] = None
        self.split = None
        self._side = None
        self._clip = 0
        g = os.environ.get("SN_GRAPH", "auto")
        self.use_graph = g == "1"
        self.graph_auto = graph_auto and g not in ("0", "1")
        self._graphs: "OrderedDict[Tuple, object]" = OrderedDict()

    def _stream(self) -> int:
        return torch.cuda.current_stream(self.dev).cuda_stream

    def _call(self, fn: str, label: str, *args) -> None:
        f = getattr(self.lib, fn)
        if self.prof is None:
            L.check(f(*args), label)
            return
        e0, e1 = torch.cuda.Event(enable_timing=True), torch.cuda.Event(enable_timing=True)
        e0.record()
        L.check(f(*args), label)
        e1.record()
        meta = self._meta
        if self._unit is not None and not (meta and meta[0] == "naf"):
            meta = tuple(meta) + ("unit",) + self._unit
        self.prof.append((fn, label, meta, e0, e1))

    def _new(self, T: int, h: int, w: int, cs: int) -> torch.Tensor:
        return torch.empty((T, h, w, cs), dtype=self.act_dtype, device=self.dev)

    def ca_mlp(self, name: str, pool: torch.Tensor, npix: int, *, out: Optional[torch.Tensor] = None, frames: Optional[Tuple[int, int]] = None, guard: Optional[int] = None) -> torch.Tensor:
        p = self.P.cas[name]
        T, nblk, cpad = pool.shape
        ca = out if out is not None else torch.empty((T, cpad), dtype=torch.float32, device=self.dev)
        f0, n = frames if frames is not None else (0, T)
        self._call("sn_ca_mlp", f"sn_ca_mlp[{name}]", pool.data_ptr() + f0 * nblk * cpad * 4, nblk, cpad, p["c"], p["cr"], 1.0 / npix, p["wa"].data_ptr(),
                   p["wb"].data_ptr(), ca.data_ptr() + f0 * cpad * 4, n, guard, self._stream())
        return ca

    def _wrap_flag(self, mode: int, circular: bool) -> int:
        if self.split is not None and mode:
            return self.split.wrap_flag(mode, circular)
        return 1 if circular else 0

    def _unit_src(self, x: Act, mode: int, *, wrap: Optional[int] = None, halo: Optional[torch.Tensor] = None, t0: int = 0, nt: int = 0) -> L.UnitSrc:
        T, h, w, cs = x.dims
        assert cs == x.c
        wrap = self._wrap_flag(mode, self.V.wrap) if wrap is None else wrap
        return L.UnitSrc(x.t.data_ptr(), T, h, w, x.c, mode, wrap, halo.data_ptr() if halo is not None else None, t0, nt, self._clip)

    def _split_pieces(self, x: Act, mode: int, circular: bool):
        T = x.dims[0]
        flag = self._wrap_flag(mode, circular)
        if self.split is None:
            yield (flag, None, 0, 0)
            return
        main = torch.cuda.current_stream(self.dev)
        ready = main.record_event()
        recv = flag == 2
        bt = 0 if mode == 1 else T - 1
        if recv and T > 1:
            yield (0, None, 1 if mode == 1 else 0, T - 1)
        if self._side is None:
            self._side = torch.cuda.Stream(self.dev)
        with torch.cuda.stream(self._side):
            self._side.wait_event(ready)
            x.t.record_stream(self._side)
            halo = self.split.exchange(x.t, mode, circular)
        if recv:
            main.wait_stream(self._side)
            halo.record_stream(main)
            yield (2, halo, bt, 1)
        else:
            yield (flag, None, 0, 0)

    def shift_cab(self, pre: str, x: Act, reverse: bool) -> Act:
        return self.cab(pre, self.temporal_roll(x, reverse))

    def gsts_unit(self, pre: str, x: Act, reverse: bool) -> Act:
        return self.naf(pre + "1.", self.naf(pre + "0.", x, 2 if reverse else 1), 0)

    def shift_block(self, pre: str, x: Act) -> Act:
        for i in range(self.V.units):
            x = self.gsts_unit(f"{pre}{UNIT_NAMES[i]}.", x, reverse=(i % 2 == 1))
        return x

    def shift_chain(self, pres: Sequence[str], x: Act) -> Act:
        ev = None
        if self.prof is not None:
            ev = (torch.cuda.Event(enable_timing=True), torch.cuda.Event(enable_timing=True))
            ev[0].record()
        y = self._shift_chain(pres, x)
        if ev is not None:
            ev[1].record()
            self.prof.append(("gsts_chain", "gsts_chain", ("chain",) + tuple(x.dims) + (len(pres) * self.V.units,), ev[0], ev[1]))
        return y

    def _shift_chain(self, pres: Sequence[str], x: Act) -> Act:
        for pre in pres:
            x = self.shift_block(pre, x)
        return x

    def down(self, pre: str, x: Act) -> Act:
        if self.V.denoise:
            return self.conv(pre + "down", [x], stride=2, prelu=self.P.scalar(pre + "down.1.weight"))
        return self.conv(pre + "down", [x], stride=2)

    def skip_up(self, name: str, x: Act, y: Act) -> Act:
        return self.conv(name, [x], in_mode=1, res=y)

    def tfr_unet(self, pre: str, x: Act, extra: Optional[Act] = None) -> Act:
        def seq(nm: str, n: int, t: Act, ex: Optional[Act] = None) -> Act:
            for i in range(n):
                t = self.cab(f"{pre}{nm}.{i}.", t, ex if i == n - 1 else None)
            return t
        enc1 = seq("encoder_level1", 1, x)
        enc2 = seq("encoder_level2", 3, self.down(pre + "down12.", enc1))
        enc3 = seq("encoder_level3", 3, self.down(pre + "down23.", enc2))
        dec3 = seq("decoder_level3", 3, enc3)
        t = self.skip_up(pre + "up32", dec3, self.cab(pre + "skip_attn2.", enc2))
        dec2 = seq("decoder_level2", 3, t)
        t = self.skip_up(pre + "up21", dec2, self.cab(pre + "skip_attn1.", enc1))
        return seq("decoder_level1", 1, t, extra)

    def stage1(self, x: Act) -> Act:
        V, p = self.V, "stage1."
        x = self.cab(p + "concat.", x)
        shortcut = x
        if V.shift_cab:
            x = self.shift_cab(p + "encoder_level0.", x, False)
            x = self.shift_cab(p + "encoder_level0_1.", x, True)
        x = self.conv(p + "down01", [x], stride=2, pad=0, prelu=self.P.scalar(p + "down01.1.weight"))
        if V.topo == "small":
            enc11 = self.shift_chain([p + "encoder_level1.", p + "encoder_level1_1.", p + "encoder_level1_2."], x)
            e = self.down(p + "down12.", enc11)
            e = self.shift_chain([f"{p}{n}." for n in ("encoder_level2", "encoder_level2_1", "encoder_level2_2",
                                                       "decoder_level2", "decoder_level2_1", "decoder_level2_2")], e)
            x = self.skip_up(p + "up21", e, self.cab(p + "skip_attn1.", enc11))
        else:
            if V.shift_cab:
                e = self.shift_cab(p + "encoder_level1.", x, False)
                enc11 = self.shift_cab(p + "encoder_level1_1.", e, True)
            else:
                enc11 = self.cab(p + "encoder_level1_1.", self.cab(p + "encoder_level1.", x))
            e = self.down(p + "down12.", enc11)
            enc22 = self.cab(p + "encoder_level2_1.", self.cab(p + "encoder_level2.", e))
            e = self.down(p + "down23.", enc22)
            enc33 = self.cab(p + "encoder_level3_1.", self.cab(p + "encoder_level3.", e))
            d = self.shift_chain([p + "decoder_level3.", p + "decoder_level3_1."], enc33)
            x = self.skip_up(p + "up32", d, self.cab(p + "skip_attn2.", enc22))
            d = self.shift_chain([p + "decoder_level2.", p + "decoder_level2_1."], x)
            x = self.skip_up(p + "up21", d, self.cab(p + "skip_attn1.", enc11))
        dec11 = self.shift_chain([p + "decoder_level1.", p + "decoder_level1_1.", p + "decoder_level1_2."], x)
        skip = self.cab(p + "skip_conv.", shortcut)
        if V.hr_cat:
            up = self.conv(p + "upsample0", [dec11], out_mode=1)
            out = self.conv(p + "conv_hr0", [up, skip])
        else:
            up = self.conv(p + "upsample0", [dec11], out_mode=1, prelu=self.P.scalar(p + "act.weight"))
            out = self.conv(p + "conv_hr0", [up], res=skip)
        return self.cab(p + "out_conv.", out)

    @torch.no_grad()
    def forward(self, x: torch.Tensor, noise_map: Optional[torch.Tensor], past: int, future: int,
                out_dtype: Optional[torch.dtype] = None, shortcut: Optional[torch.Tensor] = None) -> torch.Tensor:
        with torch.cuda.device(self.dev):
            graphed = self.use_graph or (self.graph_auto and x.shape[0] * x.shape[2] * x.shape[3] <= self.GRAPH_AUTO_PXF)
            eager = (not graphed or self.split is not None or self.prof is not None or out_dtype is not None or shortcut is not None
                     or torch.cuda.is_current_stream_capturing())
            rerun = lambda: self._forward(x, noise_map, past, future, out_dtype, shortcut)
            return self._checked(rerun if eager else lambda: self._forward_graphed(x, noise_map, past, future), rerun, int(x.shape[0]))

    @torch.no_grad()
    def forward_clips(self, x: torch.Tensor, noise_map: Optional[torch.Tensor], past: int, future: int,
                      out_dtype: Optional[torch.dtype] = None, shortcut: Optional[torch.Tensor] = None) -> torch.Tensor:
        if self.split is not None:
            raise ValueError("forward_clips cannot be combined with a temporal split (set_temporal_split)")
        if x.dim() != 5:
            raise ValueError(f"forward_clips expects x:[B,T,C,H,W], got {tuple(x.shape)}")
        B, T, cin, H, W = x.shape
        xf = x.reshape(B * T, cin, H, W)
        nm = noise_map.expand(B, T, 1, H, W).reshape(B * T, 1, H, W) if noise_map is not None else None
        sc = None
        if shortcut is not None:
            assert shortcut.dim() == 5 and tuple(shortcut.shape[:2]) == (B, T), tuple(shortcut.shape)
            sc = shortcut.reshape(B * T, *shortcut.shape[2:])
        n_out = max(T - past - future, 0)
        with torch.cuda.device(self.dev):
            graphed = self.use_graph or (self.graph_auto and B * T * H * W <= self.GRAPH_AUTO_PXF)
            eager = (not graphed or self.prof is not None or out_dtype is not None or shortcut is not None
                     or torch.cuda.is_current_stream_capturing())
            rerun = lambda: self._forward(xf, nm, past, future, out_dtype, sc, clip=T)
            out = self._checked(rerun if eager else lambda: self._forward_graphed(xf, nm, past, future, clip=T), rerun, T)
            return out.reshape(B, n_out, *out.shape[1:])

    def _checked(self, first, rerun, frames: int) -> torch.Tensor:
        return first()

    class GuardScope:
        tripped = False
        frames = 1

    @contextlib.contextmanager
    def guard_scope(self):
        yield Network.GuardScope()

    def _forward_graphed(self, x, noise_map, past, future, clip: int = 0):
        key = (tuple(x.shape), x.dtype, None if noise_map is None else (tuple(noise_map.shape), noise_map.dtype), past, future, clip)

        def run(xx, nn):
            return self._forward(xx, nn, past, future, clip=clip) if clip else self._forward(xx, nn, past, future)
        ent = self._graphs.get(key)
        if ent is None:
            self._graphs[key] = "seen"
            self._evict_graphs()
            return run(x, noise_map)
        self._graphs.move_to_end(key)
        if ent == "eager":
            return run(x, noise_map)
        if ent == "seen":
            try:
                sx = x.clone()
                sn = noise_map.clone() if noise_map is not None else None
                g = torch.cuda.CUDAGraph()
                with torch.cuda.graph(g, capture_error_mode="thread_local"):
                    so = run(sx, sn)
                ent = self._graphs[key] = (g, sx, sn, so)
                self._evict_graphs()
            except Exception as e:
                import warnings
                if torch.cuda.is_current_stream_capturing():
                    try:
                        g.capture_end()
                    except Exception:
                        pass
                warnings.warn(f"shiftnet_amd: hipGraph capture failed ({type(e).__name__}: {e}); running eagerly")
                self._graphs[key] = "eager"
                torch.cuda.synchronize(self.dev)
                return run(x, noise_map)
        g, sx, sn, so = ent
        sx.copy_(x)
        if sn is not None:
            sn.copy_(noise_map)
        g.replay()
        return so.clone()

    GRAPH_AUTO_PXF = 500_000
    GRAPH_SLOTS = 2

    def _evict_graphs(self) -> None:
        live = [k for k, v in self._graphs.items() if isinstance(v, tuple)]
        while len(live) > self.GRAPH_SLOTS:
            k = live.pop(0)
            g = self._graphs.pop(k)[0]
            g.reset()
        while len(self._graphs) > 16:
            k = next(iter(self._graphs))
            v = self._graphs.pop(k)
            if isinstance(v, tuple):
                v[0].reset()

    def _forward(self, x: torch.Tensor, noise_map: Optional[torch.Tensor], past: int, future: int,
                 out_dtype: Optional[torch.dtype] = None, shortcut: Optional[torch.Tensor] = None, clip: int = 0) -> torch.Tensor:
        assert not clip or (self.split is None and x.shape[0] % clip == 0)
        self._clip = clip
        try:
            return self._forward_frames(x, noise_map, past, future, out_dtype, shortcut)
        finally:
            self._clip = 0

    def _forward_frames(self, x: torch.Tensor, noise_map: Optional[torch.Tensor], past: int, future: int,
                        out_dtype: Optional[torch.dtype], shortcut: Optional[torch.Tensor]) -> torch.Tensor:
        V = self.V
        x = x.contiguous()
        T, cin, H, W = x.shape
        div = 8 if V.topo == "plus" else 4
        if H % div or W % div:
            raise ValueError(f"{V.name}: H and W must be multiples of {div} (got {H}x{W})")
        sp = self.split
        Tc = self._clip or T
        B = T // Tc
        lo = past if (sp is None or sp.rank == 0) else 0
        hi = Tc - (future if (sp is None or sp.rank == sp.world - 1) else 0)
        n_out = max(hi - lo, 0)
        out = torch.empty((B * n_out, 3, H, W), dtype=out_dtype or x.dtype, device=x.device)
        if sp is not None:
            sp.validate(n_out)
        if n_out == 0:
            return out
        x0 = self.cab("feat_extract.1.", self.conv("feat_extract.0", [self._ingest(x, noise_map)]))
        t = x0
        for i in range(1, V.n_orb + 1):
            t = self.tfr_unet(f"orb{i}.", t, x0 if (i == V.n_orb and not V.denoise) else None)
        res0 = t
        sam = self.conv("conv_trans", [res0])
        dec = self.stage1(sam)
        feats = sam if V.denoise else res0

        def cut(a: Act) -> Act:
            return Act(a.t[lo:hi], a.c)
        prelu = self.P.scalar("lrelu.weight") if V.denoise else None
        if self._clip:
            y = self.conv("rconcat", [x0, feats, dec], prelu=prelu, remap=(n_out, Tc, lo))
        else:
            y = self.conv("rconcat", [cut(x0), cut(feats), cut(dec)], prelu=prelu)
# ... 12 lines not shown
```

Measured before the change: 165.6 frames/s.

## Fold SkipUpSample bilinear upsample-add into the skip-attention CAB's second conv epilogue

Skip-connection upsampling (low-res conv followed by bilinear 2x upsample plus residual add) is now folded into the epilogue of the skip CAB's final conv. Both the streaming fused CAB kernel and the 3x3 pipelined conv kernel stage a low-res tile into LDS alongside the input halo and blend it per output pixel. This removes the separate full-resolution upsample-add pass and the intermediate full-resolution CAB output write and read. In exchange the kernels use more LDS per buffer, carry extra epilogue ALU work, and add sched barriers, which may reduce occupancy.

Result: no change. 167.9 frames/s, median of 4 (+1.4%).

```diff
diff --git a/include/shiftnet_hip.h b/include/shiftnet_hip.h
--- a/include/shiftnet_hip.h
+++ b/include/shiftnet_hip.h
@@ -69,6 +69,11 @@
 int sn_cab_ca_lines(const float* partial, int nblk, int cpad, const void* lines, int lines_len, int cs, int c, int cr, int h, int w,
                     const float* w2, const float* wa, const float* wb, float* scratch, float* ca, int T, void* stream);
 int sn_cab_fused(const sn_conv_desc* conv1, const sn_conv_desc* conv2, int tile_rows, void* stream);
+
+typedef struct sn_up2_src { const void* lo; int hs; int ws; } sn_up2_src;
+int sn_up2_fold_supported(const sn_conv_desc* conv2, const sn_up2_src* up);
+int sn_conv2d_up2(const sn_conv_desc* conv2, const sn_up2_src* up, void* stream);
+int sn_cab_fused_up2(const sn_conv_desc* conv1, const sn_conv_desc* conv2, const sn_up2_src* up, int tile_rows, void* stream);
 
 int sn32_cab_ca(const float* partial, int nblk, int cpad, const float* mid, int c, int cr, int h, int w,
                 const float* w2, const float* wa, const float* wb, float* scratch, float* ca, int T, void* stream);
diff --git a/shift-net_amd/csrc/sn_cabf.hip b/shift-net_amd/csrc/sn_cabf.hip
--- a/shift-net_amd/csrc/sn_cabf.hip
+++ b/shift-net_amd/csrc/sn_cabf.hip
@@ -1,7 +1,7 @@
 #include "sn_common.h"
 #include "../../include/shiftnet_hip.h"
 
-int sn_cabp_launch(const sn_conv_desc* a, const sn_conv_desc* b, void* stream);
+int sn_cabp_launch(const sn_conv_desc* a, const sn_conv_desc* b, const sn_up2_src* up, void* stream);
 
 namespace {
 
@@ -309,7 +309,7 @@
     if (!key) return SN_EINVAL;
     if (tile_rows == 0) {
         if (!a->in[0] || a->res || a->res2 || a->oscale || b->pool || b->act != 0 || !b->out || b->res != a->in[0] || a->h_in < 2 || a->w_in < 2) return SN_EINVAL;
-        return sn_cabp_launch(a, b, stream);
+        return sn_cabp_launch(a, b, nullptr, stream);
     }
     if (!a->in[0] || a->res || a->res2 || a->oscale || b->pool || b->act != 0 || !b->out || b->res != a->in[0]) return SN_EINVAL;
     if (b->oscale && b->oscale_stride < 16 * b->mt) return SN_EINVAL;
@@ -328,4 +328,12 @@
     }
 }
 
-}
+int sn_cab_fused_up2(const sn_conv_desc* a, const sn_conv_desc* b, const sn_up2_src* up, int tile_rows, void* stream) {
+    sn_clear_error();
+    if (tile_rows != 0 || cabf_key(a, b) != 1016 || !sn_up2_fold_supported(b, up) || !up->lo) return SN_EINVAL;
+    if (!a->in[0] || a->res || a->res2 || a->oscale || b->pool || b->act != 0 || !b->out || b->res != a->in[0] || a->h_in < 2 || a->w_in < 2) return SN_EINVAL;
+    if (b->oscale && b->oscale_stride < 16 * b->mt) return SN_EINVAL;
+    return sn_cabp_launch(a, b, up, stream);
+}
+
+}
diff --git a/shift-net_amd/csrc/sn_conv.hip b/shift-net_amd/csrc/sn_conv.hip
--- a/shift-net_amd/csrc/sn_conv.hip
+++ b/shift-net_amd/csrc/sn_conv.hip
@@ -1,4 +1,5 @@
 #include "sn_common.h"
+#include "sn_up2.h"
 #include "../../include/shiftnet_hip.h"
 
 int sn_conv3p_key(const sn_conv_desc* d, bool want_pool);
@@ -711,9 +712,8 @@
     const int e = (int)blockIdx.x * 256 + (int)threadIdx.x;
     if (e >= w2 * npb) return;
     const int x = e / npb, piece = e - x * npb;
-    float sx = x * 0.5f - 0.25f; if (sx < 0.f) sx = 0.f;
-    const int x0 = (int)sx, x1 = min(x0 + 1, ws - 1);
-    const float lx = sx - x0, hx = 1.f - lx;
+    int x0, x1; float hx, lx;
+    up2_col(x, ws, x0, x1, hx, lx);
     const int ra = max(i - 1, 0), rc = min(i + 1, hs - 1);
     const bf16_t* b = lo + (size_t)t * hs * ws * cs + piece * 8;
     const uint4 qa0 = *(const uint4*)(b + ((size_t)ra * ws + x0) * cs), qa1 = *(const uint4*)(b + ((size_t)ra * ws + x1) * cs);
@@ -723,12 +723,14 @@
     const uint4 r0 = *(const uint4*)(res + o0), r1 = *(const uint4*)(res + o1);
     float a0[8], a1[8], b0[8], b1[8], c0[8], c1[8], f0[8], f1[8], u0[8], u1[8];
     unpack8(qa0, a0); unpack8(qa1, a1); unpack8(qb0, b0); unpack8(qb1, b1); unpack8(qc0, c0); unpack8(qc1, c1); unpack8(r0, f0); unpack8(r1, f1);
-    const float ly0 = i > 0 ? 0.75f : 0.f, hy0 = 1.f - ly0;
+    float hy0, ly0, hy1, ly1;
+    up2_row(i, false, hy0, ly0);
+    up2_row(i, true, hy1, ly1);
 #pragma unroll
     for (int j = 0; j < 8; ++j) {
-        const float va = hx * a0[j] + lx * a1[j], vb = hx * b0[j] + lx * b1[j], vc = hx * c0[j] + lx * c1[j];
-        u0[j] = (hy0 * va + ly0 * vb) + f0[j];
-        u1[j] = (0.75f * vb + 0.25f * vc) + f1[j];
+        const float va = up2_blend_h(hx, lx, a0[j], a1[j]), vb = up2_blend_h(hx, lx, b0[j], b1[j]), vc = up2_blend_h(hx, lx, c0[j], c1[j]);
+        u0[j] = up2_blend_v(hy0, ly0, va, vb, f0[j]);
+        u1[j] = up2_blend_v(hy1, ly1, vb, vc, f1[j]);
     }
     *(uint4*)(out + o0) = pack8(u0);
     *(uint4*)(out + o1) = pack8(u1);
diff --git a/shift-net_amd/csrc/sn_conv3p.hip b/shift-net_amd/csrc/sn_conv3p.hip
--- a/shift-net_amd/csrc/sn_conv3p.hip
+++ b/shift-net_amd/csrc/sn_conv3p.hip
@@ -1,4 +1,5 @@
 #include "sn_common.h"
+#include "sn_up2.h"
 #include "../../include/shiftnet_hip.h"
 
 namespace {
@@ -15,7 +16,34 @@
     int dbg;
     int lines_len;
     int S, nseg, nsg, qs;
+    const bf16_t* lo; int hs, ws;
 };
+
+constexpr int UP2_ROWS = 6, UP2_COLS = 18;
+constexpr int up2_dma(int cs) { return (UP2_ROWS * UP2_COLS * (cs / 8) + 63) / 64; }
+
+template <int CS> __device__ __forceinline__ void up2_item(int k, int lane, int& row, int& col, int& qoff) {
+    constexpr int NPB = CS / 8, NIT = UP2_ROWS * UP2_COLS * NPB;
+    const int i = k * 64 + lane, ic = i < NIT ? i : NIT - 1, px = ic / NPB;
+    qoff = (ic - px * NPB) * 16;
+    row = px / UP2_COLS;
+    col = px - row * UP2_COLS;
+}
+
+template <int MT, int CS> __device__ __forceinline__ void up2_fold(float (&v)[MT][4], const char* lt, float hx, float lx, float wt, float wb) {
+    constexpr int PSB = CS * 2;
+    typedef unsigned w_t __attribute__((ext_vector_type(MT * 2)));
+    const w_t t0 = *(const w_t*)lt, t1 = *(const w_t*)(lt + PSB), b0 = *(const w_t*)(lt + UP2_COLS * PSB), b1 = *(const w_t*)(lt + (UP2_COLS + 1) * PSB);
+#pragma unroll
+    for (int m = 0; m < MT; ++m)
+#pragma unroll
+        for (int e = 0; e < 2; ++e) {
+            const int wi = m * 2 + e;
+            const unsigned pk = pack_bf2(v[m][2 * e], v[m][2 * e + 1]);
+            v[m][2 * e] = up2_value(hx, lx, wt, wb, bf_lo(t0[wi]), bf_lo(t1[wi]), bf_lo(b0[wi]), bf_lo(b1[wi]), bf_lo(pk));
+            v[m][2 * e + 1] = up2_value(hx, lx, wt, wb, bf_hi(t0[wi]), bf_hi(t1[wi]), bf_hi(b0[wi]), bf_hi(b1[wi]), bf_hi(pk));
+        }
+}
 
 __device__ __forceinline__ float max_bare(float a, float b) {
     float r;
@@ -43,15 +71,17 @@
 
 constexpr int c3p_waves(int mt) { return mt == 1 ? 4 : mt == 2 ? 3 : 2; }
 
-template <int MT, int CS, int TH, int D, int MODE, bool RL = false>
+template <int MT, int CS, int TH, int D, int MODE, bool RL = false, bool UP = false>
 __global__ __launch_bounds__(320, c3p_waves(MT)) void conv3p_kernel(const C3P P) {
     extern __shared__ __attribute__((aligned(16))) char smem[];
     constexpr int TW = 32, RH = TH + 2, RW = TW + 2, NPB = CS / 8, PSB = CS * 2;
     constexpr int KTOT = 9 * CS, KS = (KTOT + 31) / 32;
     constexpr int ROWP = RW * NPB, NITEM = RH * ROWP, NDMA = (NITEM + 63) / 64, XBUF = NDMA * 1024;
     static_assert(!RL || MODE == 2, "residual staging belongs to MODE 2");
+    static_assert(!UP || (RL && TH == 8), "the folded SkipUpSample tail: MODE 2 with the residual staged, 8-row tiles");
     constexpr int RDMA = RL ? (TH * TW * NPB) / 64 : 0;
-    constexpr int NBUF = D + 1, BUFSZ = XBUF + RDMA * 1024, NL = NDMA + RDMA;
+    constexpr int LDMA = UP ? up2_dma(CS) : 0, LOFF = XBUF + RDMA * 1024;
+    constexpr int NBUF = D + 1, BUFSZ = LOFF + LDMA * 1024, NL = NDMA + RDMA + LDMA;
     constexpr bool WLDS = MT * KS > 16;
     constexpr int WBYTES = WLDS ? MT * KS * 1024 : 0;
     constexpr int RPW = TH / 4, NTW = RPW * 2;
@@ -98,6 +128,11 @@
                 rvoff[k] = row * rowpitch + rem * 16;
             }
         }
+        int lrow[UP ? LDMA : 1], lcol[UP ? LDMA : 1], lq[UP ? LDMA : 1];
+        if constexpr (UP) {
+#pragma unroll
+            for (int k = 0; k < LDMA; ++k) up2_item<CS>(k, lane, lrow[k], lcol[k], lq[k]);
+        }
         int ft = t, ftx = tx, fty = ty;
         for (int i = -D; i < n; ++i) {
             if (i >= 0) {
@@ -123,6 +158,15 @@
 #pragma unroll
                     for (int k = 0; k < RDMA; ++k)
                         dma16(rr, dst + XBUF + k * 1024, rvoff[k] + o2);
+                }
+                if constexpr (UP) {
+                    const __amdgpu_buffer_rsrc_t rl = frame_rsrc(P.lo + (size_t)ft * P.hs * P.ws * CS, P.hs * P.ws * PSB);
+                    const int lr0 = fty * (TH / 2) - 1, lc0 = ftx * (TW / 2) - 1;
+#pragma unroll
+                    for (int k = 0; k < LDMA; ++k) {
+                        const int sr = min(max(lr0 + lrow[k], 0), P.hs - 1), sc = min(max(lc0 + lcol[k], 0), P.ws - 1);
+                        dma16(rl, dst + LOFF + k * 1024, (sr * P.ws + sc) * PSB + lq[k]);
+                    }
                 }
                 if (++fty == P.nty) { fty = 0; if (++ftx == P.ntx) { ftx = 0; ++ft; } }
             }
@@ -257,6 +301,13 @@
                     v[m][0] = mul_then_add(v[m][0], osc[m].x, bf_lo(lo)); v[m][1] = mul_then_add(v[m][1], osc[m].y, bf_hi(lo));
                     v[m][2] = mul_then_add(v[m][2], osc[m].z, bf_lo(hi)); v[m][3] = mul_then_add(v[m][3], osc[m].w, bf_hi(hi));
                 }
+            }
+            if constexpr (UP) {
+                const int ox0 = tx * TW;
+                int x0, x1; float hx, lx, wt, wb;
+                up2_col(ox0 + xb * 16 + p, P.ws, x0, x1, hx, lx);
+                up2_row(ty * (TH / 2) + wv, rr & 1, wt, wb);
+                up2_fold<MT, CS>(v, xs + LOFF + ((wv + (rr & 1)) * UP2_COLS + (x0 - (ox0 >> 1) + 1)) * PSB + (c0 < CS ? c0 * 2 : 0), hx, lx, wt, wb);
             }
             bool ok = true;
             if (MASKED) ok = (rr < ylim) && (xb * 16 < xlim);
@@ -379,13 +430,15 @@
     }
 }
 
-template <int MT, int CS, int TH, int D, int WR>
+template <int MT, int CS, int TH, int D, int WR, bool UP = false>
 __global__ __launch_bounds__(320, c3p_waves(MT)) void cabp_kernel(const C3P P) {
     extern __shared__ __attribute__((aligned(16))) char smem[];
     constexpr int TW = 32, RH = TH + 4, RW = TW + 4, MH = TH + 2, MW = TW + 2, NPB = CS / 8, PSB = CS * 2;
     constexpr int KTOT = 9 * CS, KS = (KTOT + 31) / 32;
     constexpr int ROWP = RW * NPB, NITEM = RH * ROWP, NDMA = (NITEM + 63) / 64, XBUF = NDMA * 1024;
-    constexpr int NBUF = D + 1, NL = NDMA;
+    static_assert(!UP || TH == 8, "the folded SkipUpSample tail: 8-row tiles");
+    constexpr int LDMA = UP ? up2_dma(CS) : 0, BUFSZ = XBUF + LDMA * 1024;
+    constexpr int NBUF = D + 1, NL = NDMA + LDMA;
     constexpr bool W1L = !(WR & 1), W2L = !(WR & 2);
     constexpr int WSET = MT * KS * 1024, W2OFF = W1L ? WSET : 0, WBYTES = W2OFF + (W2L ? WSET : 0);
     constexpr int NM = MH * MW, NT1 = (NM + 15) / 16, PER1 = (NT1 + 3) / 4;
@@ -429,6 +482,11 @@
             voff[k] = r * rowpitch + j * 16;
             pxk[k] = j / NPB;
         }
+        int lrow[UP ? LDMA : 1], lcol[UP ? LDMA : 1], lq[UP ? LDMA : 1];
+        if constexpr (UP) {
+#pragma unroll
+            for (int k = 0; k < LDMA; ++k) up2_item<CS>(k, lane, lrow[k], lcol[k], lq[k]);
+        }
         int ft = t, ftx = tx, fty = ty;
         for (int i = -D; i < n; ++i) {
             if (i >= 0) {
@@ -441,12 +499,21 @@
                 const int ix0 = ftx * TW - 2;
                 const int o = ((fty * TH - 2) * P.w + ix0) * PSB;
                 const bool edge = ftx == 0 || ix0 + RW > P.w;
-                char* const dst = xbufs + (j % NBUF) * XBUF;
+                char* const dst = xbufs + (j % NBUF) * BUFSZ;
 #pragma unroll
                 for (int k = 0; k < NDMA; ++k) {
                     int vo = voff[k] + o;
                     if (edge) { const int gx = ix0 + pxk[k]; vo = (gx < 0 || gx >= P.w) ? (int)0x80000000 : vo; }
                     dma16(rs, dst + k * 1024, vo);
+                }
+                if constexpr (UP) {
+                    const __amdgpu_buffer_rsrc_t rl = frame_rsrc(P.lo + (size_t)ft * P.hs * P.ws * CS, P.hs * P.ws * PSB);
+                    const int lr0 = fty * (TH / 2) - 1, lc0 = ftx * (TW / 2) - 1;
+#pragma unroll
+                    for (int k = 0; k < LDMA; ++k) {
+                        const int sr = min(max(lr0 + lrow[k], 0), P.hs - 1), sc = min(max(lc0 + lcol[k], 0), P.ws - 1);
+                        dma16(rl, dst + XBUF + k * 1024, (sr * P.ws + sc) * PSB + lq[k]);
+                    }
                 }
                 if (++fty == P.nty) { fty = 0; if (++ftx == P.ntx) { ftx = 0; ++ft; } }
             }
@@ -505,8 +572,10 @@
     const float slope = P.prelu;
     float4 osc[MT];
     auto load_osc = [&](int ft) {
-#pragma unroll
-        for (int m = 0; m < MT; ++m) osc[m] = *(const float4*)(P.oscale + (size_t)ft * P.oscale_stride + c0 + m * 4);
+        int cc = c0;
+        if constexpr (UP) pin(cc);
+#pragma unroll
+        for (int m = 0; m < MT; ++m) osc[m] = *(const float4*)(P.oscale + (size_t)ft * P.oscale_stride + cc + m * 4);
     };
     load_osc(t);
     auto pin_osc = [&]() __attribute__((always_inline)) {
@@ -539,7 +608,7 @@
 
     for (int i = 0; i < n; ++i) {
         __builtin_amdgcn_s_barrier();
-        const char* const xs = xbufs + (i % NBUF) * XBUF;
+        const char* const xs = xbufs + (i % NBUF) * BUFSZ;
         const int oy0 = ty * TH, ox0 = tx * TW;
         const bool inner = oy0 >= 1 && oy0 + TH + 1 <= P.h && ox0 >= 1 && ox0 + TW + 1 <= P.w;
 #pragma unroll
@@ -575,7 +644,9 @@
                 const int i1 = ps * NH1 + nh;
                 bool in = true;
                 if (!inner) {
-                    const int pq = pix1[i1] / PSB, my = pq / RW, mx = pq - my * RW;
+                    int po = pix1[i1];
+                    if constexpr (UP) pin(po);
+                    const int pq = po / PSB, my = pq / RW, mx = pq - my * RW;
                     const int gy = oy0 - 1 + my, gx = ox0 - 1 + mx;
                     in = gy >= 0 && gy < P.h && gx >= 0 && gx < P.w;
                 }
@@ -648,6 +719,12 @@
                     const unsigned lo = qv[((m * 8) % PIECE) / 4], hi = qv[((m * 8) % PIECE) / 4 + 1];
                     v[m][0] = mul_then_add(acc[m][nh][0], osc[m].x, bf_lo(lo)); v[m][1] = mul_then_add(acc[m][nh][1], osc[m].y, bf_hi(lo));
                     v[m][2] = mul_then_add(acc[m][nh][2], osc[m].z, bf_lo(hi)); v[m][3] = mul_then_add(acc[m][nh][3], osc[m].w, bf_hi(hi));
+                }
+                if constexpr (UP) {
+                    int x0, x1; float hx, lx, wt, wb;
+                    up2_col(ox0 + xb * 16 + p, P.ws, x0, x1, hx, lx);
+                    up2_row((oy0 >> 1) + wv, rr & 1, wt, wb);
+                    up2_fold<MT, CS>(v, xs + XBUF + ((wv + (rr & 1)) * UP2_COLS + (x0 - (ox0 >> 1) + 1)) * PSB + (c0 < CS ? c0 * 2 : 0), hx, lx, wt, wb);
                 }
                 const bool ok = full || ((rr < ylim) && (xb * 16 < xlim));
 #pragma unroll
@@ -663,6 +740,7 @@
                         __builtin_amdgcn_raw_buffer_store_b64(d, ro, vo, 0, 0);
                     }
                 }
+                if constexpr (UP) __builtin_amdgcn_sched_barrier(0);
             }
         }
         if (++ty == P.nty) {
@@ -714,16 +792,16 @@
     return p;
 }
 
-template <int MT, int CS, int TH, int D, int MODE, bool RL>
+template <int MT, int CS, int TH, int D, int MODE, bool RL, bool UP = false>
 int launch_conv3p_mode(const C3P& K, const C3PPlan& pl, hipStream_t st) {
-    constexpr int NPB = CS / 8, NDMA = ((TH + 2) * 34 * NPB + 63) / 64, KS = (9 * CS + 31) / 32, RDMA = RL ? (TH * 32 * NPB) / 64 : 0;
+    constexpr int NPB = CS / 8, NDMA = ((TH + 2) * 34 * NPB + 63) / 64, KS = (9 * CS + 31) / 32, RDMA = RL ? (TH * 32 * NPB) / 64 : 0, LDMA = UP ? up2_dma(CS) : 0;
     C3P P = K;
     P.ntx = pl.ntx; P.nty = pl.nty; P.S = pl.S; P.nseg = pl.nseg; P.nsg = pl.nsg; P.qs = pl.qs; P.pool_rows = pl.pool_rows;
-    const size_t lds = (size_t)(D + 1) * (NDMA + RDMA) * 1024 + (MT * KS > 16 ? MT * KS * 1024 : 0);
+    const size_t lds = (size_t)(D + 1) * (NDMA + RDMA + LDMA) * 1024 + (MT * KS > 16 ? MT * KS * 1024 : 0);
     if (lds > 160 * 1024) return SN_EINVAL;
-    if (lds > 64 * 1024 && hipFuncSetAttribute((const void*)conv3p_kernel<MT, CS, TH, D, MODE, RL>, hipFuncAttributeMaxDynamicSharedMemorySize, (int)lds) != hipSuccess)
+    if (lds > 64 * 1024 && hipFuncSetAttribute((const void*)conv3p_kernel<MT, CS, TH, D, MODE, RL, UP>, hipFuncAttributeMaxDynamicSharedMemorySize, (int)lds) != hipSuccess)
         return SN_ELAUNCH;
-    hipLaunchKernelGGL((conv3p_kernel<MT, CS, TH, D, MODE, RL>), dim3(pl.grid), dim3(320), lds, st, P);
+    hipLaunchKernelGGL((conv3p_kernel<MT, CS, TH, D, MODE, RL, UP>), dim3(pl.grid), dim3(320), lds, st, P);
     return sn_check_launch();
 }
 
@@ -738,16 +816,16 @@
     }
 }
 
-template <int MT, int CS, int TH, int D, int WR = 0>
+template <int MT, int CS, int TH, int D, int WR = 0, bool UP = false>
 int launch_cabp(const C3P& K, const C3PPlan& pl, hipStream_t st) {
-    constexpr int NPB = CS / 8, NDMA = ((TH + 4) * 36 * NPB + 63) / 64, KS = (9 * CS + 31) / 32;
+    constexpr int NPB = CS / 8, NDMA = ((TH + 4) * 36 * NPB + 63) / 64, KS = (9 * CS + 31) / 32, LDMA = UP ? up2_dma(CS) : 0;
     C3P P = K;
     P.ntx = pl.ntx; P.nty = pl.nty; P.S = pl.S; P.nseg = pl.nseg; P.nsg = pl.nsg; P.qs = pl.qs; P.pool_rows = 0;
-    const size_t lds = (size_t)(D + 1) * NDMA * 1024 + ((TH + 2) * 34 * CS * 2 + 15) / 16 * 16 + ((WR & 1) ? 0 : MT * KS * 1024) + ((WR & 2) ? 0 : MT * KS * 1024);
+    const size_t lds = (size_t)(D + 1) * (NDMA + LDMA) * 1024 + ((TH + 2) * 34 * CS * 2 + 15) / 16 * 16 + ((WR & 1) ? 0 : MT * KS * 1024) + ((WR & 2) ? 0 : MT * KS * 1024);
     if (lds > 160 * 1024) return SN_EINVAL;
-    if (lds > 64 * 1024 && hipFuncSetAttribute((const void*)cabp_kernel<MT, CS, TH, D, WR>, hipFuncAttributeMaxDynamicSharedMemorySize, (int)lds) != hipSuccess)
+    if (lds > 64 * 1024 && hipFuncSetAttribute((const void*)cabp_kernel<MT, CS, TH, D, WR, UP>, hipFuncAttributeMaxDynamicSharedMemorySize, (int)lds) != hipSuccess)
         return SN_ELAUNCH;
-    hipLaunchKernelGGL((cabp_kernel<MT, CS, TH, D, WR>), dim3(pl.grid), dim3(320), lds, st, P);
+    hipLaunchKernelGGL((cabp_kernel<MT, CS, TH, D, WR, UP>), dim3(pl.grid), dim3(320), lds, st, P);
     return sn_check_launch();
 }
 
@@ -823,17 +901,23 @@
     return launch_conv3p<MT, CS, 8, D, D, false>(K, pl, mode, st);
 }
 
-int sn_conv3p_launch(const sn_conv_desc* d, int lines_len, int route, const int* plan8, void* stream) {
+static int c3p_launch(const sn_conv_desc* d, int lines_len, int route, const int* plan8, const sn_up2_src* up, void* stream) {
     if ((route >> 24) != SN_CONV_K_STREAM || !plan8) return SN_EINVAL;
     C3P K;
     K.in = (const bf16_t*)d->in[0]; K.res = (const bf16_t*)d->res; K.out = (bf16_t*)d->out;
     K.wfrag = (const uint4*)d->wfrag; K.bias = d->bias; K.oscale = d->oscale; K.oscale_stride = d->oscale_stride;
     K.pool = d->pool; K.pool_rows = 0; K.act = d->act; K.prelu = d->prelu;
     K.T = d->T; K.h = d->h_out; K.w = d->w_out; K.lines_len = lines_len; K.dbg = (d->flags >> 12) & 7;
+    K.w2 = nullptr; K.b2 = nullptr; K.lo = nullptr; K.hs = K.ws = 0;
     const C3PPlan pl = {plan8[0], plan8[1], plan8[2], plan8[3], plan8[4], plan8[5], plan8[6], plan8[7]};
     hipStream_t st = (hipStream_t)stream;
     const int mt = (route >> 20) & 15, cs = (route >> 12) & 255, D = (route >> 8) & 15, mode = (route >> 4) & 15;
     const bool rl = route & 1;
+    if (up) {
+        if (route != SN_CONV_ROUTE(SN_CONV_K_STREAM, 2, 24, 1, 2, 1) || K.dbg) return SN_EINVAL;
+        K.lo = (const bf16_t*)up->lo; K.hs = up->hs; K.ws = up->ws;
+        return launch_conv3p_mode<2, 24, 8, 1, 2, true, true>(K, pl, st);
+    }
     switch (mt * 1000 + cs) {
         case 1016:
             if (rl) return launch_conv3p_mode<1, 16, 8, 2, 2, true>(K, pl, st);
@@ -847,7 +931,11 @@
     }
 }
 
-int sn_cabp_launch(const sn_conv_desc* a, const sn_conv_desc* b, void* stream) {
+int sn_conv3p_launch(const sn_conv_desc* d, int lines_len, int route, const int* plan8, void* stream) {
+    return c3p_launch(d, lines_len, route, plan8, nullptr, stream);
+}
+
+int sn_cabp_launch(const sn_conv_desc* a, const sn_conv_desc* b, const sn_up2_src* up, void* stream) {
     const int key = a->mt * 1000 + a->cs_in, ncu = c3p_ncu();
     if (!ncu || !(key == 1016 || key == 2024) || a->act != 1 || !(a->prelu >= 0.f && a->prelu <= 1.f) || !b->oscale || b->res2) return SN_EINVAL;
     if ((size_t)a->h_out * a->w_out * a->cs_out * 2 >= 0x7fffffffull) return SN_EINVAL;
@@ -856,11 +944,39 @@
     K.wfrag = (const uint4*)a->wfrag; K.bias = a->bias; K.w2 = (const uint4*)b->wfrag; K.b2 = b->bias;
     K.oscale = b->oscale; K.oscale_stride = b->oscale_stride; K.pool = nullptr; K.pool_rows = 0; K.act = 1; K.prelu = a->prelu;
     K.T = a->T; K.h = a->h_out; K.w = a->w_out; K.lines_len = 0; K.dbg = 0;
+    K.lo = up ? (const bf16_t*)up->lo : nullptr; K.hs = up ? up->hs : 0; K.ws = up ? up->ws : 0;
     const int o = (a->flags >> 4) & 15;
     const bool shallow = ((a->flags >> 10) & 3) == 3;
     const C3PPlan pl = c3p_plan(a->T, a->h_out, a->w_out, 8, ncu, o ? o : (key == 1016 ? (shallow ? 3 : 2) : 1), c3p_segment(a->h_out, a->w_out, 8, c3p_wgs_default(key)));
     hipStream_t st = (hipStream_t)stream;
+    if (up) {
+        if (key != 1016 || shallow || ((b->flags >> 12) & 1)) return SN_EINVAL;
+        return launch_cabp<1, 16, 8, 2, 2, true>(K, pl, st);
+    }
     if (shallow) return key == 1016 ? launch_cabp<1, 16, 8, 1>(K, pl, st) : launch_cabp<2, 24, 8, 1>(K, pl, st);
     if (key == 1016 && !((b->flags >> 12) & 1)) return launch_cabp<1, 16, 8, 2, 2>(K, pl, st);
     return key == 1016 ? launch_cabp<1, 16, 8, 2>(K, pl, st) : launch_cabp<2, 24, 8, 2>(K, pl, st);
 }
+
+static int up2_fold_width(const sn_conv_desc* d, const sn_up2_src* up) {
+    if (!d || !up || up->hs < 2 || up->ws < 2 || d->h_out != 2 * up->hs || d->w_out != 2 * up->ws || d->out_mode != 0 || d->res2) return 0;
+    if (!(d->k == 3 && d->stride == 1 && d->pad == 1 && d->in_mode == 0 && d->n_in == 1 && d->cs_in == d->cs_out && d->ks == (9 * d->cs_in + 31) / 32 &&
+          d->h_in == d->h_out && d->w_in == d->w_out) || sn_remap_set(d->clip_n, d->clip_T, d->clip_lo) || (d->flags & SN_CONV_TILE_KERNEL)) return 0;
+    if ((size_t)d->h_out * d->w_out * d->cs_out * 2 >= 0x7fffffffull) return 0;
+    const int key = d->mt * 1000 + d->cs_in;
+    if (key == 1016) return ((d->flags >> 12) & 1) ? 0 : 16;
+    if (key == 2024) return (d->flags & 512) ? 0 : 24;
+    return 0;
+}
+
+int sn_up2_fold_supported(const sn_conv_desc* conv2, const sn_up2_src* up) { return up2_fold_width(conv2, up) != 0 ? 1 : 0; }
+
+int sn_conv2d_up2(const sn_conv_desc* d, const sn_up2_src* up, void* stream) {
+    sn_clear_error();
+    if (up2_fold_width(d, up) != 24 || !up->lo || !d->out || !d->in[0] || !d->wfrag || !d->res || !d->oscale || d->oscale_stride < 16 * d->mt || d->pool ||
+        d->act != 0 || d->T < 1) return SN_EINVAL;
+    int plan8[8];
+    const int route = sn_conv3p_route(d, 0, 0, plan8);
+    if (route < 0) return SN_EINVAL;
+    return c3p_launch(d, 0, route, plan8, up, stream);
+}
diff --git a/shift-net_amd/csrc/sn_up2.h b/shift-net_amd/csrc/sn_up2.h
--- /dev/null
+++ b/shift-net_amd/csrc/sn_up2.h
@@ -0,0 +1,30 @@
+#pragma once
+#include "sn_common.h"
+
+__device__ __forceinline__ void up2_col(int x, int ws, int& x0, int& x1, float& hx, float& lx) {
+    float sx = x * 0.5f - 0.25f; if (sx < 0.f) sx = 0.f;
+    x0 = (int)sx; x1 = min(x0 + 1, ws - 1);
+    lx = sx - x0; hx = 1.f - lx;
+}
+
+__device__ __forceinline__ void up2_row(int i, bool odd, float& wt, float& wb) {
+    if (odd) { wt = 0.75f; wb = 0.25f; }
+    else { wb = i > 0 ? 0.75f : 0.f; wt = 1.f - wb; }
+}
+
+__device__ __forceinline__ float up2_blend_h(float hx, float lx, float p0, float p1) {
+#pragma clang fp contract(off)
+    const float r = lx * p1;
+    return __builtin_fmaf(hx, p0, r);
+}
+
+__device__ __forceinline__ float up2_blend_v(float wt, float wb, float vt, float vb, float f) {
+#pragma clang fp contract(off)
+    const float r = wb * vb;
+    const float s = __builtin_fmaf(wt, vt, r);
+    return s + f;
+}
+
+__device__ __forceinline__ float up2_value(float hx, float lx, float wt, float wb, float t0, float t1, float b0, float b1, float f) {
+    return up2_blend_v(wt, wb, up2_blend_h(hx, lx, t0, t1), up2_blend_h(hx, lx, b0, b1), f);
+}
diff --git a/shift-net_amd/shiftnet_amd/engine.py b/shift-net_amd/shiftnet_amd/engine.py
--- a/shift-net_amd/shiftnet_amd/engine.py
+++ b/shift-net_amd/shiftnet_amd/engine.py
@@ -60,7 +60,7 @@
     def conv(self, name: str, ins: Sequence[Act], *, stride: int = 1, pad: Optional[int] = None, prelu: Optional[float] = None,
              res: Optional[Act] = None, out_mode: int = 0, pool: bool = False, in_mode: int = 0, oscale: Optional[torch.Tensor] = None,
              nchw_out: Optional[torch.Tensor] = None, nchw_sc: Optional[torch.Tensor] = None, res2: Optional[Act] = None,
-             remap: Optional[Tuple[int, int, int]] = None):
+             remap: Optional[Tuple[int, int, int]] = None, up: Optional[Act] = None):
         p = self.P.convs[name]
         k, cout = int(p["k"]), int(p["cout"])
         T, hs, ws, cs_in = ins[0].dims
@@ -110,6 +110,10 @@
             pool_buf = torch.empty((T, nblk, 16 * d.mt), dtype=torch.float32, device=self.dev)
             d.pool = pool_buf.data_ptr()
         self._meta = ("conv", T, h_out, w_out, len(ins) * cs_in, int(d.cs_out), k, stride, in_mode, out_mode)
+        if up is not None:
+            assert up.dims == (T, h_out // 2, w_out // 2, int(d.cs_out)) and not pool, (up.dims, out_act.dims)
+            self._call_as("sn_conv2d", "sn_conv2d_up2", f"sn_conv2d_up2[{name}]", C.byref(d), C.byref(L.Up2Src(up.t.data_ptr(), up.dims[1], up.dims[2])), self._stream())
+            return out_act
         self._call("sn_conv2d", f"sn_conv2d[{name}]", C.byref(d), self._stream())
         if pool:
             return out_act, pool_buf, h_out * w_out
@@ -123,22 +127,30 @@
     range_guard = os.environ.get("SN_RANGE_GUARD", "1") != "0"
     range_guard_async = os.environ.get("SN_RANGE_GUARD", "1") == "async"
 
-    def cab(self, pre: str, x: Act, extra: Optional[Act] = None) -> Act:
+    def _call_as(self, rec: str, fn: str, label: str, *args) -> None:
+        self._call(fn, label, *args)
+        if self.prof is not None:
+            _, lb, meta, e0, e1 = self.prof.pop()
+            self.prof.append((rec, lb, meta, e0, e1))
+
+    def cab(self, pre: str, x: Act, extra: Optional[Act] = None, up: Optional[Act] = None) -> Act:
         p = self.P.cas[pre + "CA"]
         T, h, w, cs = x.dims
         slope = self.P.scalar(pre + "body.1.weight")
         if self.cab_fused in ("8", "16", "s8", "s16") or (self.cab_fused[0] == "p" and extra is None and not self.conv_tiles and
-                                                          (self.cab_fused == "p" or (cs == 16 and T * h * w >= self.CAB_FUSED_MIN_PX))):
-            out = self._cab_fused(pre, x, extra, slope)
+                                                          (self.cab_fused == "p" or (cs == 16 and T * h * w >= self.CAB_FUSED_MIN_PX))
+                                                          and (up is None or cs == 16)):
+            out = self._cab_fused(pre, x, extra, slope, up)
             if out is not None:
                 return out
+        assert up is None or (cs == 24 and extra is None), "skip_up_cab folds where _skipup_fold says so"
         scratch = torch.empty((self.lib.sn_cab_ca_scratch_floats(T),), dtype=torch.float32, device=self.dev)
         mid, pool, _ = self.conv(pre + "body.0", [x], prelu=slope, pool=True)
         _, nblk, cpad = pool.shape
         ca = torch.empty((T, cpad), dtype=torch.float32, device=self.dev)
         self._call("sn_cab_ca", f"sn_cab_ca[{pre}]", pool.data_ptr(), nblk, cpad, mid.t.data_ptr(), cs, p["c"], p["cr"], h, w,
                    p["w2"].data_ptr(), p["wa"].data_ptr(), p["wb"].data_ptr(), scratch.data_ptr(), ca.data_ptr(), T, self._stream())
-        return self.conv(pre + "body.2", [mid], res=x, oscale=ca, res2=extra)
+        return self.conv(pre + "body.2", [mid], res=x, oscale=ca, res2=extra, up=up)
 
     cab_fused = os.environ.get("SN_CAB_FUSED", "p16")
     CAB_FUSED_MIN_PX = 4 << 20
@@ -158,7 +170,7 @@
         d.flags = L.SN_CONV_TILE_KERNEL
         return d
 
-    def _cab_fused(self, pre: str, x: Act, extra: Optional[Act], slope: float) -> Optional[Act]:
+    def _cab_fused(self, pre: str, x: Act, extra: Optional[Act], slope: float, up: Optional[Act] = None) -> Optional[Act]:
         lib = self.lib
         T, h, w, cs = x.dims
         if h < 2 or w < 2:
@@ -194,6 +206,11 @@
         self._call("sn_cab_ca_lines", f"sn_cab_ca[{pre}]", pool.data_ptr(), nblk, 16 * d1.mt, lines.data_ptr(), ll, cs, p["c"], p["cr"], h, w,
                    p["w2"].data_ptr(), p["wa"].data_ptr(), p["wb"].data_ptr(), scratch.data_ptr(), ca.data_ptr(), T, st)
         self._meta = ("cabf", T, h, w, cs, 3 if extra is not None else 2)
+        if up is not None:
+            assert rows == 0 and extra is None and up.dims == (T, h // 2, w // 2, cs), (up.dims, x.dims)
+            self._call_as("sn_cab_fused", "sn_cab_fused_up2", f"sn_cab_fused_up2[{pre}]", C.byref(d1), C.byref(d2),
+                          C.byref(L.Up2Src(up.t.data_ptr(), up.dims[1], up.dims[2])), rows, st)
+            return Act(out, x.c)
         self._call("sn_cab_fused", f"sn_cab_fused[{pre}]", C.byref(d1), C.byref(d2), rows, st)
         return Act(out, x.c)
 
@@ -425,6 +442,35 @@
         self._call("sn_upsample2_add", f"sn_upsample2_add[{name}]", lo.t.data_ptr(), y.t.data_ptr(), out.data_ptr(), T, hs, ws, cs, self._stream())
         return Act(out, lo.c)
 
+    skip_up_fold = os.environ.get("SN_SKIPUP_FOLD", "1") != "0"
+
+    def _skipup_fold(self, cab_pre: str, enc: Act) -> bool:
+        T, h, w, cs = enc.dims
+        if not (self.skip_up_fold and self.skip_up_lowres) or self.conv_tiles or h < 4 or w < 4 or (h | w) & 1 or self.cab_fused[0] not in "0p":
+            return False
+        slope = self.P.scalar(cab_pre + "body.1.weight")
+        streaming_cab = self.cab_fused == "p" or (self.cab_fused == "p16" and cs == 16 and T * h * w >= self.CAB_FUSED_MIN_PX)
+        d2 = self._conv_desc(cab_pre + "body.2", enc)
+        if cs == 16:
+            if not (streaming_cab and 0.0 <= slope <= 1.0) or self.conv_depth == 3:
+                return False
+            d2.flags = L.conv_flags(dbg=self.conv_dbg & 1)
+        elif cs == 24:
+            if self.conv_dbg:
+                return False
+            d2.flags = L.conv_flags(self.conv_wgs, self.conv_stream_all, self.conv_res_regs, self.conv_depth, self.conv_dbg, self.conv_s2_small)
+        else:
+            return False
+        return bool(self.lib.sn_up2_fold_supported(C.byref(d2), C.byref(L.Up2Src(None, h // 2, w // 2))))
+
+    def skip_up_cab(self, name: str, dec: Act, cab_pre: str, enc: Act) -> Act:
+        if not self._skipup_fold(cab_pre, enc):
+            return super().skip_up_cab(name, dec, cab_pre, enc)
+        lo = self.conv(name, [dec])
+        assert enc.dims == (lo.dims[0], 2 * lo.dims[1], 2 * lo.dims[2], lo.dims[3]), (enc.dims, lo.dims)
+        out = self.cab(cab_pre, enc, up=lo)
+        return Act(out.t, lo.c)
+
     def _ingest(self, x: torch.Tensor, noise_map: Optional[torch.Tensor]) -> Act:
         T, cin, H, W = x.shape
         nm_ptr = None
diff --git a/shift-net_amd/shiftnet_amd/lib.py b/shift-net_amd/shiftnet_amd/lib.py
--- a/shift-net_amd/shiftnet_amd/lib.py
+++ b/shift-net_amd/shiftnet_amd/lib.py
@@ -25,6 +25,7 @@
     "sn32_conv2d", "sn32_conv2d_route", "sn32_gsts_gather", "sn32_layernorm", "sn32_gate", "sn32_gate_sum", "sn32_chan_sum", "sn32_scale_residual", "sn32_ingest", "sn32_cab_ca", "sn32_dw_gate", "sn32_conv1x1_gate2", "sn32_gsts_shiftconv", "sn32_conv_csum_tiles",
     "sn_ln_gemm_gate", "sn_lngate_blocks", "sn_grp5_gemm_gate", "sn_grp5_blocks", "sn_gsts_cab2_phase1", "sn_cab1_phase1", "sn_phase1_pool_blocks", "sn_phase1_g1_store_bytes", "sn_p1r_plan", "sn_p1r_strip_begin",
     "sn_cab2_phase2_cab1_phase1", "sn_cab2_phase2_cab1_phase1_supported",
+    "sn_up2_fold_supported", "sn_conv2d_up2", "sn_cab_fused_up2",
 ]
 
 
@@ -62,6 +63,10 @@
 
 
 SN_CONV_TILE_KERNEL = 1
+
+
+class Up2Src(C.Structure):
+    _fields_ = [("lo", C.c_void_p), ("hs", C.c_int), ("ws", C.c_int)]
 
 
 def conv_flags(wgs: int = 0, stream_all: bool = False, res_regs: bool = False, depth: int = 0, dbg: int = 0, s2_small: bool = False) -> int:
@@ -218,6 +223,9 @@
     lib.sn_cab_stats.argtypes = [C.POINTER(ConvDesc), ci, vp]
     lib.sn_cab_ca_lines.argtypes = [vp, ci, ci, vp, ci, ci, ci, ci, ci, ci, vp, vp, vp, vp, vp, ci, vp]
     lib.sn_cab_fused.argtypes = [C.POINTER(ConvDesc), C.POINTER(ConvDesc), ci, vp]
+    lib.sn_up2_fold_supported.argtypes = [C.POINTER(ConvDesc), C.POINTER(Up2Src)]
+    lib.sn_conv2d_up2.argtypes = [C.POINTER(ConvDesc), C.POINTER(Up2Src), vp]
+    lib.sn_cab_fused_up2.argtypes = [C.POINTER(ConvDesc), C.POINTER(ConvDesc), C.POINTER(Up2Src), ci, vp]
     lib.sn32_cab_ca.argtypes = [vp, ci, ci, vp, ci, ci, ci, ci, vp, vp, vp, vp, vp, ci, vp]
     lib.sn_gsts_gather.argtypes = [C.POINTER(UnitSrc), vp, vp, vp]
     lib.sn_temporal_roll.argtypes = [C.POINTER(UnitSrc), vp, vp]
diff --git a/shift-net_amd/shiftnet_amd/network.py b/shift-net_amd/shiftnet_amd/network.py
--- a/shift-net_amd/shiftnet_amd/network.py
+++ b/shift-net_amd/shiftnet_amd/network.py
@@ -146,6 +146,9 @@
     def skip_up(self, name: str, x: Act, y: Act) -> Act:
         return self.conv(name, [x], in_mode=1, res=y)
 
+    def skip_up_cab(self, name: str, dec: Act, cab_pre: str, enc: Act) -> Act:
+        return self.skip_up(name, dec, self.cab(cab_pre, enc))
+
     def tfr_unet(self, pre: str, x: Act, extra: Optional[Act] = None) -> Act:
         def seq(nm: str, n: int, t: Act, ex: Optional[Act] = None) -> Act:
             for i in range(n):
@@ -155,9 +158,9 @@
         enc2 = seq("encoder_level2", 3, self.down(pre + "down12.", enc1))
         enc3 = seq("encoder_level3", 3, self.down(pre + "down23.", enc2))
         dec3 = seq("decoder_level3", 3, enc3)
-        t = self.skip_up(pre + "up32", dec3, self.cab(pre + "skip_attn2.", enc2))
+        t = self.skip_up_cab(pre + "up32", dec3, pre + "skip_attn2.", enc2)
         dec2 = seq("decoder_level2", 3, t)
-        t = self.skip_up(pre + "up21", dec2, self.cab(pre + "skip_attn1.", enc1))
+        t = self.skip_up_cab(pre + "up21", dec2, pre + "skip_attn1.", enc1)
         return seq("decoder_level1", 1, t, extra)
 
     def stage1(self, x: Act) -> Act:
@@ -173,7 +176,7 @@
             e = self.down(p + "down12.", enc11)
             e = self.shift_chain([f"{p}{n}." for n in ("encoder_level2", "encoder_level2_1", "encoder_level2_2",
                                                        "decoder_level2", "decoder_level2_1", "decoder_level2_2")], e)
-            x = self.skip_up(p + "up21", e, self.cab(p + "skip_attn1.", enc11))
+            x = self.skip_up_cab(p + "up21", e, p + "skip_attn1.", enc11)
         else:
             if V.shift_cab:
                 e = self.shift_cab(p + "encoder_level1.", x, False)
@@ -185,9 +188,9 @@
             e = self.down(p + "down23.", enc22)
             enc33 = self.cab(p + "encoder_level3_1.", self.cab(p + "encoder_level3.", e))
             d = self.shift_chain([p + "decoder_level3.", p + "decoder_level3_1."], enc33)
-            x = self.skip_up(p + "up32", d, self.cab(p + "skip_attn2.", enc22))
+            x = self.skip_up_cab(p + "up32", d, p + "skip_attn2.", enc22)
             d = self.shift_chain([p + "decoder_level2.", p + "decoder_level2_1."], x)
-            x = self.skip_up(p + "up21", d, self.cab(p + "skip_attn1.", enc11))
+            x = self.skip_up_cab(p + "up21", d, p + "skip_attn1.", enc11)
         dec11 = self.shift_chain([p + "decoder_level1.", p + "decoder_level1_1.", p + "decoder_level1_2."], x)
         skip = self.cab(p + "skip_conv.", shortcut)
         if V.hr_cat:
```
